# SakibSaikia/CPURayTracer

Hardware: AMD Instinct MI355X
Metric: Msamples/sec (WxHxspp/s), 1200x800 cover scene spp=128 d=50 (higher is better)
Workload: dtype f32; 1 GPU; cover scene (488 spheres, scene seed 1) 1200x800 spp=128 depth=50, render seed 1; rows sharded cyclically (row j to rank j mod N) over 1 GPU(s), RCCL gather of strips to rank 0; n_spheres=488, spp=128, spp_per_gpu=128, passes=1

## Files before the change

### cpuraytracer_amd/_capi.py

```python
import ctypes as C
import os

import numpy as np

_HERE = os.path.dirname(os.path.abspath(__file__))
LIB_PATH = os.path.join(_HERE, "lib", "librt_hip.so")


class RtSphere(C.Structure):
    _fields_ = [("cx", C.c_float), ("cy", C.c_float), ("cz", C.c_float), ("r", C.c_float)]


class RtMaterial(C.Structure):
    _fields_ = [("type", C.c_uint32), ("tex_type", C.c_uint32), ("smoothness", C.c_float), ("ior", C.c_float),
                ("tiling", C.c_float), ("rgb0", C.c_float * 3), ("rgb1", C.c_float * 3), ("luminance", C.c_float)]


class RtCamera(C.Structure):
    _fields_ = [("origin", C.c_float * 4), ("x", C.c_float * 4), ("y", C.c_float * 4),
                ("origin_image_plane", C.c_float * 4), ("aperture", C.c_float), ("focal_length", C.c_float)]


class RtLight(C.Structure):
    _fields_ = [("direction", C.c_float * 3), ("color", C.c_float * 3), ("luminance", C.c_float)]


class RtRowset(C.Structure):
    _fields_ = [("first_row", C.c_uint32), ("num_rows", C.c_uint32), ("block_rows", C.c_uint32),
                ("shard", C.c_uint32), ("nshards", C.c_uint32)]


class RtStats(C.Structure):
    _fields_ = [("samples", C.c_uint64), ("traversals", C.c_uint64), ("segments", C.c_uint64),
                ("ms_render", C.c_double), ("ms_accumulate", C.c_double), ("ms_resolve", C.c_double),
                ("local_rows", C.c_uint32), ("passes", C.c_uint32)]


SPHERE_DTYPE = np.dtype([("cx", "<f4"), ("cy", "<f4"), ("cz", "<f4"), ("r", "<f4")])
MATERIAL_DTYPE = np.dtype([("type", "<u4"), ("tex_type", "<u4"), ("smoothness", "<f4"), ("ior", "<f4"),
                           ("tiling", "<f4"), ("rgb0", "<f4", (3,)), ("rgb1", "<f4", (3,)), ("luminance", "<f4")])

RT_OK = 0
RT_ERR_NO_DEVICE = 1
RT_SAMPLER_COSINE_HEMISPHERE, RT_SAMPLER_SQRT_DISK = 1, 2

EXPORTS = [
    "rt_last_error", "rt_api_version", "rt_create", "rt_destroy", "rt_set_stream", "rt_set_workspace_limit", "rt_set_sampler", "rt_set_frame_pipelining", "rt_set_frame_batch", "rt_set_frame_lookahead", "rt_committed_samples",
    "rt_scene_upload", "rt_render", "rt_clear", "rt_resolve", "rt_last_resolve_ms", "rt_download", "rt_copy_to_device",
    "rt_synchronize", "rt_rowset_local_rows", "rt_rowset_global_row", "rt_unit_halton", "rt_unit_math",
    "rt_unit_primary_rays", "rt_unit_closest_hit", "rt_unit_trace", "rt_unit_camera_rays", "rt_unit_scatter", "rt_unit_tonemap", "rt_unit_layout", "rt_unit_layout_info", "rt_unit_grid_rows",
    "rt_unit_tile_masks", "rt_unit_tile_masks_host", "rt_unit_tile_cone",
]

_lib = None


class RtError(RuntimeError):
    def __init__(self, code, msg):
        super().__init__("librt_hip: [%d] %s" % (code, msg))
        self.code = code


def load():
    global _lib
    if _lib is not None:
        return _lib
    if not os.path.exists(LIB_PATH):
        raise RuntimeError("librt_hip.so is missing (%s): run `python -c 'import __graft_entry__ as g; g.build()'`; "
                           "there is no CPU fallback for the render path" % LIB_PATH)
    L = C.CDLL(LIB_PATH)
    L.rt_last_error.restype = C.c_char_p
    L.rt_api_version.restype = C.c_int
    L.rt_create.argtypes = [C.c_int, C.POINTER(C.c_void_p)]
    L.rt_destroy.argtypes = [C.c_void_p]
    L.rt_destroy.restype = None
    L.rt_set_stream.argtypes = [C.c_void_p, C.c_void_p]
    L.rt_set_workspace_limit.argtypes = [C.c_void_p, C.c_uint64]
    L.rt_set_sampler.argtypes = [C.c_void_p, C.c_uint32]
    L.rt_set_frame_pipelining.argtypes = [C.c_void_p, C.c_uint32]
    L.rt_set_frame_batch.argtypes = [C.c_void_p, C.c_uint32]
    L.rt_committed_samples.argtypes = [C.c_void_p, C.POINTER(C.c_uint32)]
    L.rt_set_frame_lookahead.argtypes = [C.c_void_p, C.c_uint32]
    L.rt_scene_upload.argtypes = [C.c_void_p, C.c_void_p, C.c_void_p, C.c_uint32, C.POINTER(RtCamera), C.POINTER(RtLight), C.c_uint32,
                                  C.POINTER(RtMaterial), C.c_float]
    L.rt_render.argtypes = [C.c_void_p, C.c_uint32, C.c_uint32, RtRowset, C.c_uint32, C.c_uint32, C.c_uint32, C.c_uint64,
                            C.POINTER(RtStats)]
    L.rt_clear.argtypes = [C.c_void_p]
    L.rt_resolve.argtypes = [C.c_void_p, C.c_uint32]
    L.rt_last_resolve_ms.argtypes = [C.c_void_p]
    L.rt_last_resolve_ms.restype = C.c_double
    L.rt_download.argtypes = [C.c_void_p, C.c_void_p, C.c_void_p]
    L.rt_copy_to_device.argtypes = [C.c_void_p, C.c_void_p, C.c_void_p]
    L.rt_synchronize.argtypes = [C.c_void_p]
    L.rt_rowset_local_rows.argtypes = [RtRowset]
    L.rt_rowset_local_rows.restype = C.c_uint32
    L.rt_rowset_global_row.argtypes = [RtRowset, C.c_uint32]
    L.rt_rowset_global_row.restype = C.c_uint32
    L.rt_unit_halton.argtypes = [C.c_void_p, C.c_void_p, C.c_uint32, C.c_uint32, C.c_void_p]
    L.rt_unit_math.argtypes = [C.c_void_p, C.c_uint32, C.c_void_p, C.c_void_p, C.c_uint32, C.c_void_p]
    L.rt_unit_primary_rays.argtypes = [C.c_void_p, C.c_uint32, C.c_uint32, C.c_void_p, C.c_uint32, C.c_void_p]
    L.rt_unit_closest_hit.argtypes = [C.c_void_p, C.c_void_p, C.c_uint32, C.c_void_p]
    L.rt_unit_trace.argtypes = [C.c_void_p, C.c_uint32, C.c_uint32, C.c_void_p, C.c_uint32, C.c_uint32, C.c_uint64,
                                C.c_void_p, C.c_void_p]
    L.rt_unit_camera_rays.argtypes = [C.c_void_p, C.POINTER(RtCamera), C.c_void_p, C.c_uint32, C.c_void_p]
    L.rt_unit_scatter.argtypes = [C.c_void_p, C.POINTER(RtMaterial), C.POINTER(RtLight), C.POINTER(C.c_float), C.c_void_p, C.c_uint32,
                                  C.c_void_p]
    L.rt_unit_tonemap.argtypes = [C.c_void_p, C.c_void_p, C.c_uint32, C.c_uint32, C.c_void_p]
    L.rt_unit_layout.argtypes = [C.c_void_p, C.c_uint32, C.c_uint32, C.POINTER(C.c_uint32), C.c_void_p, C.c_void_p]
    L.rt_unit_layout_info.argtypes = [C.c_void_p, C.c_uint32, C.POINTER(C.c_uint32)]
    if hasattr(L, "rt_unit_tile_masks"):
        L.rt_unit_tile_masks.argtypes = [C.c_void_p, C.c_uint32, C.c_uint32, RtRowset, C.c_uint32, C.POINTER(C.c_uint32), C.c_void_p,
                                         C.c_uint32, C.c_void_p, C.c_void_p]
        L.rt_unit_tile_masks_host.argtypes = [C.c_void_p, C.c_uint32, C.POINTER(RtCamera), C.c_uint32, C.c_uint32, RtRowset, C.c_uint32,
                                              C.c_uint32, C.POINTER(C.c_uint32), C.c_void_p, C.c_void_p]
        L.rt_unit_tile_cone.argtypes = [C.POINTER(RtCamera), C.c_uint32, C.c_uint32, C.c_uint32, C.c_uint32, C.c_uint32, C.c_void_p]
    _lib = L
    return L


def check(rc):
    if rc != RT_OK:
        raise RtError(rc, load().rt_last_error().decode())


def whole_image(H):
    return RtRowset(0, H, H, 0, 1)


BLOCK_ROWS = 1


def cyclic_rows(H, rank, world, block_rows=BLOCK_ROWS):
    return RtRowset(0, H, block_rows, rank, world)
```

### cpuraytracer_amd/csrc/rt_capi.hip

```cpp
#include <hip/hip_runtime.h>

#include <algorithm>
#include <cmath>
#include <cstdio>
#include <cstdlib>
#include <cstring>
#include <memory>
#include <mutex>
#include <set>
#include <string>
#include <unordered_map>
#include <array>
#include <utility>
#include <vector>

#include "../../include/rt_api.h"
#include "rt_kernels.h"

namespace {

thread_local std::string g_err;

int Fail(int code, const std::string& msg) {
    g_err = msg;
    return code;
}

#define RT_HIP(call)                                                                                             \
    do {                                                                                                         \
        hipError_t e_ = (call);                                                                                  \
        if (e_ != hipSuccess) {                                                                                  \
            return Fail(e_ == hipErrorOutOfMemory ? RT_ERR_OUT_OF_MEMORY : RT_ERR_HIP,                           \
                        std::string(#call) + ": " + hipGetErrorString(e_) + " (" __FILE__ ":" + std::to_string(__LINE__) + ")"); \
        }                                                                                                        \
    } while (0)

uint32_t EnvU32(const char* name, uint32_t dflt) {
    const char* v = std::getenv(name);
    if (!v || !*v) return dflt;
    return (uint32_t)std::strtoul(v, nullptr, 10);
}

uint32_t TreeTopFromEnv() {
    const uint32_t t = EnvU32("RT_TREE_TOP", 128);
    return (t < 4 || t > 128) ? 128u : t;
}

template <typename T>
struct DevBuf {
    T* ptr = nullptr;
    size_t count = 0;
    int Reserve(size_t n) {
        if (n <= count) return RT_OK;
        if (ptr) (void)hipFree(ptr);
        ptr = nullptr;
        count = 0;
        hipError_t e = hipMalloc(reinterpret_cast<void**>(&ptr), n * sizeof(T));
        if (e != hipSuccess) {
            (void)hipGetLastError();
            return Fail(RT_ERR_OUT_OF_MEMORY, std::string("hipMalloc: ") + hipGetErrorString(e));
        }
        count = n;
        return RT_OK;
    }
    void Release() {
        if (ptr) (void)hipFree(ptr);
        ptr = nullptr;
        count = 0;
    }
};

}

struct rt_ctx {
    int device = 0;
    hipStream_t ownStream = nullptr;
    hipStream_t stream = nullptr;
    hipEvent_t ev[4] = {nullptr, nullptr, nullptr, nullptr};
    std::vector<hipEvent_t> passEv;
    int cuCount = 0;
    size_t ldsPerBlockMax = 0;
    uint64_t workspaceLimit = 8ull << 30;

    bool hasScene = false;
    uint32_t n = 0;
    DevBuf<float4> scan, tree, leaf;
    DevBuf<uint32_t> orig;
    DevBuf<uint16_t> sgCells, sgEntries, sgGlobal;
    DevBuf<float4> sgSph;
    struct ExtraLight {
        DevBuf<uint16_t> cells, entries, global;
    };
    ExtraLight extraIdx[RT_MAX_LIGHTS];
    DevBuf<rtd::LightRec> lightRecs;
    DevBuf<uint16_t> gridCells;
    DevBuf<uint32_t> gridQ;
    bool useShadowGrid = true;
    DevBuf<float> radius;
    DevBuf<rt_material> mats;
    DevBuf<uint4> mats16;
    bool mats16Ok = false;
    rtd::TraceParams base{};

    uint32_t W = 0, H = 0, rows = 0;
    rt_rowset rs{};
    uint32_t accumulated = 0;
    uint32_t sampler = 0;
    DevBuf<float> hdr;
    DevBuf<uint8_t> ldr;
    DevBuf<float> samples;
    DevBuf<uint32_t> queue;
    DevBuf<unsigned long long> counters;
    DevBuf<float2> jitterTab, lensTab;
    double lastResolveMs = 0.0;

    uint32_t blocksPerCu = 4;
    uint32_t blockThreads = 256;
    bool useMfma = true;
    bool matsInLds = true;
    bool useRayCache = true;
    bool useStash = true;
    bool treeInLds = true;
    uint32_t treeTop = 128;
    bool forceGlobal = false;

    bool useTileOrder = true;
    bool tileOrderValid = false;
    uint32_t tileW = 0, tileH = 0;
    rt_rowset tileRs{};
    DevBuf<float> pilotRays, pilotHits;
    DevBuf<uint32_t> tileOrder, matType;
    DevBuf<uint8_t> tileClass;
    bool tileMaskValid = false;
    uint32_t maskW = 0, maskH = 0, maskLimit = 0, maskTiles = 0;
    rt_rowset maskRs{};
    DevBuf<uint32_t> tileMasks;
    uint64_t freshScans = 0;

    uint32_t pipeDepth = 0;
    bool pipeOpen = false;
    uint32_t pipeSeq = 0;
    uint32_t pipeSppCap = 0, pipeNpix = 0, pipeRing = 0;
    uint32_t pipeInSel = 0;
    uint32_t pipeCommits = 0;
    uint32_t batchFrames = 1;
    bool pendOn = false;
    uint32_t pendW = 0, pendH = 0, pendS0 = 0, pendS1 = 0, pendDepth = 0;
    rt_rowset pendRs{};
    uint64_t pendSeed = 0;
    uint32_t lookahead = 1;
    bool aheadValid = false;
    uint32_t aheadW = 0, aheadH = 0, aheadBase = 0, aheadSpp = 0, aheadNext = 0, aheadDepth = 0;
    rt_rowset aheadRs{};
    uint64_t aheadSeed = 0;
    uint32_t pipeMaxDepth = 0;
    uint64_t pipeSeed = 0;
    rtd::RegionTable pipeRegions{};
    DevBuf<float> ring;
    DevBuf<rtd::ContEntry> cont[2];
    DevBuf<uint32_t> contN[2];
    DevBuf<rtd::FrameCtl> ctl;
};

static uint32_t RowsetLocalRows(rt_rowset rs) {
    if (rs.block_rows == 0 || rs.nshards == 0 || rs.shard >= rs.nshards) return 0;
    uint32_t rows = 0;
    const uint32_t nblocks = (rs.num_rows + rs.block_rows - 1) / rs.block_rows;
    for (uint32_t b = rs.shard; b < nblocks; b += rs.nshards) {
        const uint32_t r0 = b * rs.block_rows;
        const uint32_t left = rs.num_rows - r0;
        rows += left < rs.block_rows ? left : rs.block_rows;
    }
    return rows;
}

struct SceneLayout {
    std::vector<float4> scan;
    std::vector<uint32_t> orig;
    std::vector<float4> leaf;
    std::vector<float4> tree;
    uint32_t levelOff[rtd::kMaxLevels] = {0}, levelCnt[rtd::kMaxLevels] = {0};
    uint32_t nLevels = 1;
    uint32_t nGroups = 0;
    float boundNorm = 0.f;
    unsigned long long singleMask[2] = {0ull, 0ull};
    uint32_t nAlways = 0;
    float treeBox[9] = {0, 0, 0, 0, 0, 0, 0, 0, 0};
    bool treeBoxOn = false;
    bool gridOn = false;
    std::vector<uint16_t> gridCellStart;
    uint32_t gridNu = 0, gridNv = 0, gridAxU = 0, gridAxV = 2;
    float gridG0u = 0.f, gridG0v = 0.f, gridInvH = 0.f, gridRmaxOverH = 0.f, gridBigNorm = 0.f;
    std::vector<uint32_t> gridQ;
    float gridQc[8] = {0, 0, 0, 0, 0, 0, 0, 0};
};

static float4 BoundOf(const rt_sphere* sp, const std::vector<uint32_t>& ids, float* normOut, float marginK) {
    if (ids.empty()) return make_float4(0.f, 0.f, 0.f, 1e30f);
    const double kEps = (double)marginK * 5.9604644775390625e-08;
    double lo[3] = {1e300, 1e300, 1e300}, hi[3] = {-1e300, -1e300, -1e300};
    for (uint32_t k : ids) {
        const double c[3] = {sp[k].cx, sp[k].cy, sp[k].cz};
        for (int a = 0; a < 3; ++a) {
            lo[a] = std::min(lo[a], c[a] - (double)sp[k].r);
            hi[a] = std::max(hi[a], c[a] + (double)sp[k].r);
        }
    }
    double cc[3] = {0.5 * (lo[0] + hi[0]), 0.5 * (lo[1] + hi[1]), 0.5 * (lo[2] + hi[2])};
    if (ids.size() > 1) {
        auto reachOf = [&](const double c[3]) {
            double far = 0.0;
            for (uint32_t k : ids) {
                const double dx = sp[k].cx - c[0], dy = sp[k].cy - c[1], dz = sp[k].cz - c[2];
                far = std::max(far, std::sqrt(dx * dx + dy * dy + dz * dz) + (double)sp[k].r);
            }
            return far;
        };
        double best = reachOf(cc);
        double step = 0.25 * best;
        for (int it = 0; it < 400 && step > 1e-7 * best; ++it) {
            bool improved = false;
            for (int ax = 0; ax < 3; ++ax)
                for (int sgn = -1; sgn <= 1; sgn += 2) {
                    double t[3] = {cc[0], cc[1], cc[2]};
                    t[ax] += sgn * step;
                    const double r = reachOf(t);
                    if (r < best) {
                        best = r;
                        cc[0] = t[0]; cc[1] = t[1]; cc[2] = t[2];
                        improved = true;
                    }
                }
            if (!improved) step *= 0.5;
        }
    }
    const float Cf[3] = {(float)cc[0], (float)cc[1], (float)cc[2]};
    double R = 0, smax = 0;
    for (uint32_t k : ids) {
        const double dx = sp[k].cx - (double)Cf[0], dy = sp[k].cy - (double)Cf[1], dz = sp[k].cz - (double)Cf[2];
        const double si = std::sqrt(dx * dx + dy * dy + dz * dz);
        smax = std::max(smax, si);
        R = std::max(R, si + (double)sp[k].r);
    }
    const double C2 = (double)Cf[0] * Cf[0] + (double)Cf[1] * Cf[1] + (double)Cf[2] * Cf[2];
    const double Cn = std::sqrt(C2);
    const double Rf2 = R * R * (1.0 + 1e-5) + 0.01 * smax * smax + kEps * (2.0 * (Cn + R) * (Cn + R) + R * R);
    float w = (float)(C2 - Rf2);
    w = std::nextafterf(std::nextafterf(w, -INFINITY), -INFINITY);
    if (normOut) *normOut = std::max(*normOut, (float)((Cn + R) * 1.001));
    return make_float4(Cf[0], Cf[1], Cf[2], w);
}

static double EnclosingRadius(const rt_sphere* sp, const uint32_t* ids, size_t n) {
    if (n == 0) return 0.0;
    double lo[3] = {1e300, 1e300, 1e300}, hi[3] = {-1e300, -1e300, -1e300};
    for (size_t q = 0; q < n; ++q) {
        const rt_sphere& s = sp[ids[q]];
        const double c[3] = {s.cx, s.cy, s.cz};
        for (int a = 0; a < 3; ++a) {
            lo[a] = std::min(lo[a], c[a] - (double)s.r);
            hi[a] = std::max(hi[a], c[a] + (double)s.r);
        }
    }
    double cc[3] = {0.5 * (lo[0] + hi[0]), 0.5 * (lo[1] + hi[1]), 0.5 * (lo[2] + hi[2])};
    auto reachOf = [&](const double c[3]) {
        double far = 0.0;
        for (size_t q = 0; q < n; ++q) {
            const rt_sphere& s = sp[ids[q]];
            const double dx = s.cx - c[0], dy = s.cy - c[1], dz = s.cz - c[2];
            far = std::max(far, std::sqrt(dx * dx + dy * dy + dz * dz) + (double)s.r);
        }
        return far;
    };
    double best = reachOf(cc);
    if (n == 1) return best;
    double step = 0.25 * best;
    for (int it = 0; it < 60 && step > 1e-4 * best; ++it) {
        bool improved = false;
        for (int ax = 0; ax < 3; ++ax)
            for (int sgn = -1; sgn <= 1; sgn += 2) {
                double t[3] = {cc[0], cc[1], cc[2]};
                t[ax] += sgn * step;
                const double r = reachOf(t);
                if (r < best) { best = r; cc[0] = t[0]; cc[1] = t[1]; cc[2] = t[2]; improved = true; }
            }
        if (!improved) step *= 0.5;
    }
    return best;
}
// ... 577 lines not shown
            tp.ray_cache_off16 = (uint32_t)(ldsBytes / 16);
            tp.ray_cache_stride16 = (cap * rtd::kStashDwords * 4 + 15) / 16;
            ldsBytes += (size_t)wavesPerBlock * tp.ray_cache_stride16 * 16;
        }
        if (matsL2 && !useStash) return Fail(RT_ERR_HIP, "internal: materials through L2 without the stash variant");
        const bool matsGlobal = matsL2 || tree || (grid && !gridLds) || !tp.mats_in_lds || (!flat && !ldsTables && !gridLds);
        if (want16 && tp.mats16_mode == 0u && matsGlobal) tp.mats16_mode = 1u;
    }
    if (!useStash && ctx->useRayCache && ldsBytes + (size_t)wavesPerBlock * rtd::kRayCacheBytes <= 160 * 1024 / ctx->blocksPerCu) {
        tp.ray_cache_off16 = (uint32_t)(ldsBytes / 16);
        tp.ray_cache_stride16 = rtd::kRayCacheBytes / 16;
        ldsBytes += (size_t)wavesPerBlock * rtd::kRayCacheBytes;
    }
    if (std::getenv("RT_VERBOSE"))
        std::fprintf(stderr, "rt_trace launch: tree=%d flat=%d ldsTables=%d blocks=%u threads=%u lds=%zu B (cand %zu, tables %zu, leaf %zu, ops %zu, sg %zu, tree %zu, cache %s, stash %u)\n",
                     (int)tree, (int)flat + 2 * (int)grid + 4 * (int)gridLds, (int)ldsTables, blocks, ctx->blockThreads, ldsBytes, candBytes, ldsTables ? lds : (size_t)0, flat ? leafBytes : (size_t)0,
                     (flat || tree) ? MfmaOpsBytesFor(topCnt) : (size_t)0, sgBytes, treeBytes, (tp.ray_cache_off16 && !useStash) ? "yes" : "no", tp.stash_cap);
    const bool hitLds = flat && tp.mats_in_lds && (sgBytes != 0 || !tp.sg_enabled);
    if (carryMode != 0) {
        const bool ok = hitLds && tp.ray_cache_off16 != 0 && ctx->blockThreads == 1024;
        if (carryMode == 1) return ok ? RT_OK : RT_ERR_INVALID_ARG;
        if (!ok) return Fail(RT_ERR_INVALID_ARG, "frame pipelining needs the flat LDS variant of the trace kernel");
    }
#define RT_LAUNCH_FN(KERNEL)                                                                                                  \
    do {                                                                                                                      \
        const void* fn_ = reinterpret_cast<const void*>(&KERNEL);                                                             \
         \
        if (ldsBytes > 48 * 1024 && RaiseLdsLimit(ctx->device, fn_) != RT_OK) return RT_ERR_HIP;                               \
        hipLaunchKernelGGL(KERNEL, dim3(blocks), dim3(ctx->blockThreads), ldsBytes, ctx->stream, tp);                         \
    } while (0)
#define RT_LAUNCH_K(...)                                                          \
    do {                                                                          \
        if (tp.n_lights == 1u) RT_LAUNCH_FN((rtd::rt_trace_kernel<__VA_ARGS__>)); \
        else RT_LAUNCH_FN((rtd::rt_trace_kernel_lights<__VA_ARGS__>));            \
    } while (0)
#define RT_LAUNCH(LDS, T, M)                                                                        \
    do {                                                                                            \
        if (((M) == 1 && hitLds) || ((M) == 2 && tp.tree_in_lds)) {                                 \
            if (tp.ray_cache_off16) RT_LAUNCH_K(LDS, T, M, true, (M) != 0);  \
            else RT_LAUNCH_K(LDS, T, M, false, (M) != 0);                    \
        } else {                                                                                    \
            if (tp.ray_cache_off16) RT_LAUNCH_K(LDS, T, M, true, false);    \
            else RT_LAUNCH_K(LDS, T, M, false, false);                      \
        }                                                                                           \
    } while (0)
#define RT_LAUNCH_T(LDS, M)                                            \
    do {                                                               \
        if (ctx->blockThreads == 1024) RT_LAUNCH(LDS, 1024, M);        \
        else if (ctx->blockThreads == 512) RT_LAUNCH(LDS, 512, M);     \
        else RT_LAUNCH(LDS, 256, M);                                   \
    } while (0)
    if (carryMode == 2) RT_LAUNCH_K(true, 1024, 1, true, true, true);
    else if (gridLds && useStash && tp.grid_in_lds) RT_LAUNCH_K(true, 1024, 3, true, true, false, true);
    else if (gridLds && tp.grid_in_lds && tp.ray_cache_off16) RT_LAUNCH_K(true, 1024, 3, true, true);
    else if (gridLds && tp.grid_in_lds) RT_LAUNCH_K(true, 1024, 3, false, true);
    else if (grid && gridSgLds && useStash && tp.grid_in_lds) RT_LAUNCH_K(false, 1024, 3, true, true, false, true, false, true);
    else if (grid && gridSgLds) return Fail(RT_ERR_HIP, "internal: the grid variant with the shadow index in LDS needs the hit stash");
    else if (grid && ctx->blockThreads == 1024 && useStash && tp.grid_in_lds && gridQBytes != 0) RT_LAUNCH_K(false, 1024, 3, true, true, false, true, false, false, true);
    else if (grid && gridQBytes != 0) return Fail(RT_ERR_HIP, "internal: quantised grid bounds without the stash variant");
    else if (grid && ctx->blockThreads == 1024 && useStash && tp.grid_in_lds) RT_LAUNCH_K(false, 1024, 3, true, true, false, true);
    else if (grid && ctx->blockThreads == 1024 && tp.grid_in_lds && tp.ray_cache_off16) RT_LAUNCH_K(false, 1024, 3, true, true);
    else if (grid && ctx->blockThreads == 1024 && tp.grid_in_lds) RT_LAUNCH_K(false, 1024, 3, false, true);
    else if (grid && ctx->blockThreads == 1024) RT_LAUNCH_K(false, 1024, 3, false, false);
    else if (grid && ctx->blockThreads == 512 && !tp.ray_cache_off16) RT_LAUNCH_K(false, 512, 3, false, false);
    else if (grid && ctx->blockThreads == 512) RT_LAUNCH_K(false, 512, 3, true, false);
    else if (grid && !tp.ray_cache_off16) RT_LAUNCH_K(false, 256, 3, false, false);
    else if (grid) RT_LAUNCH_K(false, 256, 3, true, false);
    else if (useStash && tree && tp.tree_in_lds) RT_LAUNCH_K(false, 1024, 2, true, true, false, true);
    else if (useStash && tree) RT_LAUNCH_K(false, 1024, 2, true, false, false, true);
    else if (useStash && hitLds && matsL2) RT_LAUNCH_K(true, 1024, 1, true, true, false, true, true);
    else if (useStash && hitLds) RT_LAUNCH_K(true, 1024, 1, true, true, false, true);
    else if (useStash) RT_LAUNCH_K(true, 1024, 1, true, false, false, true);
    else if (tree) RT_LAUNCH_T(false, 2);
    else if (flat) RT_LAUNCH_T(true, 1);
    else if (ldsTables) RT_LAUNCH_T(true, 0);
    else RT_LAUNCH_T(false, 0);
#undef RT_LAUNCH_T
#undef RT_LAUNCH
#undef RT_LAUNCH_K
#undef RT_LAUNCH_FN
    RT_HIP(hipGetLastError());
    return RT_OK;
}


static int LaunchClosest(rt_ctx* ctx, const float* dRays, uint32_t n, float* dOut) {
        rtd::TraceParams tp = ctx->base;
        const TraceVariant V = ChooseVariant(ctx, tp);
        tp.mats_in_lds = 0;
        tp.sg_in_lds = 0;
        const uint32_t topCnt = tp.level_cnt[tp.n_levels - 1];
        const size_t waves = 256 / 64;
        size_t ldsBytes = waves * (V.grid ? rtd::kWaveGridBytes : (V.tree ? rtd::kWaveCandBytes : rtd::kWaveListBytes));
        if (V.grid) {
            tp.grid_in_lds = 0;
        } else if (V.tree) {
            ldsBytes += MfmaOpsBytesFor(topCnt);
            const size_t treeBytes = (size_t)(tp.level_off[tp.n_levels - 1] + topCnt) * 16;
            tp.tree_in_lds = (ctx->treeInLds && ldsBytes + treeBytes <= 160 * 1024) ? 1u : 0u;
            if (tp.tree_in_lds) ldsBytes += treeBytes;
        } else if (V.flat || V.ldsTables) {
            ldsBytes += LdsBytesFor(tp.n, tp.n_padded, false);
            if (V.flat) ldsBytes += V.leafBytes + MfmaOpsBytesFor(topCnt);
        }
#define RT_UNIT_CLOSEST(LDS, M)                                                                                        \
    do {                                                                                                               \
        const void* fn_ = reinterpret_cast<const void*>(&rtd::k_unit_closest<LDS, M>);                                 \
        if (ldsBytes > 48 * 1024) RT_HIP(hipFuncSetAttribute(fn_, hipFuncAttributeMaxDynamicSharedMemorySize, (int)ldsBytes)); \
        hipLaunchKernelGGL((rtd::k_unit_closest<LDS, M>), dim3((n + 255) / 256), dim3(256), ldsBytes, ctx->stream, tp, dRays, n, dOut); \
    } while (0)
        if (V.grid) RT_UNIT_CLOSEST(false, 3);
        else if (V.tree) RT_UNIT_CLOSEST(false, 2);
        else if (V.flat) RT_UNIT_CLOSEST(true, 1);
        else if (V.ldsTables) RT_UNIT_CLOSEST(true, 0);
        else RT_UNIT_CLOSEST(false, 0);
#undef RT_UNIT_CLOSEST
        RT_HIP(hipGetLastError());
    return RT_OK;
}

static int BuildTileOrder(rt_ctx* ctx, uint32_t W, uint32_t H, rt_rowset rs, uint32_t npix) {
    if (ctx->tileOrderValid && ctx->tileW == W && ctx->tileH == H && std::memcmp(&ctx->tileRs, &rs, sizeof(rs)) == 0) return RT_OK;
    ctx->tileOrderValid = false;
    const uint32_t nFull = npix >> 6;
    if (!ctx->useTileOrder || nFull < 2u * (uint32_t)ctx->cuCount) return RT_OK;
    int rc;
    const uint32_t nPilot = nFull * rtd::kPilotsPerTile;
    if ((rc = ctx->pilotRays.Reserve((size_t)nPilot * 6)) != RT_OK) return rc;
    if ((rc = ctx->pilotHits.Reserve((size_t)nPilot * 10)) != RT_OK) return rc;
    if ((rc = ctx->tileClass.Reserve(nFull)) != RT_OK) return rc;
    if ((rc = ctx->tileOrder.Reserve(nFull)) != RT_OK) return rc;
    rtd::TraceParams tp = ctx->base;
    tp.W = W;
    tp.H = H;
    tp.rs = rs;
    tp.s0 = 1;
    tp.sampler = ctx->sampler;
    tp.jitter_tab = nullptr;
    tp.lens_tab = nullptr;
    hipLaunchKernelGGL(rtd::rt_pilot_rays_kernel, dim3((nPilot + 255) / 256), dim3(256), 0, ctx->stream, tp, nFull, ctx->pilotRays.ptr);
    RT_HIP(hipGetLastError());
    if ((rc = LaunchClosest(ctx, ctx->pilotRays.ptr, nPilot, ctx->pilotHits.ptr)) != RT_OK) return rc;
    hipLaunchKernelGGL(rtd::rt_tile_class_kernel, dim3((nFull + 255) / 256), dim3(256), 0, ctx->stream, ctx->pilotHits.ptr, nFull, W,
                       ctx->matType.ptr, ctx->tileClass.ptr);
    hipLaunchKernelGGL(rtd::rt_tile_order_kernel, dim3(1), dim3(1024), 0, ctx->stream, ctx->tileClass.ptr, nFull, ctx->tileOrder.ptr);
    RT_HIP(hipGetLastError());
    ctx->tileOrderValid = true;
    ctx->tileW = W;
    ctx->tileH = H;
    ctx->tileRs = rs;
    return RT_OK;
}

static int BuildTileMasks(rt_ctx* ctx, uint32_t W, uint32_t H, rt_rowset rs, uint32_t npix) {
    const uint32_t limit = EnvU32("RT_PRIMARY_MASK_LIMIT", rtd::kTileMaskLimitDefault);
    const uint32_t nFull = npix >> 6;
    const rtd::TraceParams& b = ctx->base;
    const bool wanted = EnvU32("RT_PRIMARY_MASK", 1u) != 0u && nFull != 0u && b.n_levels == 1u && b.level_cnt[0] <= 128u &&
                        ChooseVariant(ctx, b).flat;
    if (!wanted) {
        ctx->tileMaskValid = false;
        return RT_OK;
    }
    if (ctx->tileMaskValid && ctx->maskW == W && ctx->maskH == H && ctx->maskLimit == limit && std::memcmp(&ctx->maskRs, &rs, sizeof(rs)) == 0)
        return RT_OK;
    ctx->tileMaskValid = false;
    int rc;
    if ((rc = ctx->tileMasks.Reserve((size_t)nFull * rtd::kTileMaskWords)) != RT_OK) return rc;
    rtd::TraceParams tp = b;
    tp.W = W;
    tp.H = H;
    tp.rs = rs;
    hipLaunchKernelGGL(rtd::rt_tile_mask_kernel, dim3((nFull + 3) / 4), dim3(256), 0, ctx->stream, tp, nFull, limit, ctx->tileMasks.ptr);
    RT_HIP(hipGetLastError());
    ctx->tileMaskValid = true;
    ctx->maskW = W;
    ctx->maskH = H;
    ctx->maskLimit = limit;
    ctx->maskTiles = nFull;
    ctx->maskRs = rs;
    return RT_OK;
}

static void PipelineDrop(rt_ctx* ctx) { ctx->pipeOpen = false; }
static uint32_t PipelineWaves(const rt_ctx* ctx) { return (uint32_t)ctx->cuCount * ctx->blocksPerCu * (ctx->blockThreads / 64); }
static void PipelineShards(const rt_ctx* ctx, rtd::TraceParams& tp) {
    uint32_t qb = EnvU32("RT_PIPE_QUEUE_BLOCK", rtd::kCarryQueueBlock) / 64u * 64u;
    if (qb == 0) qb = 64;
    QueueShards(tp, PipelineWaves(ctx), qb, EnvU32("RT_PIPE_STATIC_BLOCKS", 1));
}

static int PipelineTraceAndCommit(rt_ctx* ctx, rtd::TraceParams& tp, uint32_t npix, bool carry) {
    tp.ctl = ctx->ctl.ptr;
    tp.cont_in = ctx->cont[ctx->pipeInSel].ptr;
    tp.cont_in_n = ctx->contN[ctx->pipeInSel].ptr;
    tp.cont_out = ctx->cont[ctx->pipeInSel ^ 1u].ptr;
    tp.cont_out_n = ctx->contN[ctx->pipeInSel ^ 1u].ptr;
    tp.carry = carry ? 1u : 0u;
    tp.region_seq = ctx->pipeSeq;
    tp.max_carry_age = ctx->pipeDepth;
    tp.min_iters = EnvU32("RT_PIPE_MIN_ITERS", 8);
    tp.counters = ctx->counters.ptr;
    int rc = LaunchTrace(ctx, tp, 2);
    if (rc != RT_OK) return rc;
    hipLaunchKernelGGL(rtd::rt_commit_kernel, dim3((npix + 255) / 256), dim3(256), 0, ctx->stream, ctx->ring.ptr, ctx->hdr.ptr, npix,
                       npix * ctx->pipeSppCap, ctx->pipeRing, ctx->pipeRegions, ctx->ctl.ptr, ctx->pipeSeq, ctx->pipeCommits);
    RT_HIP(hipGetLastError());
    ++ctx->pipeCommits;
    ctx->pipeInSel ^= 1u;
    return RT_OK;
}

static int PipelineFlush(rt_ctx* ctx) {
    if (!ctx->pipeOpen) return RT_OK;
    const uint32_t npix = ctx->pipeNpix;
    rtd::TraceParams tp = ctx->base;
    tp.total_paths = 0;
    PipelineShards(ctx, tp);
    hipLaunchKernelGGL(rtd::rt_raygen_tables_kernel, dim3(1), dim3(256), 0, ctx->stream, (float2*)nullptr, 0u, 0u, (float2*)nullptr, 0u, 0u,
                       ctx->sampler, ctx->queue.ptr, ctx->ctl.ptr);
    RT_HIP(hipGetLastError());
    tp.W = ctx->W;
    tp.H = ctx->H;
    tp.rs = ctx->rs;
    tp.s0 = 1;
    tp.spp_pass = 1;
    tp.npix_local = npix;
    tp.max_depth = ctx->pipeMaxDepth;
    tp.sampler = ctx->sampler;
    tp.seed = ctx->pipeSeed;
    tp.samples = ctx->ring.ptr;
    int rc = PipelineTraceAndCommit(ctx, tp, npix, false);
    ctx->pipeOpen = false;
    if (rc != RT_OK) ctx->accumulated = 0;
    return rc;
}

static int PipelineRender(rt_ctx* ctx, uint32_t W, uint32_t H, rt_rowset rs, uint32_t npix, uint32_t s0, uint32_t s1, uint32_t max_depth,
                          uint64_t seed) {
    const uint32_t spp = s1 - s0;
    const uint32_t nRing = ctx->pipeDepth + 2u;
    int rc;
    if (ctx->pipeOpen && (ctx->pipeNpix != npix || spp > ctx->pipeSppCap || ctx->pipeRing != nRing || ctx->pipeMaxDepth != max_depth ||
                          ctx->pipeSeed != seed)) {
        if ((rc = PipelineFlush(ctx)) != RT_OK) return rc;
    }
    if (!ctx->pipeOpen) {
        ctx->pipeNpix = npix;
        ctx->pipeSppCap = spp;
        ctx->pipeRing = nRing;
        ctx->pipeMaxDepth = max_depth;
        ctx->pipeSeed = seed;
        ctx->pipeInSel = 0;
        ctx->pipeRegions = rtd::RegionTable{};
        const size_t waves = PipelineWaves(ctx);
        if ((rc = ctx->ring.Reserve((size_t)nRing * npix * spp * 3)) != RT_OK) return rc;
        for (int k = 0; k < 2; ++k) {
            if ((rc = ctx->cont[k].Reserve(waves * 64)) != RT_OK) return rc;
            if ((rc = ctx->contN[k].Reserve(waves)) != RT_OK) return rc;
            RT_HIP(hipMemsetAsync(ctx->contN[k].ptr, 0, waves * sizeof(uint32_t), ctx->stream));
        }
        if ((rc = ctx->ctl.Reserve(1)) != RT_OK) return rc;
        rtd::FrameCtl init{};
        init.oldest_open = 0xffffffffu;
        init.committed_seq[0] = ctx->pipeSeq;
        init.committed_samples[0] = ctx->accumulated;
        ctx->pipeCommits = 0;
        RT_HIP(hipMemcpyAsync(ctx->ctl.ptr, &init, sizeof(init), hipMemcpyHostToDevice, ctx->stream));
        RT_HIP(hipStreamSynchronize(ctx->stream));
        ctx->pipeOpen = true;
    }
    const uint32_t seq = ++ctx->pipeSeq;
    const uint32_t slot = seq % nRing;
    ctx->pipeRegions.seq[slot] = seq;
    ctx->pipeRegions.spp[slot] = spp;
    rtd::TraceParams tp = ctx->base;
    tp.W = W;
    tp.H = H;
    tp.rs = rs;
    tp.s0 = s0;
    tp.spp_pass = spp;
    tp.total_paths = npix * spp;
    tp.npix_local = npix;
    tp.max_depth = max_depth;
    tp.sampler = ctx->sampler;
    tp.seed = seed;
    tp.path_list = nullptr;
    tp.tile_order = nullptr;
    tp.samples = ctx->ring.ptr;
    tp.sample_base = slot * npix * ctx->pipeSppCap;
    tp.trav_out = nullptr;
    const uint32_t k0 = s0 + rs.first_row;
    const uint32_t nLens = spp + W + rs.num_rows;
    if ((rc = ctx->jitterTab.Reserve(spp)) != RT_OK) return rc;
    if ((rc = ctx->lensTab.Reserve(nLens)) != RT_OK) return rc;
    tp.jitter_tab = ctx->jitterTab.ptr;
    tp.lens_tab = ctx->lensTab.ptr;
    tp.lens_k0 = k0;
    const uint32_t nmax = spp > nLens ? spp : nLens;
    PipelineShards(ctx, tp);
    hipLaunchKernelGGL(rtd::rt_raygen_tables_kernel, dim3((nmax + 255) / 256), dim3(256), 0, ctx->stream, ctx->jitterTab.ptr, s0, spp,
                       ctx->lensTab.ptr, k0, nLens, ctx->sampler, ctx->queue.ptr, ctx->ctl.ptr);
    RT_HIP(hipGetLastError());
    return PipelineTraceAndCommit(ctx, tp, npix, true);
}

namespace {
template <typename T>
struct TmpDev {
    T* p = nullptr;
    ~TmpDev() {
        if (p) (void)hipFree(p);
    }
    hipError_t Alloc(size_t n) { return hipMalloc(reinterpret_cast<void**>(&p), (n ? n : 1) * sizeof(T)); }
};
}

extern "C" {

const char* rt_last_error(void) { return g_err.c_str(); }
int rt_api_version(void) { return RT_API_VERSION; }

int rt_create(int device_ordinal, rt_ctx** out) {
    if (!out) return Fail(RT_ERR_INVALID_ARG, "rt_create: null out");
    *out = nullptr;
    int count = 0;
    hipError_t e = hipGetDeviceCount(&count);
    if (e != hipSuccess || count <= 0)
        return Fail(RT_ERR_NO_DEVICE, std::string("rt_create: no HIP device (") + hipGetErrorString(e) +
                                          "); this library has no CPU fallback");
    if (device_ordinal < 0 || device_ordinal >= count) return Fail(RT_ERR_NO_DEVICE, "rt_create: device ordinal out of range");
    RT_HIP(hipSetDevice(device_ordinal));
    std::unique_ptr<rt_ctx, void (*)(rt_ctx*)> guard(new rt_ctx(), rt_destroy);
    rt_ctx* ctx = guard.get();
    ctx->device = device_ordinal;
    hipDeviceProp_t prop;
    RT_HIP(hipGetDeviceProperties(&prop, device_ordinal));
    ctx->cuCount = prop.multiProcessorCount;
    ctx->ldsPerBlockMax = prop.sharedMemPerBlock;
    RT_HIP(hipStreamCreateWithFlags(&ctx->ownStream, hipStreamNonBlocking));
    ctx->stream = ctx->ownStream;
    for (auto& ev : ctx->ev) RT_HIP(hipEventCreate(&ev));
    {
        const char* scan = std::getenv("RT_SCAN");
        ctx->useMfma = !(scan && std::strcmp(scan, "valu") == 0);
        ctx->matsInLds = EnvU32("RT_MATS_LDS", 1) != 0;
        ctx->useShadowGrid = EnvU32("RT_SHADOW_GRID", 1) != 0;
        ctx->useRayCache = EnvU32("RT_RAY_CACHE", 1) != 0;
        ctx->useStash = EnvU32("RT_STASH", 1) != 0;
        ctx->treeInLds = EnvU32("RT_TREE_LDS", 1) != 0;
        ctx->useTileOrder = EnvU32("RT_TILE_ORDER", 1) != 0;
        ctx->treeTop = TreeTopFromEnv();
    }
    ctx->blocksPerCu = EnvU32("RT_BLOCKS_PER_CU", ctx->useMfma ? 1 : 4);
    if (ctx->blocksPerCu == 0) ctx->blocksPerCu = 1;
    ctx->forceGlobal = EnvU32("RT_FORCE_GLOBAL_TABLES", 0) != 0;
    ctx->blockThreads = EnvU32("RT_BLOCK_THREADS", ctx->useMfma ? 1024 : 256);
    if (ctx->blockThreads != 256 && ctx->blockThreads != 512 && ctx->blockThreads != 1024) ctx->blockThreads = 256;
    int rc = ctx->queue.Reserve(rtd::kQueueShards * rtd::kShardStrideWords);
    if (rc == RT_OK) rc = ctx->counters.Reserve(4);
    if (rc != RT_OK) return rc;
    {
        size_t freeB = 0, totalB = 0;
        RT_HIP(hipMemGetInfo(&freeB, &totalB));
        uint64_t lim = 64ull << 30;
        if (lim > freeB / 2) lim = freeB / 2;
        const uint32_t envGiB = EnvU32("RT_WORKSPACE_GIB", 0);
        if (envGiB) lim = (uint64_t)envGiB << 30;
        if (lim < (1ull << 20)) lim = 1ull << 20;
        ctx->workspaceLimit = lim;
    }
    *out = guard.release();
    return RT_OK;
}

void rt_destroy(rt_ctx* ctx) {
    if (!ctx) return;
    (void)hipSetDevice(ctx->device);
    (void)hipStreamSynchronize(ctx->stream);
    ctx->scan.Release();
    ctx->orig.Release();
    ctx->tree.Release();
    ctx->sgCells.Release();
    ctx->gridCells.Release();
    ctx->gridQ.Release();
    ctx->sgEntries.Release();
    ctx->sgGlobal.Release();
    ctx->sgSph.Release();
    for (auto& x : ctx->extraIdx) {
        x.cells.Release();
        x.entries.Release();
        x.global.Release();
    }
    ctx->lightRecs.Release();
    ctx->radius.Release();
    ctx->mats.Release();
    ctx->mats16.Release();
    ctx->hdr.Release();
    ctx->ldr.Release();
    ctx->samples.Release();
    ctx->queue.Release();
    ctx->counters.Release();
    ctx->jitterTab.Release();
    ctx->lensTab.Release();
    ctx->leaf.Release();
    ctx->pilotRays.Release();
    ctx->pilotHits.Release();
    ctx->tileOrder.Release();
    ctx->tileMasks.Release();
    ctx->tileClass.Release();
    ctx->matType.Release();
    ctx->ring.Release();
    ctx->cont[0].Release();
    ctx->cont[1].Release();
    ctx->contN[0].Release();
    ctx->contN[1].Release();
    ctx->ctl.Release();
    for (auto& ev : ctx->ev)
        if (ev) (void)hipEventDestroy(ev);
    for (auto& ev : ctx->passEv)
        if (ev) (void)hipEventDestroy(ev);
    if (ctx->ownStream) (void)hipStreamDestroy(ctx->ownStream);
    delete ctx;
}

static int BatchFlush(rt_ctx* ctx);

int rt_set_stream(rt_ctx* ctx, void* hip_stream) {
    if (!ctx) return Fail(RT_ERR_INVALID_ARG, "rt_set_stream: null ctx");
    {
        RT_HIP(hipSetDevice(ctx->device));
        const int rcb = BatchFlush(ctx);
        if (rcb != RT_OK) return rcb;
        const int rcf = PipelineFlush(ctx);
        if (rcf != RT_OK) return rcf;
    }
    ctx->aheadValid = false;
    ctx->stream = hip_stream ? reinterpret_cast<hipStream_t>(hip_stream) : ctx->ownStream;
    return RT_OK;
}

int rt_set_workspace_limit(rt_ctx* ctx, uint64_t bytes) {
    if (!ctx || bytes < (1u << 20)) return Fail(RT_ERR_INVALID_ARG, "rt_set_workspace_limit: need >= 1 MiB");
    ctx->workspaceLimit = bytes;
    return RT_OK;
}

static bool PackMaterials(const std::vector<rt_material>& matc, std::vector<uint4>& out) {
    auto byteOf = [](float c, uint32_t& b) {
        const float r = std::nearbyint(c * 255.0f);
        if (!(r >= 0.f && r <= 255.f)) return false;
        b = (uint32_t)r;
        return (float)b * (1.0f / 255.0f) == c;
    };
    out.assign(matc.size(), make_uint4(0u, 0u, 0u, 0u));
    for (size_t e = 0; e < matc.size(); ++e) {
        const rt_material& m = matc[e];
        if (m.type > 3u || m.tex_type > 1u) return false;
        uint32_t c0[3] = {0, 0, 0}, c1[3] = {0, 0, 0};
        const bool glass = m.type == RT_MAT_DIELECTRIC_TRANSPARENT;
        for (int k = 0; k < 3; ++k) {
            if (!glass && !byteOf(m.rgb0[k], c0[k])) return false;
            if (!glass && m.tex_type == RT_TEX_CHECKER && !byteOf(m.rgb1[k], c1[k])) return false;
        }
        const float slotA = m.type == RT_MAT_EMISSIVE ? m.luminance : m.smoothness;
        const float slotB = glass ? m.ior : m.tiling;
        uint32_t a, b;
        std::memcpy(&a, &slotA, 4);
        std::memcpy(&b, &slotB, 4);
        out[e] = make_uint4(m.type | m.tex_type << 2 | c0[0] << 8 | c0[1] << 16 | c0[2] << 24, c1[0] | c1[1] << 8 | c1[2] << 16, a, b);
    }
    return true;
}

int rt_scene_upload(rt_ctx* ctx, const rt_sphere* spheres, const rt_material* materials, uint32_t n, const rt_camera* camera,
                    const rt_light* lights, uint32_t n_lights, const rt_material* sky, float exposure_scale) {
    if (!ctx || !spheres || !materials || !camera || (!lights && n_lights != 0) || !sky || n == 0)
        return Fail(RT_ERR_INVALID_ARG, "rt_scene_upload: null pointer or empty scene");
    if (n_lights > RT_MAX_LIGHTS) return Fail(RT_ERR_INVALID_ARG, "rt_scene_upload: more than RT_MAX_LIGHTS lights");
    const rt_light noLight{{0.f, 1.f, 0.f}, {0.f, 0.f, 0.f}, 0.f};
    const rt_light* sun = n_lights ? lights : &noLight;
    RT_HIP(hipSetDevice(ctx->device));
    int rc;
    if ((rc = BatchFlush(ctx)) != RT_OK) return rc;
    SceneLayout L;
    BuildLayout(spheres, n, ctx->treeTop, L);
    if (L.scan.size() >= 65536) return Fail(RT_ERR_INVALID_ARG, "rt_scene_upload: scenes beyond 65,535 scan entries (about 65,000 spheres) are not supported");
    const uint32_t nPad = (uint32_t)L.scan.size();
    if ((rc = ctx->scan.Reserve(nPad)) != RT_OK) return rc;
    if ((rc = ctx->orig.Reserve(nPad)) != RT_OK) return rc;
    if ((rc = ctx->tree.Reserve(L.tree.size())) != RT_OK) return rc;
    if ((rc = ctx->leaf.Reserve(nPad)) != RT_OK) return rc;
    if ((rc = ctx->radius.Reserve(nPad)) != RT_OK) return rc;
    if ((rc = ctx->mats.Reserve(nPad)) != RT_OK) return rc;
    std::vector<float> rad(nPad, 0.f);
    std::vector<rt_material> matc(nPad);
    std::memset(matc.data(), 0, nPad * sizeof(rt_material));
    for (uint32_t e = 0; e < nPad; ++e) {
        if (L.orig[e] == 0xffffffffu) continue;
        rad[e] = spheres[L.orig[e]].r;
        matc[e] = materials[L.orig[e]];
    }
    RT_HIP(hipStreamSynchronize(ctx->stream));
    RT_HIP(hipMemcpy(ctx->scan.ptr, L.scan.data(), nPad * sizeof(float4), hipMemcpyHostToDevice));
    RT_HIP(hipMemcpy(ctx->orig.ptr, L.orig.data(), nPad * sizeof(uint32_t), hipMemcpyHostToDevice));
    RT_HIP(hipMemcpy(ctx->tree.ptr, L.tree.data(), L.tree.size() * sizeof(float4), hipMemcpyHostToDevice));
    RT_HIP(hipMemcpy(ctx->leaf.ptr, L.leaf.data(), nPad * sizeof(float4), hipMemcpyHostToDevice));
    RT_HIP(hipMemcpy(ctx->radius.ptr, rad.data(), nPad * sizeof(float), hipMemcpyHostToDevice));
    RT_HIP(hipMemcpy(ctx->mats.ptr, matc.data(), nPad * sizeof(rt_material), hipMemcpyHostToDevice));
    {
        std::vector<uint4> m16;
        ctx->mats16Ok = PackMaterials(matc, m16);
        if (ctx->mats16Ok) {
            if ((rc = ctx->mats16.Reserve(nPad)) != RT_OK) return rc;
            RT_HIP(hipMemcpy(ctx->mats16.ptr, m16.data(), nPad * sizeof(uint4), hipMemcpyHostToDevice));
        }
    }
    {
        std::vector<uint32_t> types(n);
        for (uint32_t k = 0; k < n; ++k) types[k] = materials[k].type;
        if ((rc = ctx->matType.Reserve(n)) != RT_OK) return rc;
        RT_HIP(hipMemcpy(ctx->matType.ptr, types.data(), n * sizeof(uint32_t), hipMemcpyHostToDevice));
        ctx->tileOrderValid = false;
        ctx->tileMaskValid = false;
    }

    ShadowGrid SG;
    if (ctx->useShadowGrid && n_lights != 0) BuildShadowGrid(spheres, L, sun->direction, (L.gridOn || L.nLevels > 1) ? EnvU32("RT_SHADOW_CELLS", 256u) : 64u, SG);
    std::vector<rtd::LightRec> recs;
    for (uint32_t k = 1; k < n_lights; ++k) {
        ShadowGrid G2;
        if (ctx->useShadowGrid) BuildShadowGrid(spheres, L, lights[k].direction, EnvU32("RT_SHADOW_CELLS", 256u), G2);
        rt_ctx::ExtraLight& X = ctx->extraIdx[k];
        rtd::LightRec R{};
        for (int c = 0; c < 3; ++c) {
            R.sun_dir[c] = lights[k].direction[c];
            R.sun_rad[c] = lights[k].luminance * lights[k].color[c];
            R.cam_o[c] = camera->origin[c];
        }
        R.sg_enabled = G2.enabled ? 1u : 0u;
        if (G2.enabled) {
            if ((rc = X.cells.Reserve(G2.cellStart.size())) != RT_OK) return rc;
            if ((rc = X.entries.Reserve(G2.entries.size() + 1)) != RT_OK) return rc;
            if ((rc = X.global.Reserve(G2.global.size() + 1)) != RT_OK) return rc;
            RT_HIP(hipMemcpy(X.cells.ptr, G2.cellStart.data(), G2.cellStart.size() * 2, hipMemcpyHostToDevice));
            if (!G2.entries.empty()) RT_HIP(hipMemcpy(X.entries.ptr, G2.entries.data(), G2.entries.size() * 2, hipMemcpyHostToDevice));
            if (!G2.global.empty()) RT_HIP(hipMemcpy(X.global.ptr, G2.global.data(), G2.global.size() * 2, hipMemcpyHostToDevice));
            for (int c = 0; c < 3; ++c) {
                R.sg_e1[c] = G2.e1[c];
                R.sg_e2[c] = G2.e2[c];
            }
            R.sg_u0 = G2.u0; R.sg_v0 = G2.v0; R.sg_inv_cell = G2.invCell; R.sg_p0sq = G2.p0sq;
            R.sg_nx = G2.nx; R.sg_ny = G2.ny; R.sg_nglobal = (uint32_t)G2.global.size();
            R.cell_start = X.cells.ptr; R.entries = X.entries.ptr; R.global = X.global.ptr;
        }
        recs.push_back(R);
    }
    if (!recs.empty()) {
        if ((rc = ctx->lightRecs.Reserve(recs.size())) != RT_OK) return rc;
        RT_HIP(hipMemcpy(ctx->lightRecs.ptr, recs.data(), recs.size() * sizeof(rtd::LightRec), hipMemcpyHostToDevice));
    }
    if (SG.enabled) {
// ... 139 lines not shown
    ctx->aheadValid = false;
    PipelineDrop(ctx);
    ctx->accumulated = 0;
    return RT_OK;
}

uint32_t rt_rowset_local_rows(rt_rowset rs) { return RowsetLocalRows(rs); }
uint32_t rt_rowset_global_row(rt_rowset rs, uint32_t lr) {
    const uint32_t lb = lr / rs.block_rows;
    const uint32_t k = lr % rs.block_rows;
    return rs.first_row + (lb * rs.nshards + rs.shard) * rs.block_rows + k;
}

static int RenderNow(rt_ctx* ctx, uint32_t W, uint32_t H, rt_rowset rs, uint32_t s0, uint32_t s1, uint32_t max_depth, uint64_t seed,
                     rt_stats* out_stats, uint32_t aheadEnd = 0);

static int BatchFlush(rt_ctx* ctx) {
    if (!ctx->pendOn) return RT_OK;
    ctx->pendOn = false;
    return RenderNow(ctx, ctx->pendW, ctx->pendH, ctx->pendRs, ctx->pendS0, ctx->pendS1, ctx->pendDepth, ctx->pendSeed, nullptr);
}

static bool PendingMustRender(const rt_ctx* ctx) { return ctx->pendOn && (ctx->accumulated == 0 || ctx->pendS0 == 1u); }

int rt_set_frame_batch(rt_ctx* ctx, uint32_t frames) {
    if (!ctx || frames == 0 || frames > 4096) return Fail(RT_ERR_INVALID_ARG, "rt_set_frame_batch: frames must be 1..4096");
    RT_HIP(hipSetDevice(ctx->device));
    const int rc = BatchFlush(ctx);
    ctx->batchFrames = frames;
    return rc;
}

int rt_set_frame_lookahead(rt_ctx* ctx, uint32_t frames) {
    if (!ctx || frames == 0 || frames > 4096) return Fail(RT_ERR_INVALID_ARG, "rt_set_frame_lookahead: frames must be 1..4096");
    ctx->lookahead = frames;
    ctx->aheadValid = false;
    return RT_OK;
}

int rt_render(rt_ctx* ctx, uint32_t W, uint32_t H, rt_rowset rs, uint32_t s0, uint32_t s1, uint32_t max_depth, uint64_t seed,
              rt_stats* out_stats) {
    if (!ctx) return Fail(RT_ERR_INVALID_ARG, "rt_render: null ctx");
    if (ctx->lookahead > 1 && ctx->batchFrames <= 1 && ctx->pipeDepth == 0 && out_stats == nullptr && ctx->hasScene && W != 0 && H != 0 && s0 != 0 && s1 > s0) {
        if (ctx->aheadValid && ctx->aheadW == W && ctx->aheadH == H && std::memcmp(&ctx->aheadRs, &rs, sizeof(rs)) == 0 && ctx->aheadDepth == max_depth &&
            ctx->aheadSeed == seed && s0 == ctx->aheadNext && s1 <= ctx->aheadBase + ctx->aheadSpp && ctx->accumulated + 1 == s0) {
            RT_HIP(hipSetDevice(ctx->device));
            const uint32_t npix = ctx->W * ctx->rows;
            hipLaunchKernelGGL(rtd::rt_accumulate_kernel, dim3((npix + 255) / 256), dim3(256), 0, ctx->stream, ctx->samples.ptr, ctx->hdr.ptr, npix,
                               ctx->aheadSpp, s0 - ctx->aheadBase, s1 - s0);
            RT_HIP(hipGetLastError());
            ctx->aheadNext = s1;
            ctx->accumulated += s1 - s0;
            return RT_OK;
        }
        const uint32_t want = s1 - s0 > ctx->lookahead ? s1 - s0 : ctx->lookahead;
        return RenderNow(ctx, W, H, rs, s0, s1, max_depth, seed, nullptr, s0 + want);
    }
    if (ctx->batchFrames > 1 && out_stats == nullptr && ctx->pipeDepth == 0 && ctx->hasScene && W != 0 && H != 0 && s0 != 0 && s1 > s0) {
        if (ctx->pendOn && !(ctx->pendW == W && ctx->pendH == H && std::memcmp(&ctx->pendRs, &rs, sizeof(rs)) == 0 && ctx->pendDepth == max_depth &&
                             ctx->pendSeed == seed && ctx->pendS1 == s0)) {
            const int rcf = BatchFlush(ctx);
            if (rcf != RT_OK) return rcf;
        }
        if (!ctx->pendOn) {
            const uint32_t rows = RowsetLocalRows(rs);
            const bool sameStrip = ctx->W == W && ctx->H == H && ctx->rows == rows && std::memcmp(&ctx->rs, &rs, sizeof(rs)) == 0;
            const bool starts = s0 == 1, continues = ctx->accumulated != 0 && sameStrip && s0 == ctx->accumulated + 1;
            if (rows != 0 && (uint64_t)rs.first_row + rs.num_rows <= H && (starts || continues)) {
                ctx->pendOn = true;
                ctx->pendW = W; ctx->pendH = H; ctx->pendRs = rs; ctx->pendS0 = s0; ctx->pendDepth = max_depth; ctx->pendSeed = seed;
            }
        }
        if (ctx->pendOn) {
            ctx->pendS1 = s1;
            if (ctx->pendS1 - ctx->pendS0 >= ctx->batchFrames) return BatchFlush(ctx);
            return RT_OK;
        }
    }
    const int rcb = BatchFlush(ctx);
    if (rcb != RT_OK) return rcb;
    return RenderNow(ctx, W, H, rs, s0, s1, max_depth, seed, out_stats);
}

static int RenderNow(rt_ctx* ctx, uint32_t W, uint32_t H, rt_rowset rs, uint32_t s0, uint32_t s1, uint32_t max_depth, uint64_t seed,
                     rt_stats* out_stats, uint32_t aheadEnd) {
    ctx->aheadValid = false;
    if (!ctx->hasScene) return Fail(RT_ERR_NO_SCENE, "rt_render: no scene uploaded");
    if (W == 0 || H == 0 || s0 == 0 || s1 <= s0) return Fail(RT_ERR_INVALID_ARG, "rt_render: empty image or sample range");
    const uint32_t rows = RowsetLocalRows(rs);
    if (rows == 0 || (uint64_t)rs.first_row + rs.num_rows > H) return Fail(RT_ERR_INVALID_ARG, "rt_render: bad row set");
    const uint64_t npix64 = (uint64_t)W * rows;
    if (npix64 > (1ull << 31) || (uint64_t)W * H > 0xffffffffull) return Fail(RT_ERR_INVALID_ARG, "rt_render: image too large");
    RT_HIP(hipSetDevice(ctx->device));
    const uint32_t npix = (uint32_t)npix64;

    const bool sameStrip = ctx->W == W && ctx->H == H && ctx->rows == rows && std::memcmp(&ctx->rs, &rs, sizeof(rs)) == 0;
    bool pipelined = ctx->pipeDepth > 0 && out_stats == nullptr;
    if (pipelined) {
        rtd::TraceParams probe = ctx->base;
        probe.total_paths = npix;
        pipelined = LaunchTrace(ctx, probe, 1) == RT_OK && (uint64_t)npix * (s1 - s0) * (ctx->pipeDepth + 2u) < (1ull << 31);
    }
    if (s0 == 1 || ctx->accumulated == 0) PipelineDrop(ctx);
    else if (!pipelined) {
        int rcf = PipelineFlush(ctx);
        if (rcf != RT_OK) return rcf;
    }
    if (s0 == 1 || ctx->accumulated == 0) {
        if (s0 != 1) return Fail(RT_ERR_SEQUENCE, "rt_render: first call of an accumulation must start at s0 == 1");
        int rc;
        if ((rc = ctx->hdr.Reserve((size_t)npix * 3)) != RT_OK) return rc;
        if ((rc = ctx->ldr.Reserve((size_t)npix * 3)) != RT_OK) return rc;
        RT_HIP(hipMemsetAsync(ctx->hdr.ptr, 0, (size_t)npix * 3 * sizeof(float), ctx->stream));
        ctx->W = W;
        ctx->H = H;
        ctx->rows = rows;
        ctx->rs = rs;
        ctx->accumulated = 0;
        if ((rc = BuildTileOrder(ctx, W, H, rs, npix)) != RT_OK) return rc;
        if ((rc = BuildTileMasks(ctx, W, H, rs, npix)) != RT_OK) return rc;
    } else if (!sameStrip || s0 != ctx->accumulated + 1) {
        return Fail(RT_ERR_SEQUENCE, "rt_render: sample range or row set does not continue the accumulation");
    }

    if (pipelined) {
        int rcp = PipelineRender(ctx, W, H, rs, npix, s0, s1, max_depth, seed);
        if (rcp != RT_OK) {
            ctx->accumulated = 0;
            PipelineDrop(ctx);
            return rcp;
        }
        ctx->accumulated += s1 - s0;
        return RT_OK;
    }

    const uint64_t bytesPerSpp = (uint64_t)npix * 12;
    uint64_t sppMax = ctx->workspaceLimit / bytesPerSpp;
    const uint64_t sppPathCap = ((1ull << 31) - 1) / npix;
    if (sppMax > sppPathCap) sppMax = sppPathCap;
    if (sppMax == 0) return Fail(RT_ERR_OUT_OF_MEMORY, "rt_render: workspace limit below one sample per pixel");
    const uint32_t sppTotal = s1 - s0;
    if (aheadEnd <= s1 || (uint64_t)(aheadEnd - s0) > sppMax || pipelined) aheadEnd = 0;
    const uint32_t sppTrace = aheadEnd ? aheadEnd - s0 : sppTotal;
    uint32_t sppPass = (uint32_t)(sppMax < sppTrace ? sppMax : sppTrace);
    int rc;
    while ((rc = ctx->samples.Reserve((size_t)npix * sppPass * 3)) != RT_OK) {
        if (rc != RT_ERR_OUT_OF_MEMORY || sppPass == 1u) return rc;
        sppPass = (sppPass + 1u) / 2u;
    }

    uint32_t passes = 0;
    auto runPasses = [&]() -> int {
        int rc;
        RT_HIP(hipMemsetAsync(ctx->counters.ptr, 0, 4 * sizeof(unsigned long long), ctx->stream));
        ctx->freshScans = 0;
        const uint32_t sEnd = aheadEnd ? aheadEnd : s1;
        for (uint32_t s = s0; s < sEnd; s += sppPass) {
            const uint32_t spp = (sEnd - s) < sppPass ? (sEnd - s) : sppPass;
            rtd::TraceParams tp = ctx->base;
            tp.W = W;
            tp.H = H;
            tp.rs = rs;
            tp.s0 = s;
            tp.spp_pass = spp;
            tp.total_paths = npix * spp;
            tp.npix_local = npix;
            tp.max_depth = max_depth;
            tp.sampler = ctx->sampler;
            tp.seed = seed;
            tp.path_list = nullptr;
            tp.tile_order = ctx->tileOrderValid ? ctx->tileOrder.ptr : nullptr;
            tp.tile_masks = (ctx->tileMaskValid && ctx->maskW == W && ctx->maskH == H && std::memcmp(&ctx->maskRs, &rs, sizeof(rs)) == 0) ? ctx->tileMasks.ptr : nullptr;
            ctx->freshScans += ((uint64_t)tp.total_paths + 63u) / 64u;
            tp.samples = ctx->samples.ptr;
            tp.trav_out = nullptr;
            tp.counters = ctx->counters.ptr;
            const uint32_t k0 = s + rs.first_row;
            const uint32_t nLens = spp + W + rs.num_rows;
            if ((rc = ctx->jitterTab.Reserve(spp)) != RT_OK) return rc;
            if ((rc = ctx->lensTab.Reserve(nLens)) != RT_OK) return rc;
            tp.jitter_tab = ctx->jitterTab.ptr;
            tp.lens_tab = ctx->lensTab.ptr;
            tp.lens_k0 = k0;
            while (ctx->passEv.size() < 3 * (size_t)(passes + 1)) {
                hipEvent_t e = nullptr;
                RT_HIP(hipEventCreate(&e));
                ctx->passEv.push_back(e);
            }
            hipEvent_t* ev = ctx->passEv.data() + 3 * (size_t)passes;
            RT_HIP(hipEventRecord(ev[0], ctx->stream));
            {
                const uint32_t nmax = spp > nLens ? spp : nLens;
                hipLaunchKernelGGL(rtd::rt_raygen_tables_kernel, dim3((nmax + 255) / 256), dim3(256), 0, ctx->stream, ctx->jitterTab.ptr, s,
                                   spp, ctx->lensTab.ptr, k0, nLens, ctx->sampler);
                RT_HIP(hipGetLastError());
            }
            if ((rc = LaunchTrace(ctx, tp)) != RT_OK) return rc;
            RT_HIP(hipEventRecord(ev[1], ctx->stream));
            hipLaunchKernelGGL(rtd::rt_accumulate_kernel, dim3((npix + 255) / 256), dim3(256), 0, ctx->stream, ctx->samples.ptr,
                               ctx->hdr.ptr, npix, spp, 0u, aheadEnd ? sppTotal : spp);
            RT_HIP(hipGetLastError());
            RT_HIP(hipEventRecord(ev[2], ctx->stream));
            ++passes;
        }
        return RT_OK;
    };
    if ((rc = runPasses()) != RT_OK) {
        ctx->accumulated = 0;
        return rc;
    }
    ctx->accumulated += sppTotal;
    if (aheadEnd && ctx->samples.ptr && passes == 1) {
        ctx->aheadValid = true;
        ctx->aheadW = W; ctx->aheadH = H; ctx->aheadRs = rs; ctx->aheadDepth = max_depth; ctx->aheadSeed = seed;
        ctx->aheadBase = s0; ctx->aheadSpp = sppTrace; ctx->aheadNext = s1;
    }

    if (out_stats) {
        float msTrace = 0.f, msAcc = 0.f;
        RT_HIP(hipEventSynchronize(ctx->passEv[3 * (size_t)(passes - 1) + 2]));
        for (uint32_t k = 0; k < passes; ++k) {
            float a = 0.f, b = 0.f;
            RT_HIP(hipEventElapsedTime(&a, ctx->passEv[3 * (size_t)k], ctx->passEv[3 * (size_t)k + 1]));
            RT_HIP(hipEventElapsedTime(&b, ctx->passEv[3 * (size_t)k + 1], ctx->passEv[3 * (size_t)k + 2]));
            msTrace += a;
            msAcc += b;
        }
        unsigned long long c[2] = {0, 0};
        RT_HIP(hipMemcpy(c, ctx->counters.ptr, sizeof(c), hipMemcpyDeviceToHost));
        std::memset(out_stats, 0, sizeof(*out_stats));
        out_stats->samples = (uint64_t)npix * sppTotal;
        out_stats->traversals = c[0];
        out_stats->segments = c[1];
        out_stats->ms_render = msTrace;
        out_stats->ms_accumulate = msAcc;
        out_stats->ms_resolve = 0.0;
        out_stats->local_rows = rows;
        out_stats->passes = passes;
    }
    return RT_OK;
}

int rt_resolve(rt_ctx* ctx, uint32_t n_samples) {
    if (!ctx) return Fail(RT_ERR_INVALID_ARG, "rt_resolve: null ctx");
    if (PendingMustRender(ctx)) {
        const int rcb = BatchFlush(ctx);
        if (rcb != RT_OK) return rcb;
    }
    if (ctx->accumulated == 0) return Fail(RT_ERR_SEQUENCE, "rt_resolve: nothing accumulated");
    RT_HIP(hipSetDevice(ctx->device));
    const uint32_t n = n_samples ? n_samples : ctx->accumulated;
    const uint32_t npix = ctx->W * ctx->rows;
    RT_HIP(hipEventRecord(ctx->ev[0], ctx->stream));
    const uint32_t* devCount = (ctx->pipeOpen && n_samples == 0) ? &ctx->ctl.ptr->committed_samples[ctx->pipeCommits & 1u] : nullptr;
    hipLaunchKernelGGL(rtd::rt_resolve_kernel, dim3((npix + 255) / 256), dim3(256), 0, ctx->stream, ctx->hdr.ptr, ctx->ldr.ptr, npix, n,
                       devCount);
    RT_HIP(hipGetLastError());
    RT_HIP(hipEventRecord(ctx->ev[1], ctx->stream));
    RT_HIP(hipEventSynchronize(ctx->ev[1]));
    float ms = 0.f;
    RT_HIP(hipEventElapsedTime(&ms, ctx->ev[0], ctx->ev[1]));
    ctx->lastResolveMs = ms;
    return RT_OK;
}

double rt_last_resolve_ms(rt_ctx* ctx) { return ctx ? ctx->lastResolveMs : 0.0; }

int rt_download(rt_ctx* ctx, float* hdr_rgb, uint8_t* ldr_rgb) {
    if (!ctx) return Fail(RT_ERR_INVALID_ARG, "rt_download: null ctx");
    if (PendingMustRender(ctx)) {
        const int rcb = BatchFlush(ctx);
        if (rcb != RT_OK) return rcb;
    }
    if (ctx->accumulated == 0) return Fail(RT_ERR_SEQUENCE, "rt_download: nothing rendered");
    RT_HIP(hipSetDevice(ctx->device));
    const size_t npix = (size_t)ctx->W * ctx->rows;
    RT_HIP(hipStreamSynchronize(ctx->stream));
    if (hdr_rgb) RT_HIP(hipMemcpy(hdr_rgb, ctx->hdr.ptr, npix * 3 * sizeof(float), hipMemcpyDeviceToHost));
    if (ldr_rgb) RT_HIP(hipMemcpy(ldr_rgb, ctx->ldr.ptr, npix * 3, hipMemcpyDeviceToHost));
    return RT_OK;
}

int rt_copy_to_device(rt_ctx* ctx, void* dev_hdr_rgb, void* dev_ldr_rgb) {
    if (!ctx) return Fail(RT_ERR_INVALID_ARG, "rt_copy_to_device: null ctx");
    if (PendingMustRender(ctx)) {
        const int rcb = BatchFlush(ctx);
        if (rcb != RT_OK) return rcb;
    }
    if (ctx->accumulated == 0) return Fail(RT_ERR_SEQUENCE, "rt_copy_to_device: nothing rendered");
    RT_HIP(hipSetDevice(ctx->device));
    const size_t npix = (size_t)ctx->W * ctx->rows;
    if (dev_hdr_rgb) RT_HIP(hipMemcpyAsync(dev_hdr_rgb, ctx->hdr.ptr, npix * 3 * sizeof(float), hipMemcpyDeviceToDevice, ctx->stream));
    if (dev_ldr_rgb) RT_HIP(hipMemcpyAsync(dev_ldr_rgb, ctx->ldr.ptr, npix * 3, hipMemcpyDeviceToDevice, ctx->stream));
    return RT_OK;
}

int rt_synchronize(rt_ctx* ctx) {
    if (!ctx) return Fail(RT_ERR_INVALID_ARG, "rt_synchronize: null ctx");
    RT_HIP(hipSetDevice(ctx->device));
    int rcf = BatchFlush(ctx);
    if (rcf != RT_OK) return rcf;
    rcf = PipelineFlush(ctx);
    if (rcf != RT_OK) return rcf;
    RT_HIP(hipStreamSynchronize(ctx->stream));
    return RT_OK;
}

int rt_unit_halton(rt_ctx* ctx, const uint32_t* index, uint32_t base, uint32_t n, float* out) {
    if (!ctx || !index || !out || base < 2) return Fail(RT_ERR_INVALID_ARG, "rt_unit_halton: invalid argument");
    if (n == 0) return RT_OK;
    RT_HIP(hipSetDevice(ctx->device));
    TmpDev<uint32_t> dIdx;
    TmpDev<float> dOut;
    RT_HIP(dIdx.Alloc(n));
    RT_HIP(dOut.Alloc(n));
    RT_HIP(hipMemcpy(dIdx.p, index, n * sizeof(uint32_t), hipMemcpyHostToDevice));
    hipLaunchKernelGGL(rtd::k_unit_halton, dim3((n + 255) / 256), dim3(256), 0, ctx->stream, dIdx.p, base, n, dOut.p);
    RT_HIP(hipGetLastError());
    RT_HIP(hipStreamSynchronize(ctx->stream));
    RT_HIP(hipMemcpy(out, dOut.p, n * sizeof(float), hipMemcpyDeviceToHost));
    return RT_OK;
}

int rt_unit_math(rt_ctx* ctx, uint32_t op, const float* x, const float* y, uint32_t n, float* out) {
    if (!ctx || !x || !out || op > 9) return Fail(RT_ERR_INVALID_ARG, "rt_unit_math: invalid argument");
    if (n == 0) return RT_OK;
    RT_HIP(hipSetDevice(ctx->device));
    TmpDev<float> dX, dY, dOut;
    RT_HIP(dX.Alloc(n));
    RT_HIP(dY.Alloc(n));
    RT_HIP(dOut.Alloc(n));
    RT_HIP(hipMemcpy(dX.p, x, n * sizeof(float), hipMemcpyHostToDevice));
    if (y) RT_HIP(hipMemcpy(dY.p, y, n * sizeof(float), hipMemcpyHostToDevice));
    else RT_HIP(hipMemset(dY.p, 0, n * sizeof(float)));
    hipLaunchKernelGGL(rtd::k_unit_math, dim3((n + 255) / 256), dim3(256), 0, ctx->stream, op, dX.p, dY.p, n, dOut.p);
    RT_HIP(hipGetLastError());
    RT_HIP(hipStreamSynchronize(ctx->stream));
    RT_HIP(hipMemcpy(out, dOut.p, n * sizeof(float), hipMemcpyDeviceToHost));
    return RT_OK;
}

int rt_unit_primary_rays(rt_ctx* ctx, uint32_t W, uint32_t H, const uint32_t* ijs, uint32_t n, float* out_rays) {
    if (!ctx || !ijs || !out_rays || W == 0 || H == 0) return Fail(RT_ERR_INVALID_ARG, "rt_unit_primary_rays: invalid argument");
    if (!ctx->hasScene) return Fail(RT_ERR_NO_SCENE, "rt_unit_primary_rays: no scene uploaded");
    if (n == 0) return RT_OK;
    RT_HIP(hipSetDevice(ctx->device));
    TmpDev<uint32_t> dIjs;
    TmpDev<float> dOut;
    RT_HIP(dIjs.Alloc((size_t)n * 3));
    RT_HIP(dOut.Alloc((size_t)n * 6));
    RT_HIP(hipMemcpy(dIjs.p, ijs, (size_t)n * 3 * sizeof(uint32_t), hipMemcpyHostToDevice));
    rtd::TraceParams tp = ctx->base;
    tp.W = W;
    tp.H = H;
    tp.sampler = ctx->sampler;
    hipLaunchKernelGGL(rtd::k_unit_primary, dim3((n + 255) / 256), dim3(256), 0, ctx->stream, tp, dIjs.p, n, dOut.p);
    RT_HIP(hipGetLastError());
    RT_HIP(hipStreamSynchronize(ctx->stream));
    RT_HIP(hipMemcpy(out_rays, dOut.p, (size_t)n * 6 * sizeof(float), hipMemcpyDeviceToHost));
    return RT_OK;
}

int rt_unit_closest_hit(rt_ctx* ctx, const float* rays, uint32_t n, float* out_hits) {
    if (!ctx || !rays || !out_hits) return Fail(RT_ERR_INVALID_ARG, "rt_unit_closest_hit: invalid argument");
    if (!ctx->hasScene) return Fail(RT_ERR_NO_SCENE, "rt_unit_closest_hit: no scene uploaded");
    if (n == 0) return RT_OK;
    RT_HIP(hipSetDevice(ctx->device));
    TmpDev<float> dRays, dOut;
    RT_HIP(dRays.Alloc((size_t)n * 6));
    RT_HIP(dOut.Alloc((size_t)n * 10));
    RT_HIP(hipMemcpy(dRays.p, rays, (size_t)n * 6 * sizeof(float), hipMemcpyHostToDevice));
    {
        const int rcl = LaunchClosest(ctx, dRays.p, n, dOut.p);
        if (rcl != RT_OK) return rcl;
    }
    RT_HIP(hipGetLastError());
    RT_HIP(hipStreamSynchronize(ctx->stream));
    RT_HIP(hipMemcpy(out_hits, dOut.p, (size_t)n * 10 * sizeof(float), hipMemcpyDeviceToHost));
    return RT_OK;
}

int rt_unit_trace(rt_ctx* ctx, uint32_t W, uint32_t H, const uint32_t* ijs, uint32_t n, uint32_t max_depth, uint64_t seed,
                  float* out_rgb, uint32_t* out_traversals) {
    if (!ctx || !ijs || !out_rgb || W == 0 || H == 0) return Fail(RT_ERR_INVALID_ARG, "rt_unit_trace: invalid argument");
    if (!ctx->hasScene) return Fail(RT_ERR_NO_SCENE, "rt_unit_trace: no scene uploaded");
    if (n == 0) return RT_OK;
    RT_HIP(hipSetDevice(ctx->device));
    TmpDev<uint32_t> dIjs, dTrav;
    TmpDev<float> dOut;
    RT_HIP(dIjs.Alloc((size_t)n * 3));
    RT_HIP(dTrav.Alloc(n));
    RT_HIP(dOut.Alloc((size_t)n * 3));
    RT_HIP(hipMemcpy(dIjs.p, ijs, (size_t)n * 3 * sizeof(uint32_t), hipMemcpyHostToDevice));
    RT_HIP(hipMemsetAsync(ctx->counters.ptr, 0, 4 * sizeof(unsigned long long), ctx->stream));
    rtd::TraceParams tp = ctx->base;
    tp.W = W;
    tp.H = H;
    tp.rs = rt_rowset{0, H, H, 0, 1};
    tp.s0 = 1;
    tp.spp_pass = 1;
    tp.total_paths = n;
    tp.npix_local = n;
    tp.max_depth = max_depth;
    tp.sampler = ctx->sampler;
    tp.seed = seed;
    tp.path_list = dIjs.p;
    tp.jitter_tab = nullptr;
    tp.lens_tab = nullptr;
    tp.samples = dOut.p;
    tp.trav_out = dTrav.p;
    tp.counters = ctx->counters.ptr;
    int rc = LaunchTrace(ctx, tp);
    if (rc != RT_OK) return rc;
    RT_HIP(hipStreamSynchronize(ctx->stream));
    RT_HIP(hipMemcpy(out_rgb, dOut.p, (size_t)n * 3 * sizeof(float), hipMemcpyDeviceToHost));
    if (out_traversals) RT_HIP(hipMemcpy(out_traversals, dTrav.p, n * sizeof(uint32_t), hipMemcpyDeviceToHost));
    return RT_OK;
}

int rt_unit_camera_rays(rt_ctx* ctx, const rt_camera* camera, const float* uv_offset, uint32_t n, float* out_rays) {
    if (!ctx || !camera || !uv_offset || !out_rays) return Fail(RT_ERR_INVALID_ARG, "rt_unit_camera_rays: invalid argument");
    if (n == 0) return RT_OK;
    RT_HIP(hipSetDevice(ctx->device));
    TmpDev<float> dIn, dOut;
    RT_HIP(dIn.Alloc((size_t)n * 4));
    RT_HIP(dOut.Alloc((size_t)n * 6));
    RT_HIP(hipMemcpy(dIn.p, uv_offset, (size_t)n * 4 * sizeof(float), hipMemcpyHostToDevice));
    rtd::TraceParams tp{};
    for (int k = 0; k < 3; ++k) {
        tp.cam_o[k] = camera->origin[k];
        tp.cam_x[k] = camera->x[k];
        tp.cam_y[k] = camera->y[k];
        tp.cam_oip[k] = camera->origin_image_plane[k];
    }
    tp.aperture = camera->aperture;
    tp.focal = camera->focal_length;
    hipLaunchKernelGGL(rtd::k_unit_camera, dim3((n + 255) / 256), dim3(256), 0, ctx->stream, tp, dIn.p, n, dOut.p);
    RT_HIP(hipGetLastError());
    RT_HIP(hipStreamSynchronize(ctx->stream));
    RT_HIP(hipMemcpy(out_rays, dOut.p, (size_t)n * 6 * sizeof(float), hipMemcpyDeviceToHost));
    return RT_OK;
}

int rt_unit_scatter(rt_ctx* ctx, const rt_material* material, const rt_light* sun, const float view_origin[3], const float* in,
                    uint32_t n, float* out) {
    if (!ctx || !material || !sun || !view_origin || !in || !out) return Fail(RT_ERR_INVALID_ARG, "rt_unit_scatter: invalid argument");
    if (n == 0) return RT_OK;
    RT_HIP(hipSetDevice(ctx->device));
    TmpDev<float> dIn, dOut;
    TmpDev<rt_material> dMat;
    RT_HIP(dIn.Alloc((size_t)n * 12));
    RT_HIP(dOut.Alloc((size_t)n * 11));
    RT_HIP(dMat.Alloc(1));
    RT_HIP(hipMemcpy(dIn.p, in, (size_t)n * 12 * sizeof(float), hipMemcpyHostToDevice));
    RT_HIP(hipMemcpy(dMat.p, material, sizeof(rt_material), hipMemcpyHostToDevice));
    rtd::TraceParams tp{};
    for (int k = 0; k < 3; ++k) {
        tp.cam_o[k] = view_origin[k];
        tp.sun_dir[k] = sun->direction[k];
        tp.sun_rad[k] = sun->luminance * sun->color[k];
    }
    tp.sampler = ctx->sampler;
    hipLaunchKernelGGL(rtd::k_unit_scatter, dim3((n + 255) / 256), dim3(256), 0, ctx->stream, tp, dMat.p, dIn.p, n, dOut.p);
    RT_HIP(hipGetLastError());
    RT_HIP(hipStreamSynchronize(ctx->stream));
    RT_HIP(hipMemcpy(out, dOut.p, (size_t)n * 11 * sizeof(float), hipMemcpyDeviceToHost));
    return RT_OK;
}

int rt_unit_tonemap(rt_ctx* ctx, const float* hdr_rgb, uint32_t n, uint32_t n_samples, uint8_t* out_rgb) {
    if (!ctx || !hdr_rgb || !out_rgb || n_samples == 0) return Fail(RT_ERR_INVALID_ARG, "rt_unit_tonemap: invalid argument");
    if (n == 0) return RT_OK;
    RT_HIP(hipSetDevice(ctx->device));
    TmpDev<float> dIn;
    TmpDev<uint8_t> dOut;
    RT_HIP(dIn.Alloc((size_t)n * 3));
    RT_HIP(dOut.Alloc((size_t)n * 3));
    RT_HIP(hipMemcpy(dIn.p, hdr_rgb, (size_t)n * 3 * sizeof(float), hipMemcpyHostToDevice));
    hipLaunchKernelGGL(rtd::k_unit_tonemap, dim3((n + 255) / 256), dim3(256), 0, ctx->stream, dIn.p, n, n_samples, dOut.p);
    RT_HIP(hipGetLastError());
    RT_HIP(hipStreamSynchronize(ctx->stream));
    RT_HIP(hipMemcpy(out_rgb, dOut.p, (size_t)n * 3, hipMemcpyDeviceToHost));
    return RT_OK;
}

int rt_unit_layout(const rt_sphere* spheres, uint32_t n, uint32_t cap_groups, uint32_t* n_groups, uint32_t* orig, float* bounds) {
    if (!spheres || n == 0 || !n_groups) return Fail(RT_ERR_INVALID_ARG, "rt_unit_layout: invalid argument");
    SceneLayout L;
    BuildLayout(spheres, n, TreeTopFromEnv(), L);
    *n_groups = L.nGroups;
    if (cap_groups == 0) return RT_OK;
    if (cap_groups < L.nGroups || !orig || !bounds) return Fail(RT_ERR_INVALID_ARG, "rt_unit_layout: capacity too small");
    std::memcpy(orig, L.orig.data(), (size_t)L.nGroups * 4 * sizeof(uint32_t));
    std::memcpy(bounds, L.tree.data(), (size_t)L.nGroups * sizeof(float4));
    return RT_OK;
}

int rt_unit_grid_rows(const float* segments, const int32_t* iu, uint32_t n, int32_t nv, int32_t* out_rows, float* out_s_enter) {
    if (!segments || !iu || !out_rows || nv <= 0) return Fail(RT_ERR_INVALID_ARG, "rt_unit_grid_rows: invalid argument");
    for (uint32_t k = 0; k < n; ++k) {
        const float* q = segments + 5 * (size_t)k;
        float slope, invAbsDu, sEnter;
        rtd::grid_segment_slope(q[0], q[1], q[2], q[3], slope, invAbsDu);
        int r0, r1;
        rtd::grid_slab_rows(q[0], q[1], q[2], q[3], q[4], slope, invAbsDu, (int)iu[k], (int)nv, r0, r1, sEnter);
        out_rows[2 * k] = r0;
        out_rows[2 * k + 1] = r1;
        if (out_s_enter) out_s_enter[k] = sEnter;
    }
    return RT_OK;
}

int rt_unit_layout_info(const rt_sphere* spheres, uint32_t n, uint32_t out[5]) {
    if (!spheres || n == 0 || !out) return Fail(RT_ERR_INVALID_ARG, "rt_unit_layout_info: invalid argument");
    SceneLayout L;
    BuildLayout(spheres, n, TreeTopFromEnv(), L);
    out[0] = L.gridOn ? 1u : (L.nLevels > 1 ? 2u : 0u);
    out[1] = L.gridOn ? L.gridNu : 0u;
    out[2] = L.gridOn ? L.gridNv : 0u;
    out[3] = L.nAlways;
    out[4] = L.nLevels;
    return RT_OK;
}

int rt_unit_tile_masks(rt_ctx* ctx, uint32_t W, uint32_t H, rt_rowset rs, uint32_t cap_tiles, uint32_t* n_tiles, uint32_t* words,
                       uint32_t cap_spheres, uint32_t* group_of_sphere, uint64_t scans[2]) {
    if (!ctx || !n_tiles || W == 0 || H == 0) return Fail(RT_ERR_INVALID_ARG, "rt_unit_tile_masks: invalid argument");
    if (!ctx->hasScene) return Fail(RT_ERR_NO_SCENE, "rt_unit_tile_masks: no scene uploaded");
    const uint32_t rows = RowsetLocalRows(rs);
    if (rows == 0 || (uint64_t)rs.first_row + rs.num_rows > H || (uint64_t)W * rows > (1ull << 31)) return Fail(RT_ERR_INVALID_ARG, "rt_unit_tile_masks: bad row set");
    RT_HIP(hipSetDevice(ctx->device));
    int rc;
    if ((rc = BuildTileMasks(ctx, W, H, rs, W * rows)) != RT_OK) return rc;
    *n_tiles = ctx->tileMaskValid ? ctx->maskTiles : 0u;
    RT_HIP(hipStreamSynchronize(ctx->stream));
    if (words && *n_tiles != 0u) {
        if (cap_tiles < *n_tiles) return Fail(RT_ERR_INVALID_ARG, "rt_unit_tile_masks: capacity too small");
        RT_HIP(hipMemcpy(words, ctx->tileMasks.ptr, (size_t)*n_tiles * rtd::kTileMaskWords * sizeof(uint32_t), hipMemcpyDeviceToHost));
    }
    if (group_of_sphere) {
        if (cap_spheres < ctx->n) return Fail(RT_ERR_INVALID_ARG, "rt_unit_tile_masks: sphere capacity too small");
        std::vector<uint32_t> orig(ctx->base.n_padded);
        RT_HIP(hipMemcpy(orig.data(), ctx->orig.ptr, orig.size() * sizeof(uint32_t), hipMemcpyDeviceToHost));
        for (uint32_t k = 0; k < ctx->n; ++k) group_of_sphere[k] = 0xffffffffu;
        for (uint32_t e = 0; e < (uint32_t)orig.size(); ++e)
            if (orig[e] < ctx->n) group_of_sphere[orig[e]] = e >> 2;
    }
    if (scans) {
        unsigned long long c[4] = {0, 0, 0, 0};
        RT_HIP(hipMemcpy(c, ctx->counters.ptr, sizeof(c), hipMemcpyDeviceToHost));
        scans[0] = ctx->freshScans;
        scans[1] = c[3];
    }
    return RT_OK;
}

int rt_unit_tile_masks_host(const rt_sphere* spheres, uint32_t n, const rt_camera* camera, uint32_t W, uint32_t H, rt_rowset rs, uint32_t limit,
                            uint32_t cap_tiles, uint32_t* n_tiles, uint32_t* words, uint32_t* group_of_sphere) {
    if (!spheres || n == 0 || !camera || !n_tiles || W == 0 || H == 0) return Fail(RT_ERR_INVALID_ARG, "rt_unit_tile_masks_host: invalid argument");
    const uint32_t rows = RowsetLocalRows(rs);
    if (rows == 0 || (uint64_t)rs.first_row + rs.num_rows > H || (uint64_t)W * rows > (1ull << 31)) return Fail(RT_ERR_INVALID_ARG, "rt_unit_tile_masks_host: bad row set");
    SceneLayout L;
    BuildLayout(spheres, n, TreeTopFromEnv(), L);
    const uint32_t nTop = L.levelCnt[L.nLevels - 1];
    const uint32_t nFull = (W * rows) >> 6;
    *n_tiles = (L.nLevels == 1 && !L.gridOn && nTop <= 128u) ? nFull : 0u;
    if (*n_tiles == 0u || !words) return RT_OK;
    if (cap_tiles < nFull) return Fail(RT_ERR_INVALID_ARG, "rt_unit_tile_masks_host: capacity too small");
    const rtd::TileMaskCam c = rtd::tile_mask_cam(camera->origin, camera->x, camera->y, camera->origin_image_plane, camera->aperture, camera->focal_length, W, H);
    for (uint32_t t = 0; t < nFull; ++t) {
        uint32_t* w = words + (size_t)rtd::kTileMaskWords * t;
        for (uint32_t k = 0; k < rtd::kTileMaskWords; ++k) w[k] = 0u;
        bool bad = false;
        uint32_t cnt = 0;
        for (uint32_t g = 0; g < nTop; ++g) {
            const float4 B = L.tree[L.levelOff[L.nLevels - 1] + g];
            const float b[4] = {B.x, B.y, B.z, B.w};
            const int r = rtd::tile_group_reached(c, rs, t, b);
            bad = bad || r < 0;
            if (r > 0) {
                uint32_t word, bit;
                rtd::tile_mask_slot(g, word, bit);
                w[word] |= bit;
                ++cnt;
            }
        }
        w[4] = rtd::tile_mask_flags(bad, cnt, limit);
        w[5] = cnt;
    }
    if (group_of_sphere) {
        for (uint32_t k = 0; k < n; ++k) group_of_sphere[k] = 0xffffffffu;
        for (uint32_t e = 0; e < (uint32_t)L.orig.size(); ++e)
            if (L.orig[e] < n) group_of_sphere[L.orig[e]] = e >> 2;
    }
    return RT_OK;
}

int rt_unit_tile_cone(const rt_camera* camera, uint32_t W, uint32_t H, uint32_t i0, uint32_t i1, uint32_t j, double out[9]) {
    if (!camera || !out || W == 0 || H == 0) return Fail(RT_ERR_INVALID_ARG, "rt_unit_tile_cone: invalid argument");
    const rtd::TileMaskCam c = rtd::tile_mask_cam(camera->origin, camera->x, camera->y, camera->origin_image_plane, camera->aperture, camera->focal_length, W, H);
    const rtd::TileCone t = rtd::tile_run_cone(c, i0, i1, j);
    for (int k = 0; k < 3; ++k) {
        out[k] = t.o[k];
        out[3 + k] = t.D[k];
    }
    out[6] = t.rhoL;
    out[7] = t.rhoF;
    out[8] = t.ok ? 1.0 : 0.0;
    return RT_OK;
}

#ifdef RT_TIMELINE
int rt_debug_timeline(rt_ctx* ctx, unsigned long long out[16]) {
    if (!ctx || !out) return Fail(RT_ERR_INVALID_ARG, "rt_debug_timeline: invalid argument");
    RT_HIP(hipSetDevice(ctx->device));
    RT_HIP(hipStreamSynchronize(ctx->stream));
    RT_HIP(hipMemcpyFromSymbol(out, HIP_SYMBOL(rtd::g_tl), 16 * sizeof(unsigned long long)));
    unsigned long long z[16] = {~0ull, 0, 0, 0, 0, 0, ~0ull, ~0ull, 0, 0, 0, 0, 0, 0, ~0ull, 0};
    RT_HIP(hipMemcpyToSymbol(HIP_SYMBOL(rtd::g_tl), z, sizeof(z)));
    return RT_OK;
}
int rt_debug_timeline_waves(rt_ctx* ctx, unsigned long long out[4096 * 8]) {
    if (!ctx || !out) return Fail(RT_ERR_INVALID_ARG, "rt_debug_timeline_waves: invalid argument");
    RT_HIP(hipSetDevice(ctx->device));
    RT_HIP(hipStreamSynchronize(ctx->stream));
    RT_HIP(hipMemcpyFromSymbol(out, HIP_SYMBOL(rtd::g_tlWave), 4096 * 8 * sizeof(unsigned long long)));
    return RT_OK;
}
int rt_debug_timeline_ring(rt_ctx* ctx, unsigned long long out[4096 * 16]) {
    if (!ctx || !out) return Fail(RT_ERR_INVALID_ARG, "rt_debug_timeline_ring: invalid argument");
    RT_HIP(hipSetDevice(ctx->device));
    RT_HIP(hipStreamSynchronize(ctx->stream));
    RT_HIP(hipMemcpyFromSymbol(out, HIP_SYMBOL(rtd::g_tlRing), 4096 * 16 * sizeof(unsigned long long)));
    return RT_OK;
}
int rt_debug_timeline_last(rt_ctx* ctx, unsigned int out[4096 * 4]) {
    if (!ctx || !out) return Fail(RT_ERR_INVALID_ARG, "rt_debug_timeline_last: invalid argument");
    RT_HIP(hipSetDevice(ctx->device));
    RT_HIP(hipStreamSynchronize(ctx->stream));
    RT_HIP(hipMemcpyFromSymbol(out, HIP_SYMBOL(rtd::g_tlLast), 4096 * 4 * sizeof(unsigned int)));
    return RT_OK;
}
int rt_debug_timeline_hist(rt_ctx* ctx, unsigned int out[1024]) {
    if (!ctx || !out) return Fail(RT_ERR_INVALID_ARG, "rt_debug_timeline_hist: invalid argument");
    RT_HIP(hipSetDevice(ctx->device));
    RT_HIP(hipStreamSynchronize(ctx->stream));
    RT_HIP(hipMemcpyFromSymbol(out, HIP_SYMBOL(rtd::g_tlHist), 1024 * sizeof(unsigned int)));
    static unsigned int zero[1024];
    RT_HIP(hipMemcpyToSymbol(HIP_SYMBOL(rtd::g_tlHist), zero, sizeof(zero)));
    return RT_OK;
}
#endif

#ifdef RT_STAMPS
int rt_debug_stamps(rt_ctx* ctx, unsigned long long out[20]) {
    if (!ctx || !out) return Fail(RT_ERR_INVALID_ARG, "rt_debug_stamps: invalid argument");
    RT_HIP(hipSetDevice(ctx->device));
    RT_HIP(hipStreamSynchronize(ctx->stream));
    RT_HIP(hipMemcpyFromSymbol(out, HIP_SYMBOL(rtd::g_dbg), 20 * sizeof(unsigned long long)));
    unsigned long long z[20] = {0};
    RT_HIP(hipMemcpyToSymbol(HIP_SYMBOL(rtd::g_dbg), z, sizeof(z)));
    return RT_OK;
}
#endif

#ifdef RT_PHASES
int rt_debug_sites(rt_ctx* ctx, unsigned long long* out, uint32_t cap, const char** names) {
    static const char* kNames =
#define RT_SITE_NAME(n) #n ","
        RT_SITE_LIST(RT_SITE_NAME)
#undef RT_SITE_NAME
        ;
    if (names) *names = kNames;
    if (!ctx || !out || cap < 2u * rtd::SITE_COUNT) return Fail(RT_ERR_INVALID_ARG, "rt_debug_sites: invalid argument");
    RT_HIP(hipSetDevice(ctx->device));
    RT_HIP(hipStreamSynchronize(ctx->stream));
    static unsigned long long raw[rtd::SITE_COUNT * 16];
    RT_HIP(hipMemcpyFromSymbol(raw, HIP_SYMBOL(rtd::g_sites), sizeof(raw)));
    for (uint32_t k = 0; k < rtd::SITE_COUNT; ++k) {
        out[2 * k] = raw[16 * k];
        out[2 * k + 1] = raw[16 * k + 1];
    }
    std::memset(raw, 0, sizeof(raw));
    RT_HIP(hipMemcpyToSymbol(HIP_SYMBOL(rtd::g_sites), raw, sizeof(raw)));
    return RT_OK;
}
#endif

}
```

### cpuraytracer_amd/csrc/rt_kernels.h

```cpp
#pragma once

#include "rt_params.h"
#include "rt_scan.h"
#include "rt_shade.h"
#include "rt_tile_mask.h"

namespace rtd {

enum : uint32_t { kIdle = 0u, kNeedClosest = 1u, kNeedShadow = 2u, kHaveHit = 3u };

constexpr uint32_t kStashDwords = 19;

RT_DEV void path_coordinates(const TraceParams& p, uint32_t q, uint32_t& i, uint32_t& j, uint32_t& s, uint32_t& slot) {
    if (p.path_list) {
        RT_SITE(K_PATHLIST);
        i = p.path_list[3 * q];
        j = p.path_list[3 * q + 1];
        s = p.path_list[3 * q + 2];
        slot = q;
    } else {
        const uint32_t tileSpan = 64u * p.spp_pass;
        const uint32_t nFull = p.npix_local >> 6;
        const uint32_t tileW = fastdiv(q, p.fd_tile);
        uint32_t pl, k;
// ... 397 lines not shown
                              : any_hit_all(scanTab, p.n_padded, pos, sunDir, aSun);
                    sh = occ ? v3(0.f, 0.f, 0.f) : shade_only(K, m, tex, pos, nrm, mt);
                } else {
                    const LightRec& Lk = p.extra_lights[k - 1u];
                    const V3 dirK = v3(Lk.sun_dir[0], Lk.sun_dir[1], Lk.sun_dir[2]);
                    const float aK = dot3(dirK, dirK);
                    occ = (Lk.sg_enabled && pp <= Lk.sg_p0sq)
                              ? shadow_query(Lk, scanTab, Lk.cell_start, Lk.entries, Lk.global, false, globSph, globIds, (const float4*)nullptr, pos, dirK, aK)
                              : any_hit_all(scanTab, p.n_padded, pos, dirK, aK);
                    sh = occ ? v3(0.f, 0.f, 0.f) : shade_only(Lk, m, tex, pos, nrm, mt);
                }
                ++nTrav;
                ++pathTrav;
                direct = direct + sh;
            }
            rad = rad + thr * (emitOnly + direct);
            if (cont) {
                thr = thr * atten;
                ro = pos;
                rd = nextDir;
                ++depth;
            } else {
                finished = true;
            }
            return;
        }
        const bool useIndex = K.sg_enabled && dot3(pos, pos) <= K.sg_p0sq;
        bool occluded = false;
        if (useIndex) occluded = shadow_query(K, scanTab, sgCell, sgEntries, sgGlobal, p.sg_glob16 != 0u, globSph, globIds, (!kLds && kScan >= 2) ? p.sg_sph : nullptr, pos, sunDir, aSun);
        RT_STAMP(th2);
        shade_value(K, m, tex, pos, nrm, !occluded, local, localOcc, mt);
        RT_STAMP(th3);
#ifdef RT_STAMPS
        thA = th0;
        thB = th3;
#endif
        RT_ACC(cyHit[0], th0, th1);
        RT_ACC(cyHit[1], th1, th2);
        RT_ACC(cyHit[2], th2, th3);
        if (useIndex) {
            RT_SITE(H_INDEXED);
            ++nTrav;
            ++pathTrav;
            if (!occluded) rad = rad + thr * local;
            else if (!scattered) rad = rad + thr * localOcc;
            if (cont) {
                thr = thr * atten;
                ro = pos;
                rd = nextDir;
                ++depth;
            } else {
                finished = true;
            }
        } else {
            RT_SITE(H_FARHIT);
            pend = thr * local;
            pathScattered = scattered;
            if (!scattered) nextDir = thr * localOcc;
            contAfterShadow = cont;
            thr = thr * atten;
            ro = pos;
            rd = sunDir;
            state = kNeedShadow;
        }
    };
    constexpr bool kPrim = kStash && kScan == 1;
    for (;;) {
        RT_SITE(K_ITER);
        RT_STAMP(ts0);
        uint32_t primTile = 0xffffffffu;
        uint64_t idleMask = __ballot(state == kIdle);
        if (kStash) {
            float* stash = reinterpret_cast<float*>(rayCache);
            const uint32_t cap = p.stash_cap;
            if (stashCnt != 0u && idleMask != 0ull) {
                RT_SITE(K_POP);
                const uint32_t nIdle = (uint32_t)__popcll(idleMask);
                const uint32_t n = stashCnt < nIdle ? stashCnt : nIdle;
                const uint32_t r = prefix_count(idleMask);
                if (state == kIdle && r < n) {
                    RT_SITE(K_POP_LANE);
                    const float* e = stash + (stashCnt - 1u - r);
                    ro = v3(e[0], e[cap], e[2u * cap]);
                    rd = v3(e[3u * cap], e[4u * cap], e[5u * cap]);
                    thr = v3(e[6u * cap], e[7u * cap], e[8u * cap]);
                    rad = v3(e[9u * cap], e[10u * cap], e[11u * cap]);
                    draws.rng = Rng{__float_as_uint(e[12u * cap]), __float_as_uint(e[13u * cap]), __float_as_uint(e[14u * cap]),
                                    __float_as_uint(e[15u * cap])};
                    q = __float_as_uint(e[16u * cap]);
                    depth = __float_as_uint(e[17u * cap]);
                    pathTrav = __float_as_uint(e[18u * cap]);
                    state = kHaveHit;
                }
                stashCnt -= n;
            }
            const uint64_t hitMask = __ballot(state == kHaveHit);
            const uint32_t nHit = (uint32_t)__popcll(hitMask);
            bool process = nHit > p.stash_process;
            if (!process && nHit != 0u && __ballot(state == kNeedClosest || state == kNeedShadow) == 0ull) {
                if (blkNext == blkEnd && !queueEmpty && !nextBlock()) queueEmpty = true;
                if (blkNext == blkEnd) {
                    process = true;
                } else {
                    RT_SITE(K_PUSH);
                    wave_lds_handoff();
                    if (state == kHaveHit) {
                        RT_SITE(K_PUSH_LANE);
                        float* e = stash + prefix_count(hitMask);
                        e[0] = ro.x; e[cap] = ro.y; e[2u * cap] = ro.z;
                        e[3u * cap] = rd.x; e[4u * cap] = rd.y; e[5u * cap] = rd.z;
                        e[6u * cap] = thr.x; e[7u * cap] = thr.y; e[8u * cap] = thr.z;
                        e[9u * cap] = rad.x; e[10u * cap] = rad.y; e[11u * cap] = rad.z;
                        e[12u * cap] = __uint_as_float(draws.rng.s0); e[13u * cap] = __uint_as_float(draws.rng.s1);
                        e[14u * cap] = __uint_as_float(draws.rng.s2); e[15u * cap] = __uint_as_float(draws.rng.s3);
                        e[16u * cap] = __uint_as_float(q);
                        e[17u * cap] = __uint_as_float(depth);
                        e[18u * cap] = __uint_as_float(pathTrav);
                        state = kIdle;
                    }
                    stashCnt = nHit;
                    wave_lds_handoff();
                }
            }
            if (process) {
                RT_SITE(K_PROCESS);
                bool finished = false;
                if (state == kHaveHit) {
                    const int hidx = (int)(depth >> 16);
                    depth &= 0xffffu;
                    state = kNeedClosest;
                    processHit(hidx, ro, finished);
                }
                if (finished) finishPath();
            }
            if (__ballot(state != kIdle) == 0ull) {
                if (blkNext == blkEnd && !queueEmpty && !nextBlock()) queueEmpty = true;
                if (blkNext != blkEnd) {
                    RT_SITE(K_GEN);
#ifdef RT_TIMELINE
                    if (blkNext % kBlk == 0u) {
                        tlLastClaim = __builtin_amdgcn_s_memrealtime();
                        ++tlBlocks;
                        tlLastBlock = blkNext / kBlk;
                    }
#endif
                    const uint32_t nGen = (blkEnd - blkNext) < (uint32_t)kWaveSize ? (blkEnd - blkNext) : (uint32_t)kWaveSize;
                    if (kPrim) {
                        if (p.tile_masks != nullptr && nGen == (uint32_t)kWaveSize && (blkNext & 63u) == 0u) {
                            RT_SITE(K_GEN_TILE);
                            const uint32_t tw = fastdiv(blkNext, p.fd_tile);
                            if (tw < (p.npix_local >> 6)) {
                                const uint32_t tile = (uint32_t)__builtin_amdgcn_readfirstlane((int)(p.tile_order ? p.tile_order[tw] : tw));
                                const uint32_t flags = (uint32_t)__builtin_amdgcn_readfirstlane((int)p.tile_masks[kTileMaskWords * tile + 4u]);
                                if (flags & 1u) primTile = tile;
                            }
                        }
                    }
                    if (lane < nGen) {
                        RT_SITE(K_GEN_LANE);
                        uint32_t i, j, sN;
                        path_coordinates(p, blkNext + lane, i, j, sN, q);
                        draws.rng = rng_seed(p.seed, j * p.W + i, sN);
                        gen_primary_ray(K, i, j, sN, ro, rd);
                        thr = v3(1.f, 1.f, 1.f);
                        rad = v3(0.f, 0.f, 0.f);
                        depth = 0;
                        pathTrav = 0;
                        state = kNeedClosest;
#ifdef RT_TIMELINE
                        tlBorn = (uint32_t)(__builtin_amdgcn_s_memrealtime() - tl0);
#endif
                    }
                    blkNext += nGen;
                }
            }
        } else if (kCache) {
            while (idleMask != 0ull) {
                if (cachePos == cacheCnt) {
                    if (queueEmpty) break;
                    if (blkNext == blkEnd && !nextBlock()) {
                        queueEmpty = true;
                        break;
                    }
#ifdef RT_TIMELINE
                    if (blkNext % kBlk == 0u) {
                        tlLastClaim = __builtin_amdgcn_s_memrealtime();
                        ++tlBlocks;
                        tlLastBlock = blkNext / kBlk;
#ifdef RT_TIMELINE_RING
                        if (!kCarry && gwave < 4096u && lane == 0)
                            g_tlRing[16u * gwave + (tlBlocks & 15u)] = ((tlLastClaim - tl0) << 24) | (unsigned long long)(__popcll(__ballot(state != kIdle)) & 127) << 17 | (tlLastBlock >> 3);
#endif
                    }
#endif
                    const uint32_t nGen = (blkEnd - blkNext) < (uint32_t)kWaveSize ? (blkEnd - blkNext) : (uint32_t)kWaveSize;
                    wave_lds_handoff();
                    if (lane < nGen) {
                        const uint32_t qn = blkNext + lane;
                        uint32_t i, j, s, slotn;
                        path_coordinates(p, qn, i, j, s, slotn);
                        const Rng g = rng_seed(p.seed, j * p.W + i, s);
                        V3 go, gd;
                        gen_primary_ray(K, i, j, s, go, gd);
                        float4* slot = rayCache + 3u * lane;
                        slot[0] = make_float4(go.x, go.y, go.z, gd.x);
                        slot[1] = make_float4(gd.y, gd.z, __uint_as_float(g.s0), __uint_as_float(g.s1));
                        slot[2] = make_float4(__uint_as_float(g.s2), __uint_as_float(g.s3), __uint_as_float(slotn), 0.f);
                    }
                    blkNext += nGen;
                    cacheCnt = nGen;
                    cachePos = 0;
                    wave_lds_handoff();
                }
                const uint32_t avail = cacheCnt - cachePos;
                const uint32_t want = (uint32_t)__popcll(idleMask);
                const uint32_t rank = prefix_count(idleMask);
                if (state == kIdle && rank < avail) {
                    const float4* slot = rayCache + 3u * (cachePos + rank);
                    const float4 A = slot[0], B = slot[1], C = slot[2];
                    ro = v3(A.x, A.y, A.z);
                    rd = v3(A.w, B.x, B.y);
                    draws.rng = Rng{__float_as_uint(B.z), __float_as_uint(B.w), __float_as_uint(C.x), __float_as_uint(C.y)};
                    q = __float_as_uint(C.z);
                    thr = v3(1.f, 1.f, 1.f);
                    rad = v3(0.f, 0.f, 0.f);
                    depth = 0;
                    pathTrav = 0;
                    if (kCarry) seq8 = p.region_seq & 255u;
                    state = kNeedClosest;
#ifdef RT_TIMELINE
                    tlBorn = (uint32_t)(__builtin_amdgcn_s_memrealtime() - tl0);
#endif
                }
                cachePos += want < avail ? want : avail;
                idleMask = __ballot(state == kIdle);
            }
        } else {
            while (idleMask != 0ull && !queueEmpty) {
                if (blkNext == blkEnd) {
                    uint32_t shardUnused = 0;
                    if (!claim_block(p, ldsK, lane, kBlk, blkNext, blkEnd, shardUnused)) {
                        queueEmpty = true;
                        break;
                    }
                }
                const uint32_t avail = blkEnd - blkNext;
                const uint32_t want = (uint32_t)__popcll(idleMask);
                const uint32_t rank = prefix_count(idleMask);
                if (state == kIdle && rank < avail) {
                    uint32_t i, j, s;
                    path_coordinates(p, blkNext + rank, i, j, s, q);
                    draws.rng = rng_seed(p.seed, j * p.W + i, s);
                    gen_primary_ray(K, i, j, s, ro, rd);
                    thr = v3(1.f, 1.f, 1.f);
                    rad = v3(0.f, 0.f, 0.f);
                    depth = 0;
                    pathTrav = 0;
                    state = kNeedClosest;
                }
                blkNext += want < avail ? want : avail;
                idleMask = __ballot(state == kIdle);
            }
        }
        if (__ballot(state != kIdle) == 0ull) {
            if (kStash && stashCnt != 0u) continue;
            break;
        }
#ifdef RT_TIMELINE
        ++tlIters;
        if (queueEmpty && cachePos == cacheCnt) {
            if (tlDrain == 0ull) tlDrain = __builtin_amdgcn_s_memrealtime();
            ++drainIters;
        }
#endif
        if (kCarry) {
            ++itersHere;
            const bool nothingToStart = queueEmpty && cachePos == cacheCnt && p.carry != 0u && itersHere >= p.min_iters;
            const bool carriable = state == kIdle || ((p.region_seq - seq8) & 255u) < p.max_carry_age;
            if (nothingToStart && __ballot(!carriable) == 0ull) {
                const uint64_t liveMask = __ballot(state != kIdle);
                carried = (uint32_t)__popcll(liveMask);
                uint32_t age1 = 0;
                if (state != kIdle) {
                    ContEntry* e = p.cont_out + ((size_t)gwave * kWaveSize + prefix_count(liveMask));
                    e->a = make_float4(ro.x, ro.y, ro.z, rd.x);
                    e->b = make_float4(rd.y, rd.z, thr.x, thr.y);
                    e->c = make_float4(thr.z, rad.x, rad.y, rad.z);
                    e->d = make_float4(__uint_as_float(draws.rng.s0), __uint_as_float(draws.rng.s1), __uint_as_float(draws.rng.s2),
                                       __uint_as_float(draws.rng.s3));
                    e->e = make_float4(__uint_as_float(q), __uint_as_float(depth), __uint_as_float(seq8), __uint_as_float(pathTrav));
                    e->f = make_float4(pend.x, pend.y, pend.z, nextDir.x);
                    e->g = make_float4(nextDir.y, nextDir.z, __uint_as_float(state | (contAfterShadow ? 4u : 0u) | (pathScattered ? 8u : 0u)), 0.f);
                    age1 = 1u + ((p.region_seq - seq8) & 255u);
                }
                for (int off = 32; off > 0; off >>= 1) {
                    const uint32_t o2 = (uint32_t)__shfl_xor((int)age1, off);
                    age1 = o2 > age1 ? o2 : age1;
                }
                if (lane == 0) atomicMax(&ldsK->exit_age_max, age1);
                break;
            }
        }

        RT_STAMP(ts1);
        float tmin = 0.f;
        int idx = -1;
        const bool live = kStash ? (state == kNeedClosest || state == kNeedShadow) : (state != kIdle);
        if (kMfma) {
            const uint32_t* tileMask = nullptr;
            if (kPrim && primTile != 0xffffffffu) {
                tileMask = p.tile_masks + kTileMaskWords * primTile;
                if (lane == 0) __hip_atomic_fetch_add(&ldsK->prim_masked, 1u, __ATOMIC_RELAXED, __HIP_MEMORY_SCOPE_WORKGROUP);
            }
            scan_list_mfma<kScan == 2, kPrim>(scanTab, leafTab, origTab, mfmaOps, nTiles, nTop, treeTab, p.level_off, p.n_levels, p.bound_norm, p.single_mask, p.n_always, p.tree_box_on ? p.tree_box : nullptr, ro, rd,
                                       live, tmin, idx, waveCand, lane, dbgScan, tileMask);
        } else if (kScan == 3) {
            const GridParams G{gridCells, p.grid_nu, p.grid_nv, p.grid_ax_u, p.grid_ax_v, p.grid_g0u, p.grid_g0v, p.grid_inv_h, p.grid_rmax_over_h, p.grid_big_norm};
            const GridQuant Q{gridQ, p.grid_q[0], p.grid_q[1], p.grid_q[2], p.grid_q[3], p.grid_q[4], p.grid_q[5], p.grid_q[6], p.grid_q[7]};
            scan_list_grid<kGridQ>(scanTab, leafTab, origTab, G, gridCells, p.n_always, p.tree_box, p.bound_norm, ro, rd, live, tmin, idx, waveCand, lane, Q);
        } else if (live) {
            scan_list_deferred(scanTab, origTab, p.n_padded, ro, rd, tmin, idx, cand);
        }
        if (live) {
            ++nTrav;
            ++pathTrav;
        }

        RT_STAMP(ts2);
        bool finished = false;
#ifdef RT_STAMPS
        thA = 0;
        thB = 0;
#endif
        if (state == kNeedClosest) {
            ++nSeg;
            if (idx < 0) {
                RT_SITE(K_TRANS_MISS);
                const V3 sky = v3(K.sky_emit[0], K.sky_emit[1], K.sky_emit[2]);
                rad = rad + thr * sky;
                finished = true;
            } else if (kStash) {
                RT_SITE(K_TRANS_HIT);
                ro = tmin * rd + ro;
                depth |= (uint32_t)idx << 16;
                state = kHaveHit;
            } else {
                processHit(idx, tmin * rd + ro, finished);
            }
        } else if (state == kNeedShadow) {
            RT_SITE(K_TRANS_SHADOW);
            if (idx < 0) rad = rad + pend;
            else if (!pathScattered) rad = rad + nextDir;
            if (contAfterShadow) {
                rd = nextDir;
                ++depth;
                state = kNeedClosest;
            } else {
                finished = true;
            }
        }
        if (finished) finishPath();
        RT_STAMP(ts3);
#ifdef RT_STAMPS
        if (thA != 0) {
            cyHit[3] += thA - ts2;
            cyHit[4] += ts3 - thB;
            cyHit[5] += 1;
        }
#endif
        RT_ACC(cyRefill, ts0, ts1);
        RT_ACC(cyScan, ts1, ts2);
        RT_ACC(cyTrans, ts2, ts3);
#ifdef RT_STAMPS
        cyIters += 1;
#endif
    }

    if (kCarry) {
        if (lane == 0) {
            p.cont_out_n[gwave] = carried;
            const uint32_t ticket = atomicAdd(&ldsK->exit_ticket, 1u);
            if (ticket == (uint32_t)(kThreads / kWaveSize) - 1u) {
                const uint32_t m = atomicMax(&ldsK->exit_age_max, 0u);
                if (m != 0u) atomicMin(&p.ctl->oldest_open, p.region_seq - (m - 1u));
            }
        }
    }
#ifdef RT_TIMELINE
    if (lane == 0) {
        const unsigned long long tl2 = __builtin_amdgcn_s_memrealtime();
        if (gwave < 4096u) {
            unsigned long long* w = g_tlWave + 8u * gwave;
            w[0] = tl0; w[1] = kCarry ? tl1 : (tlDrain != 0ull ? tlDrain : tl2); w[2] = tl2; w[3] = tlBlocks; w[4] = kCarry ? carried : tlLastBlock;
            w[5] = kCarry ? ((tlLastClaim - tl0) << 8 | (unsigned long long)tlCarriedIn) : tlLastClaim; w[6] = tlIters; w[7] = drainIters;
        }
    }
#endif
    unsigned long long t = nTrav, s = nSeg;
    for (int off = 32; off > 0; off >>= 1) {
        t += __shfl_down(t, off);
        s += __shfl_down(s, off);
    }
#ifdef RT_STAMPS
    {
        unsigned long long it = dbgScan[2];
        for (int off = 32; off > 0; off >>= 1) it += __shfl_down(it, off);
        if (lane == 0) atomicAdd(&g_dbg[6], it);
    }
#endif
    if (lane == 0) {
        atomicAdd(&p.counters[0], t);
        atomicAdd(&p.counters[1], s);
        if (kPrim && p.tile_masks != nullptr) {
            const uint32_t ticket = __hip_atomic_fetch_add(&ldsK->exit_ticket, 1u, __ATOMIC_ACQ_REL, __HIP_MEMORY_SCOPE_WORKGROUP);
            if (ticket == (uint32_t)(kThreads / kWaveSize) - 1u)
                atomicAdd(&p.counters[3], (unsigned long long)__hip_atomic_load(&ldsK->prim_masked, __ATOMIC_RELAXED, __HIP_MEMORY_SCOPE_WORKGROUP));
        }
#ifdef RT_STAMPS
        atomicAdd(&g_dbg[0], cyRefill);
        atomicAdd(&g_dbg[1], cyScan);
        atomicAdd(&g_dbg[2], cyTrans);
        atomicAdd(&g_dbg[3], cyIters);
        atomicAdd(&g_dbg[4], dbgScan[0]);
        atomicAdd(&g_dbg[5], dbgScan[1]);
        atomicAdd(&g_dbg[7], dbgScan[3]);
        atomicAdd(&g_dbg[8], dbgScan[4]);
        atomicAdd(&g_dbg[9], dbgScan[5]);
        atomicAdd(&g_dbg[10], dbgScan[6]);
        atomicAdd(&g_dbg[11], dbgScan[7]);
        atomicAdd(&g_dbg[12], cyHit[0]);
        atomicAdd(&g_dbg[13], cyHit[1]);
        atomicAdd(&g_dbg[14], cyHit[2]);
        atomicAdd(&g_dbg[15], cyHit[3]);
        atomicAdd(&g_dbg[16], cyHit[4]);
        atomicAdd(&g_dbg[17], cyHit[5]);
#endif
    }
}

template <bool kLds, int kThreads, int kScan, bool kCache, bool kHitLds = false, bool kCarry = false, bool kStash = false, bool kMatsL2 = false,
          bool kSgLds = false, bool kGridQ = false>
__global__ void __launch_bounds__(kThreads, 1) rt_trace_kernel(const TraceParams p) {
    trace_body<false, kLds, kThreads, kScan, kCache, kHitLds, kCarry, kStash, kMatsL2, kSgLds, kGridQ>(p);
}
template <bool kLds, int kThreads, int kScan, bool kCache, bool kHitLds = false, bool kCarry = false, bool kStash = false, bool kMatsL2 = false,
          bool kSgLds = false, bool kGridQ = false>
__global__ void __launch_bounds__(kThreads, 1) rt_trace_kernel_lights(const TraceParams p) {
    trace_body<true, kLds, kThreads, kScan, kCache, kHitLds, kCarry, kStash, kMatsL2, kSgLds, kGridQ>(p);
}

__global__ void __launch_bounds__(256) rt_raygen_tables_kernel(float2* jitter, uint32_t s0, uint32_t nJitter, float2* lens, uint32_t k0,
                                                               uint32_t nLens, uint32_t sampler, uint32_t* shardHeads = nullptr,
                                                               FrameCtl* ctl = nullptr) {
    const uint32_t k = blockIdx.x * blockDim.x + threadIdx.x;
    if (shardHeads && k < kQueueShards) shardHeads[kShardStrideWords * k] = 0u;
    if (ctl && k == 0) ctl->oldest_open = 0xffffffffu;
    if (k < nJitter) jitter[k] = make_float2(halton(s0 + k, 2), halton(s0 + k, 3));
    if (k < nLens) {
        float lx, ly;
        halton_disk_4_5(k0 + k, lx, ly, sampler);
        lens[k] = make_float2(lx, ly);
    }
}

#ifndef RT_PILOTS_PER_TILE
#define RT_PILOTS_PER_TILE 3
#endif
constexpr uint32_t kPilotsPerTile = RT_PILOTS_PER_TILE;
__global__ void __launch_bounds__(256) rt_pilot_rays_kernel(const TraceParams p, uint32_t nFull, float* rays) {
    const uint32_t t = blockIdx.x * blockDim.x + threadIdx.x;
    if (t >= nFull * kPilotsPerTile) return;
    const uint32_t tile = t / kPilotsPerTile, which = t - tile * kPilotsPerTile;
    const uint32_t pl = (tile << 6) + (which * 63u + (kPilotsPerTile - 1u) / 2u) / (kPilotsPerTile - 1u);
    const uint32_t lr = pl / p.W;
    V3 o, d;
    gen_primary_ray(p, pl - lr * p.W, rowset_global_row(p.rs, lr), 1u, o, d);
    float* w = rays + 6 * (size_t)t;
    w[0] = o.x; w[1] = o.y; w[2] = o.z; w[3] = d.x; w[4] = d.y; w[5] = d.z;
}
RT_DEV uint32_t pilot_class(const float* hits, uint32_t t, const uint32_t* matTypeByOrig) {
    uint32_t c = 0;
    for (uint32_t k = 0; k < kPilotsPerTile; ++k) {
        const int oidx = __float_as_int(hits[10 * ((size_t)t * kPilotsPerTile + k) + 1]);
        if (oidx >= 0) {
            const uint32_t ty = matTypeByOrig[oidx];
            const uint32_t ck = ty == RT_MAT_DIELECTRIC_TRANSPARENT ? 3u : (ty == RT_MAT_METAL ? 2u : 1u);
            c = ck > c ? ck : c;
        }
    }
    return c;
}
__global__ void __launch_bounds__(256) rt_tile_class_kernel(const float* hits, uint32_t nFull, uint32_t W, const uint32_t* matTypeByOrig,
                                                            uint8_t* cls) {
    const uint32_t t = blockIdx.x * blockDim.x + threadIdx.x;
    if (t >= nFull) return;
    uint32_t c = pilot_class(hits, t, matTypeByOrig);
    if (c != 3u) {
        const int64_t first = (int64_t)t << 6;
        const int64_t near[6] = {first - 64, first + 64, first - (int64_t)W, first - (int64_t)W + 63, first + (int64_t)W, first + (int64_t)W + 63};
        for (int k = 0; k < 6; ++k) {
            const int64_t n = near[k] >> 6;
            if (near[k] >= 0 && n < (int64_t)nFull && pilot_class(hits, (uint32_t)n, matTypeByOrig) == 3u) c = 3u;
        }
    }
    cls[t] = (uint8_t)c;
}
__global__ void __launch_bounds__(1024) rt_tile_order_kernel(const uint8_t* cls, uint32_t nFull, uint32_t* order) {
    __shared__ uint32_t waveTot[16][4];
    const uint32_t tid = threadIdx.x, lane = tid & 63u, w = tid >> 6;
    const uint32_t per = (nFull + 1023u) / 1024u;
    const uint32_t t0 = tid * per < nFull ? tid * per : nFull, t1 = (t0 + per) < nFull ? (t0 + per) : nFull;
    uint32_t cnt[4] = {0u, 0u, 0u, 0u};
    for (uint32_t t = t0; t < t1; ++t) {
        const uint32_t c = cls[t];
        for (uint32_t k = 0; k < 4u; ++k) cnt[k] += c == k ? 1u : 0u;
    }
    uint32_t pos[4];
    for (uint32_t k = 0; k < 4u; ++k) {
        uint32_t incl = cnt[k];
        for (int off = 1; off < 64; off <<= 1) {
            const uint32_t v = (uint32_t)__shfl_up((int)incl, off);
            if ((int)lane >= off) incl += v;
        }
        if (lane == 63u) waveTot[w][k] = incl;
        pos[k] = incl - cnt[k];
    }
    __syncthreads();
    uint32_t base = 0;
    for (int k = 3; k >= 0; --k) {
        uint32_t before = 0, tot = 0;
        for (uint32_t v = 0; v < 16u; ++v) {
            before += v < w ? waveTot[v][k] : 0u;
            tot += waveTot[v][k];
        }
        pos[k] += base + before;
        base += tot;
    }
    for (uint32_t t = t0; t < t1; ++t) {
        const uint32_t c = cls[t];
        uint32_t at = 0;
        for (uint32_t k = 0; k < 4u; ++k) {
            at = c == k ? pos[k] : at;
            pos[k] += c == k ? 1u : 0u;
        }
        order[at] = t;
    }
}

static_assert(kTileMaskPerRay == 2.0 * (double)kMarginRel, "the masks bound the filter's own per-ray margin");
__global__ void __launch_bounds__(256) rt_tile_mask_kernel(const TraceParams p, uint32_t nFull, uint32_t limit, uint32_t* __restrict__ words) {
    const uint32_t tile = blockIdx.x * 4u + (threadIdx.x >> 6), lane = threadIdx.x & 63u;
    if (tile >= nFull) return;
    RT_SITE(T_MASK);
    const TileMaskCam c = tile_mask_cam(p.cam_o, p.cam_x, p.cam_y, p.cam_oip, p.aperture, p.focal, p.W, p.H);
    const uint32_t topLevel = p.n_levels - 1u;
    const uint32_t nTop = p.level_cnt[topLevel];
    const float4* bounds = p.tree + p.level_off[topLevel];
    int r0 = 0, r1 = 0;
    if (lane < nTop) {
        const float4 B = bounds[lane];
        const float b[4] = {B.x, B.y, B.z, B.w};
        r0 = tile_group_reached(c, p.rs, tile, b);
    }
    if (lane + 64u < nTop && nTop <= 128u) {
        const float4 B = bounds[lane + 64u];
        const float b[4] = {B.x, B.y, B.z, B.w};
        r1 = tile_group_reached(c, p.rs, tile, b);
    }
    const uint64_t m0 = __ballot(r0 > 0), m1 = __ballot(r1 > 0);
    const bool bad = __ballot(r0 < 0 || r1 < 0) != 0ull || nTop > 128u;
    if (lane == 0) {
        auto wordA = [](uint64_t m) { return __builtin_bitreverse32((uint32_t)m & 0xffffu) | (__builtin_bitreverse32((uint32_t)(m >> 32) & 0xffffu) >> 16); };
        auto wordB = [](uint64_t m) { return __builtin_bitreverse32((uint32_t)(m >> 16) & 0xffffu) | (__builtin_bitreverse32((uint32_t)(m >> 48) & 0xffffu) >> 16); };
        const uint32_t cnt = (uint32_t)(__popcll(m0) + __popcll(m1));
        uint4* w = reinterpret_cast<uint4*>(words + (size_t)kTileMaskWords * tile);
        w[0] = make_uint4(wordA(m0), wordA(m1), wordB(m0), wordB(m1));
        w[1] = make_uint4(tile_mask_flags(bad, cnt, limit), cnt, 0u, 0u);
    }
}

__global__ void __launch_bounds__(256) rt_accumulate_kernel(const float* __restrict__ samples, float* __restrict__ hdr, uint32_t npix,
                                                            uint32_t spp, uint32_t first = 0, uint32_t count = 0xffffffffu) {
    const uint32_t pix = blockIdx.x * blockDim.x + threadIdx.x;
    if (pix >= npix) return;
    float r = hdr[3 * (size_t)pix], g = hdr[3 * (size_t)pix + 1], b = hdr[3 * (size_t)pix + 2];
    const uint32_t nFull = npix >> 6, tile = pix >> 6;
    const uint32_t stride = tile < nFull ? 64u : npix - (nFull << 6);
    const float3* sp = reinterpret_cast<const float3*>(samples) + (size_t)tile * 64u * spp + (pix - (tile << 6));
    uint32_t s = first < spp ? first : spp;
    const uint32_t end = count > spp - s ? spp : s + count;
    for (; s + 8 <= end; s += 8) {
        float3 v[8];
#pragma unroll
        for (int k = 0; k < 8; ++k) v[k] = sp[(size_t)(s + k) * stride];
#pragma unroll
        for (int k = 0; k < 8; ++k) {
            r += v[k].x;
            g += v[k].y;
            b += v[k].z;
        }
    }
    for (; s < end; ++s) {
        const float3 v = sp[(size_t)s * stride];
        r += v.x;
        g += v.y;
        b += v.z;
    }
    hdr[3 * (size_t)pix] = r;
    hdr[3 * (size_t)pix + 1] = g;
    hdr[3 * (size_t)pix + 2] = b;
}

struct RegionTable {
    uint32_t seq[kMaxFramesInFlight];
    uint32_t spp[kMaxFramesInFlight];
};
__global__ void __launch_bounds__(256) rt_commit_kernel(const float* __restrict__ ring, float* __restrict__ hdr, uint32_t npix,
                                                        uint32_t regionEntries, uint32_t nRing, RegionTable rt, FrameCtl* ctl,
                                                        uint32_t newestSeq, uint32_t commitNo) {
    const uint32_t committed = ctl->committed_seq[commitNo & 1u], open = ctl->oldest_open;
    uint32_t limit = newestSeq;
    if (open != 0xffffffffu && open - 1u < limit) limit = open - 1u;
    if (limit < committed) limit = committed;
    if (blockIdx.x == 0 && threadIdx.x == 0) {
        uint32_t add = 0;
        for (uint32_t q = committed + 1u; q <= limit; ++q) add += rt.spp[q % nRing];
        ctl->committed_seq[(commitNo + 1u) & 1u] = limit;
        ctl->committed_samples[(commitNo + 1u) & 1u] = ctl->committed_samples[commitNo & 1u] + add;
    }
    if (limit == committed) return;
    for (uint32_t pix = blockIdx.x * blockDim.x + threadIdx.x; pix < npix; pix += gridDim.x * blockDim.x) {
        float r = hdr[3 * (size_t)pix], g = hdr[3 * (size_t)pix + 1], b = hdr[3 * (size_t)pix + 2];
        const uint32_t nFull = npix >> 6, tile = pix >> 6;
        const uint32_t stride = tile < nFull ? 64u : npix - (nFull << 6);
        for (uint32_t q = committed + 1u; q <= limit; ++q) {
            const uint32_t slot = q % nRing, spp = rt.spp[slot];
            const float3* sp = reinterpret_cast<const float3*>(ring) + (size_t)slot * regionEntries + (size_t)tile * 64u * spp + (pix - (tile << 6));
            for (uint32_t s = 0; s < spp; ++s) {
                const float3 v = sp[(size_t)s * stride];
                r += v.x;
                g += v.y;
                b += v.z;
            }
        }
        hdr[3 * (size_t)pix] = r;
        hdr[3 * (size_t)pix + 1] = g;
        hdr[3 * (size_t)pix + 2] = b;
    }
}

RT_DEV float tonemap_channel(float h, float n) {
    const float a = 2.51f, b = 0.03f, c = 2.43f, d = 0.59f, e = 0.14f;
    float color = h / n;
    color = sat1((color * (a * color + b)) / (color * (c * color + d) + e));
    color = rt_powf(color, 1 / 2.2f);
    return color;
}
__global__ void __launch_bounds__(256) rt_resolve_kernel(const float* __restrict__ hdr, uint8_t* __restrict__ ldr, uint32_t npix,
                                                         uint32_t nSamples, const uint32_t* committedSamples = nullptr) {
    const uint32_t pix = blockIdx.x * blockDim.x + threadIdx.x;
    if (pix >= npix) return;
    if (committedSamples) nSamples = *committedSamples > 0u ? *committedSamples : 1u;
    const float n = (float)nSamples;
    for (int ch = 0; ch < 3; ++ch) ldr[3 * (size_t)pix + ch] = (uint8_t)rne_u8(tonemap_channel(hdr[3 * (size_t)pix + ch], n));
}

__global__ void k_unit_halton(const uint32_t* index, uint32_t base, uint32_t n, float* out) {
    const uint32_t k = blockIdx.x * blockDim.x + threadIdx.x;
    if (k < n) out[k] = halton(index[k], base);
}
__global__ void k_unit_math(uint32_t op, const float* x, const float* y, uint32_t n, float* out) {
    const uint32_t k = blockIdx.x * blockDim.x + threadIdx.x;
    if (k >= n) return;
    float r = 0.f;
    if (op == 0) r = rt_sinf(x[k]);
    else if (op == 1) r = rt_cosf(x[k]);
    else if (op == 2) r = rt_powf(x[k], y[k]);
    else if (op == 3) r = rt_tanf(x[k]);
#if RT_MARKSTEIN
    else if (op == 4) r = recip_rn(x[k]);
    else if (op == 5) {
        const V3 q = div3(v3(x[k], 0.f, -x[k]), y[k]);
        r = q.x;
    }
#else
    else if (op == 4) r = 1.0f / x[k];
    else if (op == 5) r = x[k] / y[k];
#endif
    else if (op == 6) r = x[k] / y[k];
    else if (op == 7) r = sqrt_rn(x[k]);
#if RT_FAST_SQRT
    else if (op == 8) r = sqrt_rn_core(x[k]);
#else
    else if (op == 8) r = __builtin_sqrtf(x[k]);
#endif
    else if (op == 9) r = __builtin_sqrtf(x[k]);
    out[k] = r;
}
__global__ void k_unit_primary(const TraceParams p, const uint32_t* ijs, uint32_t n, float* out) {
    const uint32_t k = blockIdx.x * blockDim.x + threadIdx.x;
    if (k >= n) return;
    V3 o, d;
    gen_primary_ray(p, ijs[3 * k], ijs[3 * k + 1], ijs[3 * k + 2], o, d);
    float* w = out + 6 * (size_t)k;
    w[0] = o.x; w[1] = o.y; w[2] = o.z; w[3] = d.x; w[4] = d.y; w[5] = d.z;
}
template <bool kLds, int kScan>
__global__ void __launch_bounds__(256) k_unit_closest(const TraceParams p, const float* rays, uint32_t n, float* out) {
    extern __shared__ float4 smem[];
    constexpr uint32_t kWaveRegion = wave_region_bytes<kScan>();
    uint16_t* candBase = reinterpret_cast<uint16_t*>(smem);
    float4* tabBase = smem + (256 / kWaveSize) * (kWaveRegion / 16);
    SceneTabs T;
    stage_scene<kLds, kScan>(p, tabBase, T);
    __syncthreads();
    const uint32_t lane = threadIdx.x & (kWaveSize - 1);
    uint16_t* waveCand = candBase + (threadIdx.x / kWaveSize) * (kWaveRegion / 2);
    const uint32_t k = blockIdx.x * blockDim.x + threadIdx.x;
    const bool live = k < n;
    V3 o = v3(0.f, 0.f, 0.f), d = v3(0.f, 0.f, 1.f);
    if (live) {
        const float* r = rays + 6 * (size_t)k;
        o = v3(r[0], r[1], r[2]);
        d = v3(r[3], r[4], r[5]);
    }
    float tmin = 0.f;
    int idx = -1;
    unsigned long long dbg[8] = {0, 0, 0, 0, 0, 0, 0, 0};
    (void)dbg;
    if (kScan == 3) {
// ... 57 lines not shown
```

### cpuraytracer_amd/csrc/rt_params.h

```cpp
#pragma once

#include <hip/hip_runtime.h>
#include <stdint.h>

#include "../../include/rt_api.h"
#include "rt_device_math.h"

namespace rtd {


#ifdef RT_STAMPS
static __device__ unsigned long long g_dbg[20];
RT_DEV unsigned long long rt_stamp() {
    unsigned long long t;
    __builtin_amdgcn_sched_barrier(0);
    asm volatile("s_memtime %0\n\ts_waitcnt lgkmcnt(0)" : "=s"(t)::"memory");
    __builtin_amdgcn_sched_barrier(0);
    return t;
}
#define RT_STAMP(var) const unsigned long long var = rt_stamp()
#define RT_ACC(sum, a, b) sum += (b) - (a)
#else
#define RT_STAMP(var)
#define RT_ACC(sum, a, b)
#endif

#ifdef RT_TIMELINE
static __device__ unsigned long long g_tl[16];
static __device__ unsigned long long g_tlRing[4096 * 16];
static __device__ unsigned int g_tlLast[4096 * 4];
static __device__ unsigned long long g_tlWave[4096 * 8];
static __device__ unsigned int g_tlHist[1024];
#endif

constexpr int kWaveSize = 64;
constexpr uint32_t kMaxLevels = 6;
constexpr uint32_t kQueueBlock = 128;
constexpr uint32_t kCarryQueueBlock = 128;

constexpr uint32_t kQueueShards = 8;
#ifndef RT_SHARD_STRIDE_WORDS
#define RT_SHARD_STRIDE_WORDS 32
#endif
constexpr uint32_t kShardStrideWords = RT_SHARD_STRIDE_WORDS;

struct FastDiv {
    uint32_t m, sh;
};
RT_DEV FastDiv make_fastdiv(uint32_t d) {
    uint32_t l = 0;
    while (l < 32u && (1ull << l) < (unsigned long long)d) ++l;
    FastDiv f;
    f.m = (uint32_t)((((1ull << l) - (unsigned long long)d) << 32) / (unsigned long long)d + 1ull);
    f.sh = (l < 1u ? l : 1u) | ((l > 0u ? l - 1u : 0u) << 8);
    return f;
}
RT_DEV uint32_t fastdiv(uint32_t n, FastDiv f) {
#if defined(__HIP_DEVICE_COMPILE__)
    const uint32_t t = __umulhi(f.m, n);
#else
    const uint32_t t = (uint32_t)(((unsigned long long)f.m * (unsigned long long)n) >> 32);
#endif
    return (t + ((n - t) >> (f.sh & 255u))) >> (f.sh >> 8);
}

struct ContEntry {
    float4 a, b, c, d, e;
    float4 f, g;
};
struct FrameCtl {
    uint32_t oldest_open;
    uint32_t committed_seq[2];
    uint32_t committed_samples[2];
};
constexpr uint32_t kMaxFramesInFlight = 16;
RT_DEV uint32_t sg_glob_slots(uint32_t nGlobal) { return nGlobal ? nGlobal + (nGlobal * 2u + 15u) / 16u : 0u; }

struct LightRec {
    float sun_dir[3], sun_rad[3];
    float cam_o[3];
    float sg_e1[3], sg_e2[3], sg_u0, sg_v0, sg_inv_cell, sg_p0sq;
    uint32_t sg_nx, sg_ny, sg_nglobal, sg_enabled;
    const uint16_t *cell_start, *entries, *global;
};

struct TraceParams {
    const float4* scan;
    const uint32_t* orig;
    const float4* leaf;
    const float4* tree;
    uint32_t level_off[kMaxLevels], level_cnt[kMaxLevels];
    uint32_t n_levels;
    uint32_t tree_in_lds;
    const float* radius;
    const rt_material* mats;
    const uint4* mats16;
    uint32_t mats16_mode;
    uint32_t n;
    uint32_t n_groups;
    uint32_t mats_in_lds;
    float bound_norm;
    unsigned long long single_mask[2];
    float tree_box[9];
    uint32_t tree_box_on;
    uint32_t n_always;
    uint32_t n_padded;
    const uint16_t* grid_cell_start;
    uint32_t grid_nu, grid_nv, grid_ax_u, grid_ax_v, grid_in_lds;
    float grid_g0u, grid_g0v, grid_inv_h, grid_rmax_over_h, grid_big_norm;
    const uint32_t* grid_qrec;
    float grid_q[8];
    const uint16_t* sg_cell_start;
    const uint16_t* sg_entries;
    const uint16_t* sg_global;
    const float4* sg_sph;
    uint32_t sg_nx, sg_ny, sg_nglobal, sg_nentries, sg_enabled, sg_in_lds;
    uint32_t sg_glob16;
    float sg_e1[3], sg_e2[3], sg_u0, sg_v0, sg_inv_cell, sg_p0sq;
    float cam_o[3], cam_x[3], cam_y[3], cam_oip[3];
    float aperture, focal;
    float sun_dir[3], sun_rad[3];
    uint32_t n_lights;
    const LightRec* extra_lights;
    float sky_emit[3];
    float exposure;
    uint32_t W, H;
    rt_rowset rs;
    uint32_t s0;
    uint32_t spp_pass;
    uint32_t total_paths;
    uint32_t npix_local;
    uint32_t max_depth;
    uint32_t sampler;
    uint64_t seed;
    const uint32_t* path_list;
    const uint32_t* tile_order;
    const float2* jitter_tab;
    const float2* lens_tab;
    uint32_t lens_k0;
    float* samples;
    uint32_t* trav_out;
    FrameCtl* ctl;
    const ContEntry* cont_in;
    const uint32_t* cont_in_n;
    ContEntry* cont_out;
    uint32_t* cont_out_n;
    uint32_t carry;
    uint32_t region_seq;
    uint32_t max_carry_age;
    uint32_t min_iters;
    uint32_t queue_block;
    uint32_t static_blocks;
    uint32_t dyn_begin, dyn_blocks;
    uint32_t sample_base;
    FastDiv fd_tile, fd_w, fd_rows;
    uint32_t ray_cache_off16;
    uint32_t ray_cache_stride16;
    uint32_t stash_cap;
    uint32_t stash_process;
    uint32_t* shard_heads;
    unsigned long long* counters;
    const uint32_t* tile_masks;
};

struct SceneConsts {
    float cam_o[3], cam_x[3], cam_y[3], cam_oip[3];
    float aperture, focal;
    float sun_dir[3], sun_rad[3];
    float sky_emit[3];
    float exposure;
    float sg_e1[3], sg_e2[3], sg_u0, sg_v0, sg_inv_cell, sg_p0sq;
    uint32_t sg_nx, sg_ny, sg_nglobal, sg_enabled;
    uint32_t W, H, s0, lens_k0;
    uint32_t sampler;
    const float2* jitter_tab;
    const float2* lens_tab;
    uint32_t exit_age_max;
    uint32_t exit_ticket;
    uint32_t dry_mask;
    uint32_t prim_masked;
};
constexpr uint32_t kSceneConstBytes = 256;
constexpr uint32_t kConstBytes = kSceneConstBytes + 8 * 256;
static_assert(sizeof(SceneConsts) <= kSceneConstBytes, "SceneConsts must fit its LDS slot");
static_assert(kMathTabWords <= 256, "math tables must fit their LDS slot");
RT_DEV void fill_consts(const TraceParams& p, SceneConsts& k) {
    for (int i = 0; i < 3; ++i) {
        k.cam_o[i] = p.cam_o[i]; k.cam_x[i] = p.cam_x[i]; k.cam_y[i] = p.cam_y[i]; k.cam_oip[i] = p.cam_oip[i];
        k.sun_dir[i] = p.sun_dir[i]; k.sun_rad[i] = p.sun_rad[i]; k.sky_emit[i] = p.sky_emit[i];
        k.sg_e1[i] = p.sg_e1[i]; k.sg_e2[i] = p.sg_e2[i];
    }
    k.aperture = p.aperture; k.focal = p.focal; k.exposure = p.exposure;
    k.sg_u0 = p.sg_u0; k.sg_v0 = p.sg_v0; k.sg_inv_cell = p.sg_inv_cell; k.sg_p0sq = p.sg_p0sq;
    k.sg_nx = p.sg_nx; k.sg_ny = p.sg_ny; k.sg_nglobal = p.sg_nglobal; k.sg_enabled = p.sg_enabled;
    k.W = p.W; k.H = p.H; k.s0 = p.s0; k.lens_k0 = p.lens_k0; k.sampler = p.sampler;
    k.jitter_tab = p.jitter_tab; k.lens_tab = p.lens_tab;
    k.exit_age_max = 0u; k.exit_ticket = 0u; k.dry_mask = 0u; k.prim_masked = 0u;
}

RT_DEV uint32_t rowset_global_row(const rt_rowset& rs, uint32_t lr, FastDiv byBlockRows) {
    const uint32_t lb = fastdiv(lr, byBlockRows);
    const uint32_t k = lr - lb * rs.block_rows;
    return rs.first_row + (lb * rs.nshards + rs.shard) * rs.block_rows + k;
}
RT_DEV uint32_t rowset_global_row(const rt_rowset& rs, uint32_t lr) {
    const uint32_t lb = lr / rs.block_rows;
    const uint32_t k = lr - lb * rs.block_rows;
    return rs.first_row + (lb * rs.nshards + rs.shard) * rs.block_rows + k;
}

template <class P>
RT_DEV void camera_get_ray(const P& p, float uvx, float uvy, float lensx, float lensy, V3& origin, V3& dir) {
    const V3 camO = v3(p.cam_o[0], p.cam_o[1], p.cam_o[2]);
    const V3 mx = v3(p.cam_x[0], p.cam_x[1], p.cam_x[2]);
    const V3 my = v3(p.cam_y[0], p.cam_y[1], p.cam_y[2]);
    const V3 oip = v3(p.cam_oip[0], p.cam_oip[1], p.cam_oip[2]);
    const float ndcx = 2.f * uvx - 1.f;
    const float ndcy = -2.f * uvy + 1.f;
    const V3 pp = (oip + ndcx * mx) + ndcy * my;
    const V3 focalPoint = camO + p.focal * normalize3(pp - camO);
    const float rdx = (0.5f * p.aperture) * lensx;
    const float rdy = (0.5f * p.aperture) * lensy;
    origin = (camO + rdx * mx) + rdy * my;
    dir = normalize3(focalPoint - origin);
}

RT_DEV void halton_disk_4_5(uint32_t k, float& lensx, float& lensy, uint32_t sampler = 0u) {
    const float theta = (2.f * 3.141592654f) * halton(k, 4);
    float r = halton(k, 5);
    if (sampler & RT_SAMPLER_SQRT_DISK) r = sqrt_rn(r);
    double sn, cs;
    sincos_f64(theta, sn, cs);
    lensx = r * (float)cs;
    lensy = r * (float)sn;
}
template <class P>
RT_DEV void gen_primary_ray(const P& p, uint32_t i, uint32_t j, uint32_t s, V3& origin, V3& dir) {
    const float xsize = (float)p.W;
    const float ysize = (float)p.H;
    float jx, jy, lensx, lensy;
    const uint32_t li = s + i + j;
    if (p.jitter_tab) {
        typedef const float __attribute__((address_space(1)))* GlobalF;
        const GlobalF jt = (GlobalF)(p.jitter_tab + (s - p.s0));
        const GlobalF lt = (GlobalF)(p.lens_tab + (li - p.lens_k0));
        jx = jt[0]; jy = jt[1]; lensx = lt[0]; lensy = lt[1];
    } else {
        RT_SITE(P_HALTON);
        jx = halton(s, 2);
        jy = halton(s, 3);
        halton_disk_4_5(li, lensx, lensy, p.sampler);
    }
    const float uvx = ((float)(int)i + jx) / xsize;
    const float uvy = ((float)(int)j + jy) / ysize;

    camera_get_ray(p, uvx, uvy, lensx, lensy, origin, dir);
}


}
```

### cpuraytracer_amd/csrc/rt_scan.h

```cpp
#pragma once

#include "rt_params.h"

namespace rtd {

constexpr uint32_t kScanGroup = 4;

RT_DEV void root_test(float disc, float b, float a, uint32_t i, const uint32_t* __restrict__ orig, float& tmin, int& idx) {
    if (disc > 0.f) {
        const float sq = sqrt_rn(disc);
        float t = (-b - sq) / a;
        if (!(t > 0.001f)) t = (-b + sq) / a;
        if (t > 0.001f && (t < tmin || (t == tmin && idx >= 0 && orig[i] < orig[idx]))) {
            tmin = t;
            idx = (int)i;
        }
    }
}

RT_DEV void scan_list(const float4* __restrict__ tab, const uint32_t* __restrict__ orig, uint32_t nEntries, V3 o, V3 d, float& tmin,
                      int& idx) {
    const float a = dot3(d, d);
    tmin = __builtin_inff();
    idx = -1;
// ... 168 lines not shown
    return __builtin_bit_cast(uint32_t, __builtin_convertvector(v, bf16x2));
}
RT_DEV void split_group_value(float v, uint32_t& hh, uint32_t& ll) {
    hh = bf16_pair_bits(v, v);
    const float rem = v - __uint_as_float(hh & 0xffff0000u);
    ll = bf16_pair_bits(rem, rem);
}
RT_DEV uint32_t split_ray_value(float v) {
    const uint32_t hh = bf16_pair_bits(v, v);
    const float rem = v - __uint_as_float(hh & 0xffff0000u);
    return bf16_pair_bits(v, rem);
}

RT_DEV uint32_t mfma_tiles_for(uint32_t nTop) { return (((nTop + 31u) / 32u) + 1u) & ~1u; }
RT_DEV void build_mfma_operands(const float4* __restrict__ bounds, uint32_t nGroups, uint32_t nTiles, float* __restrict__ ops, uint32_t tid,
                                uint32_t nthreads) {
    uint32_t* img = reinterpret_cast<uint32_t*>(ops);
    for (uint32_t e = tid; e < nTiles * 64; e += nthreads) {
        const uint32_t t = e >> 6, l = e & 63, h = l >> 5, R = l & 31u;
        const uint32_t gi = t * 32 + 16u * ((R >> 2) & 1u) + (R & 3u) + 4u * (R >> 3);
        float4 B = make_float4(0.f, 0.f, 0.f, 1e30f);
        if (gi < nGroups) B = bounds[gi];
        uint32_t* o = img + (size_t)t * kOpsPerTile + l;
        split_group_value(h == 0 ? -B.x : -B.z, o[0], o[64]);
        split_group_value(h == 0 ? -B.y : 1.f, o[128], o[192]);
        uint32_t y0hh, y0ll, y1hh, y1ll;
        split_group_value(h == 0 ? B.x : B.z, y0hh, y0ll);
        split_group_value(h == 0 ? B.y : B.w, y1hh, y1ll);
        o[256] = y0hh;
        o[320] = (y0ll & 0xffffu) | (y1hh << 16);
        o[384] = (y1hh & 0xffffu) | (y1ll << 16);
        o[448] = h == 0 ? 0x3f803f80u : 0u;
    }
}

#ifndef RT_FILTER_SQRT_RAW
#define RT_FILTER_SQRT_RAW 1
#endif
RT_DEV float filter_sqrt_up(float x) {
#if RT_FILTER_SQRT_RAW && defined(__HIP_DEVICE_COMPILE__)
    return __builtin_amdgcn_sqrtf(__builtin_fmaxf(x, 1e-30f)) * 1.000001f;
#else
    return __builtin_sqrtf(x);
#endif
}

#ifndef RT_EXACT_MARKSTEIN
#define RT_EXACT_MARKSTEIN 1
#endif
RT_DEV float pooled_root(float b, float sq, float ra) {
#if RT_MARKSTEIN && RT_EXACT_MARKSTEIN
    const bool ok = (__float_as_uint(ra) - 0x36000000u) <= 0x3b800000u && (__builtin_fabsf(b) + sq) < 0x1p100f;
    if (__builtin_expect(__ballot(!ok) == 0ull, 1)) {
        const float ya = recip_rn(ra);
        float t = div_rn(-b - sq, ra, ya);
        if (!(t > 0.001f)) t = div_rn(-b + sq, ra, ya);
        return t;
    }
#endif
    {
        RT_SITE(M_ROOT_SLOW);
        float t = (-b - sq) / ra;
        if (!(t > 0.001f)) t = (-b + sq) / ra;
        return t;
    }
}

RT_DEV float min_with_positive(float x, float p) {
    const int xi = __float_as_int(x), pi = __float_as_int(p);
    return __int_as_float(xi < pi ? xi : pi);
}

#ifndef RT_PK_POST
#define RT_PK_POST 0
#endif
RT_DEV void mfma_post(const f32x16& Tb, const f32x16& Tg, float bthr, uint32_t& rejectedBits) {
#if RT_PK_POST
#pragma unroll
    for (int e = 0; e < 16; e += 2) {
        const f32x2 m = {min_with_positive(Tb[e], bthr), min_with_positive(Tb[e + 1], bthr)};
        const f32x2 b = {Tb[e], Tb[e + 1]};
        const f32x2 t = {Tg[e], Tg[e + 1]};
        const f32x2 g = __builtin_elementwise_fma(m, b, -t);
        rejectedBits = __builtin_amdgcn_alignbit(rejectedBits, __float_as_uint(g[0]), 31);
        rejectedBits = __builtin_amdgcn_alignbit(rejectedBits, __float_as_uint(g[1]), 31);
    }
    return;
#endif
#pragma unroll
    for (int e = 0; e < 16; ++e) {
        const float t = Tg[e];
        const float g = __builtin_fmaf(min_with_positive(Tb[e], bthr), Tb[e], -t);
        rejectedBits = __builtin_amdgcn_alignbit(rejectedBits, __float_as_uint(g), 31);
    }
}

RT_DEV int bound_rejected(const float4 B, V3 g, V3 d, float a, float dO, float cr, float bt) {
    const float b = __builtin_fmaf(-d.z, B.z, __builtin_fmaf(-d.y, B.y, __builtin_fmaf(-d.x, B.x, dO)));
    const float t = __builtin_fmaf(g.z, B.z, __builtin_fmaf(g.y, B.y, __builtin_fmaf(g.x, B.x, __builtin_fmaf(a, B.w, cr))));
    return __float_as_int(__builtin_fmaf(min_with_positive(b, bt), b, -t));
}

RT_DEV int bound_rejected_far(const float4 B, V3 g, V3 d, float a, float dO, float cr, float bt, float u) {
    const float b = __builtin_fmaf(-d.z, B.z, __builtin_fmaf(-d.y, B.y, __builtin_fmaf(-d.x, B.x, dO)));
    const float t = __builtin_fmaf(g.z, B.z, __builtin_fmaf(g.y, B.y, __builtin_fmaf(g.x, B.x, __builtin_fmaf(a, B.w, cr))));
    const float dec = __builtin_fmaf(min_with_positive(b, bt), b, -t);
    const float bu = b + u;
    const float fo = __builtin_fmaf(u, b + bu, t);
    return (bu < -bt && fo > 0.f) ? -1 : __float_as_int(dec);
}

RT_DEV int bound_rejected_span(const float4 B, V3 g, V3 d, float a, float dO, float cr, float bt, float un, float uf) {
    const float b = __builtin_fmaf(-d.z, B.z, __builtin_fmaf(-d.y, B.y, __builtin_fmaf(-d.x, B.x, dO)));
    const float t = __builtin_fmaf(g.z, B.z, __builtin_fmaf(g.y, B.y, __builtin_fmaf(g.x, B.x, __builtin_fmaf(a, B.w, cr))));
    const float dec = __builtin_fmaf(min_with_positive(b, bt), b, -t);
    const float bf = b + uf;
    const float ff = __builtin_fmaf(uf, b + bf, t);
    const float bn = b + un;
    const float fn = __builtin_fmaf(un, b + bn, t);
    return ((bf < -bt && ff > 0.f) || (bn > bt && fn > 0.f)) ? -1 : __float_as_int(dec);
}

RT_DEV void wave_lds_handoff() {
    __builtin_amdgcn_fence(__ATOMIC_RELEASE, "wavefront");
    __builtin_amdgcn_wave_barrier();
    __builtin_amdgcn_fence(__ATOMIC_ACQUIRE, "wavefront");
}

RT_DEV uint32_t prefix_count(uint64_t mask) {
    return __builtin_amdgcn_mbcnt_hi((uint32_t)(mask >> 32), __builtin_amdgcn_mbcnt_lo((uint32_t)mask, 0u));
}
RT_DEV uint32_t wave_inclusive_sum(uint32_t v) {
    v += (uint32_t)__builtin_amdgcn_update_dpp(0, (int)v, 0x111, 0xf, 0xf, false);
    v += (uint32_t)__builtin_amdgcn_update_dpp(0, (int)v, 0x112, 0xf, 0xf, false);
    v += (uint32_t)__builtin_amdgcn_update_dpp(0, (int)v, 0x114, 0xf, 0xf, false);
    v += (uint32_t)__builtin_amdgcn_update_dpp(0, (int)v, 0x118, 0xf, 0xf, false);
    v += (uint32_t)__builtin_amdgcn_update_dpp(0, (int)v, 0x142, 0xa, 0xf, false);
    v += (uint32_t)__builtin_amdgcn_update_dpp(0, (int)v, 0x143, 0xc, 0xf, false);
    return v;
}
RT_DEV float lane_fetch(uint32_t src, float v) { return __int_as_float(__builtin_amdgcn_ds_bpermute((int)(src << 2), __float_as_int(v))); }

RT_DEV bool next_candidate(unsigned long long& cur, unsigned long long& nxt, uint32_t& hOff, uint32_t& gid) {
    if (cur == 0ull) {
        cur = nxt;
        nxt = 0ull;
        hOff = 16u;
    }
    if (cur == 0ull) return false;
    const uint32_t N = (uint32_t)__builtin_clzll(cur);
    cur &= ~(0x8000000000000000ull >> N);
    gid = hOff + N + (N & 48u);
    return true;
}

template <bool kTree, bool kPrim = false>
RT_DEV void scan_list_mfma(const float4* __restrict__ tab, const float4* __restrict__ leaf, const uint32_t* __restrict__ orig,
                           const float* __restrict__ ops, uint32_t nTiles,
                           uint32_t nTop, const float4* __restrict__ tree, const uint32_t* levelOff, uint32_t nLevels, float boundNorm,
                           const unsigned long long* singleMask, uint32_t nAlways, const float* treeBox, V3 o, V3 d, bool live, float& tmin, int& idx, uint16_t* waveCand, uint32_t lane, unsigned long long* dbg,
                           const uint32_t* tileMask = nullptr) {
    static_assert(!kPrim || !kTree, "tile masks belong to the flat scan");
    RT_SITE(S_SCAN);
    const float a = dot3(d, d);
    tmin = __builtin_inff();
    idx = -1;
    const float dO = dot3(d, o);
    const float m2a = -2.f * a;
    const float gx = m2a * o.x, gy = m2a * o.y, gz = m2a * o.z;
    const float oo = dot3(o, o);
    const float cr = live ? (a * oo) * (1.f - 2.f * kMarginRel) : 1e30f;
    const float crLeaf = (a * oo) * (1.f - 2.f * kMarginKLeaf * 5.9604645e-8f);
    const float bt = 1e-4f * filter_sqrt_up(a) * (filter_sqrt_up(oo) + boundNorm);
    unsigned long long cur, nxt;
    RT_STAMP(tf0);
    if (kPrim && tileMask != nullptr) {
        RT_SITE(S_MASKED);
        const uint4 m = *reinterpret_cast<const uint4*>(tileMask);
        cur = live ? (((unsigned long long)m.x << 32) | (unsigned long long)m.y) : 0ull;
        nxt = live ? (((unsigned long long)m.z << 32) | (unsigned long long)m.w) : 0ull;
    } else {
    uint32_t b01x = split_ray_value(d.x), b01y = split_ray_value(d.y), b23x = split_ray_value(d.z), b23y = split_ray_value(dO);
    const uint32_t sgx = split_ray_value(gx), sgy = split_ray_value(gy), sgz = split_ray_value(gz), sga = split_ray_value(a);
    uint32_t g01a = sgx, g01b = __builtin_amdgcn_perm(sgy, sgx, 0x05040100u), g01c = __builtin_amdgcn_alignbit(sgy, sgy, 16);
    uint32_t g23a = sgz, g23b = __builtin_amdgcn_perm(sga, sgz, 0x05040100u), g23c = __builtin_amdgcn_alignbit(sga, sga, 16);
    uint32_t cr0 = __float_as_uint(cr), cr1 = cr0, bt0 = __float_as_uint(bt), bt1 = bt0;
#define RT_SWAP32(A, B)                                                        \
    {                                                                          \
        const auto r_ = __builtin_amdgcn_permlane32_swap((A), (B), false, false); \
        (A) = r_[0];                                                           \
        (B) = r_[1];                                                           \
    }
    RT_SWAP32(b01x, b23x)
    RT_SWAP32(b01y, b23y)
    RT_SWAP32(g01a, g23a)
    RT_SWAP32(g01b, g23b)
    RT_SWAP32(g01c, g23c)
    RT_SWAP32(cr0, cr1)
    RT_SWAP32(bt0, bt1)
#undef RT_SWAP32
    const bf16x8 Bb0 = __builtin_bit_cast(bf16x8, (u32x4){b01x, b01x, b01y, b01y});
    const bf16x8 Bb1 = __builtin_bit_cast(bf16x8, (u32x4){b23x, b23x, b23y, b23y});
    const bf16x8 Bg0 = __builtin_bit_cast(bf16x8, (u32x4){g01a, g01b, g01c, split_ray_value(__uint_as_float(cr0))});
    const bf16x8 Bg1 = __builtin_bit_cast(bf16x8, (u32x4){g23a, g23b, g23c, split_ray_value(__uint_as_float(cr1))});
    const float btT0 = __uint_as_float(bt0), btT1 = __uint_as_float(bt1);
    const uint32_t* opsImg = reinterpret_cast<const uint32_t*>(ops);
    uint32_t w0a = 0xffffffffu, w1a = 0xffffffffu, w0b = 0xffffffffu, w1b = 0xffffffffu;
    for (uint32_t sp = 0; sp < nTiles; sp += 2) {
        RT_SITE(S_TILEPAIR);
        uint32_t r0 = 0u, r1 = 0u;
#pragma unroll
        for (uint32_t k = 0; k < 2; ++k) {
            const uint32_t* op = opsImg + (size_t)(sp + k) * kOpsPerTile + lane;
            const bf16x8 Ab = __builtin_bit_cast(bf16x8, (u32x4){op[0], op[64], op[128], op[192]});
            const bf16x8 Ag = __builtin_bit_cast(bf16x8, (u32x4){op[256], op[320], op[384], op[448]});
            const f32x16 zero = {0.f, 0.f, 0.f, 0.f, 0.f, 0.f, 0.f, 0.f, 0.f, 0.f, 0.f, 0.f, 0.f, 0.f, 0.f, 0.f};
            {
                const f32x16 Tb = __builtin_amdgcn_mfma_f32_32x32x16_bf16(Ab, Bb0, zero, 0, 0, 0);
                const f32x16 Tg = __builtin_amdgcn_mfma_f32_32x32x16_bf16(Ag, Bg0, zero, 0, 0, 0);
                mfma_post(Tb, Tg, btT0, r0);
            }
            {
                const f32x16 Tb = __builtin_amdgcn_mfma_f32_32x32x16_bf16(Ab, Bb1, zero, 0, 0, 0);
                const f32x16 Tg = __builtin_amdgcn_mfma_f32_32x32x16_bf16(Ag, Bg1, zero, 0, 0, 0);
                mfma_post(Tb, Tg, btT1, r1);
            }
        }
        if (sp == 0u) {
            w0a = r0;
            w1a = r1;
        } else {
            w0b = r0;
            w1b = r1;
        }
    }
    {
        const auto ra = __builtin_amdgcn_permlane32_swap(w0a, w1a, false, false);
        const auto rb = __builtin_amdgcn_permlane32_swap(w0b, w1b, false, false);
        w0a = ra[0]; w1a = ra[1]; w0b = rb[0]; w1b = rb[1];
    }
    cur = ~(((unsigned long long)w0a << 32) | (unsigned long long)w0b);
    nxt = ~(((unsigned long long)w1a << 32) | (unsigned long long)w1b);
    }
    RT_STAMP(tf1);
    uint32_t hOff = 0u;
#ifdef RT_STAMPS
    const uint32_t tot = (uint32_t)(__popcll(cur) + __popcll(nxt));
#endif
    if (!kTree) {
        uint16_t* poolA = waveCand;
        uint16_t* poolB = waveCand + kPoolA;
        unsigned long long* best = reinterpret_cast<unsigned long long*>(waveCand + kPoolA + kPoolB);
        best[lane] = ~0ull;
        wave_lds_handoff();
        uint32_t cntB = 0;
#if RT_LIST_WORDS
        uint32_t cw0 = (uint32_t)(cur >> 32), cw1 = (uint32_t)cur, cw2 = (uint32_t)(nxt >> 32), cw3 = (uint32_t)nxt;
        auto pushWord = [&](uint32_t w, uint32_t tagBase, uint32_t scale, uint16_t*& wp) __attribute__((always_inline)) {
            while (w != 0u) {
                RT_SITE(S_PUSH_WORD);
                const uint32_t N = (uint32_t)__builtin_clz(w);
                w ^= 0x80000000u >> N;
                *wp++ = (uint16_t)(tagBase + scale * (N + (N & 16u)));
            }
        };
        {
            const uint32_t s0 = cw0 & (uint32_t)(singleMask[0] >> 32), s1 = cw1 & (uint32_t)singleMask[0];
            const uint32_t s2 = cw2 & (uint32_t)(singleMask[1] >> 32), s3 = cw3 & (uint32_t)singleMask[1];
            const uint32_t nS = (uint32_t)(__builtin_popcount(s0) + __builtin_popcount(s1) + __builtin_popcount(s2) + __builtin_popcount(s3));
            const uint32_t inclS = wave_inclusive_sum(nS);
            const uint32_t totalS = (uint32_t)__builtin_amdgcn_readlane((int)inclS, 63);
            if (totalS != 0u && totalS <= kPoolB - 4u * kWaveSize) {
                RT_SITE(S_SINGLE);
                cw0 ^= s0; cw1 ^= s1; cw2 ^= s2; cw3 ^= s3;
                uint16_t* wp = poolB + (inclS - nS);
                const uint32_t tag = lane << 10;
                pushWord(s0, tag, 4u, wp);
                pushWord(s1, tag + 4u * 64u, 4u, wp);
                pushWord(s2, tag + 4u * 16u, 4u, wp);
                pushWord(s3, tag + 4u * 80u, 4u, wp);
                cntB = totalS;
            }
        }
        const uint32_t nMine = (uint32_t)(__builtin_popcount(cw0) + __builtin_popcount(cw1) + __builtin_popcount(cw2) + __builtin_popcount(cw3));
        bool pending = nMine != 0u;
#else
        {
            const unsigned long long sCur = cur & singleMask[0], sNxt = nxt & singleMask[1];
            const uint32_t nS = (uint32_t)(__popcll(sCur) + __popcll(sNxt));
            const uint32_t inclS = wave_inclusive_sum(nS);
            const uint32_t totalS = (uint32_t)__builtin_amdgcn_readlane((int)inclS, 63);
            if (totalS != 0u && totalS <= kPoolB - 4u * kWaveSize) {
                RT_SITE(S_SINGLE);
                cur &= ~sCur;
                nxt &= ~sNxt;
                uint16_t* wp = poolB + (inclS - nS);
                const uint32_t tag = lane << 10;
                unsigned long long m0 = sCur, m1 = sNxt;
                while (m0 != 0ull) {
                    RT_SITE(S_SINGLE_PUSH0);
                    const uint32_t N = (uint32_t)__builtin_clzll(m0);
                    m0 &= ~(0x8000000000000000ull >> N);
                    *wp++ = (uint16_t)(tag | (4u * (N + (N & 48u))));
                }
                while (m1 != 0ull) {
                    RT_SITE(S_SINGLE_PUSH1);
// ... 727 lines not shown
```

### cpuraytracer_amd/csrc/rt_sites.h

```cpp
#pragma once
#include <stdint.h>

namespace rtd {
#define RT_SITE_LIST(X) \
    X(K_WAVE) X(K_ITER) X(K_PATHLIST) X(K_PARTIAL) X(P_HALTON) X(M_DIV_SLOW) X(M_SQRT_SLOW) X(M_ROOT_SLOW) X(K_POP) X(K_POP_LANE) X(K_PUSH) \
    X(K_PUSH_LANE) X(K_PROCESS) X(K_GEN) X(K_GEN_LANE) X(K_NEXTBLOCK) X(K_CLAIM) X(K_TRANS_MISS) X(K_TRANS_HIT) \
    X(K_TRANS_SHADOW) X(K_FINISH) X(H_PROCESS) X(H_MAT16) X(H_MULTI) X(H_SCATTER) X(H_SHADEV) X(H_TRANSPARENT) X(H_METAL) X(H_OPAQUE) \
    X(H_OPAQUE_DIFFUSE) X(H_SHADOWQ) X(H_SQ_WALK) X(H_SQ_CONSIDER) X(H_SQ_GROUND) X(H_SQ_GTAIL) X(H_SQ_ROUND) X(H_SQ_TAIL1) X(H_SQ_CELL) \
    X(H_SQ_ROOTS) X(H_SQ_FULL) X(H_SHADE) X(H_INDEXED) X(H_FARHIT) X(S_SCAN) X(S_TILEPAIR) X(S_SINGLE) \
    X(S_SINGLE_PUSH0) X(S_SINGLE_PUSH1) X(S_PASS) X(S_TAKE) X(S_PUSH_WORD) X(S_TAKE_PUSH0) X(S_TAKE_PUSH1) X(S_ASTEP) X(S_ASTEP2) X(S_APUSH) X(S_DRAIN) X(S_BSTEP) X(S_BSTEP2) X(S_BMIN) \
    X(G_SCAN) X(G_DRAIN) X(G_BSTEP) X(G_BMIN) X(G_BIG) X(G_BIGPUSH) X(G_FEED) X(G_FEED_LANE) X(G_ROUND) X(G_STEP) X(G_PUSH) \
    X(K_GEN_TILE) X(S_MASKED) X(T_MASK)
enum RtSite : uint32_t {
#define RT_SITE_ENUM(n) SITE_##n,
    RT_SITE_LIST(RT_SITE_ENUM)
#undef RT_SITE_ENUM
    SITE_COUNT
};
#if defined(RT_PHASES) && defined(__HIPCC__)
static __device__ unsigned long long g_sites[SITE_COUNT * 16];
__device__ __forceinline__ void rt_site(uint32_t id) {
    const unsigned long long m = __ballot(1);
    if ((threadIdx.x & 63u) == (uint32_t)__ffsll(m) - 1u) {
        atomicAdd(&g_sites[id * 16u], 1ull);
        atomicAdd(&g_sites[id * 16u + 1u], (unsigned long long)__popcll(m));
    }
}
#define RT_SITE(n) rtd::rt_site(rtd::SITE_##n)
#else
#define RT_SITE(n)
#endif

}
```

### cpuraytracer_amd/csrc/rt_tile_mask.h

```cpp
#pragma once

#include <stdint.h>

#include "../../include/rt_api.h"
#include "rt_device_math.h"

namespace rtd {

constexpr uint32_t kTileMaskWords = 8;
constexpr uint32_t kTileMaskLimitDefault = 16;
constexpr double kTileMaskPerRay = 2.0 * 4096.0 * 5.9604644775390625e-8;

struct TileMaskCam {
    float cam_o[3], cam_x[3], cam_y[3], cam_oip[3];
    float aperture, focal;
    uint32_t W, H;
};

template <class A>
RT_DEV TileMaskCam tile_mask_cam(const A& o, const A& x, const A& y, const A& oip, float aperture, float focal, uint32_t W, uint32_t H) {
    TileMaskCam c;
    for (int k = 0; k < 3; ++k) {
        c.cam_o[k] = o[k]; c.cam_x[k] = x[k]; c.cam_y[k] = y[k]; c.cam_oip[k] = oip[k];
    }
    c.aperture = aperture; c.focal = focal; c.W = W; c.H = H;
    return c;
}
RT_DEV uint32_t tile_mask_flags(bool bad, uint32_t candidates, uint32_t limit) { return (!bad && candidates <= limit) ? 1u : 0u; }

struct TileCone {
    double o[3], D[3];
    double rhoL, rhoF, normO;
    bool ok;
};

RT_DEV double tm_len3(const double v[3]) { return __builtin_sqrt(v[0] * v[0] + v[1] * v[1] + v[2] * v[2]); }

RT_DEV bool tm_focal_offset(const TileMaskCam& c, double uvx, double uvy, double out[3]) {
    const double ndcx = 2.0 * uvx - 1.0, ndcy = -2.0 * uvy + 1.0;
    double v[3];
    for (int k = 0; k < 3; ++k) v[k] = ((double)c.cam_oip[k] + ndcx * (double)c.cam_x[k] + ndcy * (double)c.cam_y[k]) - (double)c.cam_o[k];
    const double l = tm_len3(v);
    if (!(l > 0.0) || !(l < 1e300)) return false;
    for (int k = 0; k < 3; ++k) out[k] = (double)c.focal * v[k] / l;
    return true;
}

RT_DEV TileCone tile_run_cone(const TileMaskCam& c, uint32_t i0, uint32_t i1, uint32_t j) {
    TileCone t;
    t.ok = false;
    t.rhoL = t.rhoF = t.normO = 0.0;
    for (int k = 0; k < 3; ++k) t.o[k] = t.D[k] = 0.0;
    const double W = (double)c.W, H = (double)c.H;
    const double mx[3] = {(double)c.cam_x[0], (double)c.cam_x[1], (double)c.cam_x[2]};
    const double my[3] = {(double)c.cam_y[0], (double)c.cam_y[1], (double)c.cam_y[2]};
    const double lx = tm_len3(mx), ly = tm_len3(my);
    if (!(c.focal > 0.f) || !(lx > 0.0) || !(ly > 0.0) || !(W > 0.0) || !(H > 0.0)) return t;
    const double u0 = ((double)i0 - 1.0) / W, u1 = ((double)i1 + 2.0) / W;
    const double v0 = ((double)j - 1.0) / H, v1 = ((double)j + 2.0) / H;
    if (!tm_focal_offset(c, 0.5 * (u0 + u1), 0.5 * (v0 + v1), t.D)) return t;
    double rho = 0.0;
    for (int q = 0; q < 4; ++q) {
        double f[3];
        if (!tm_focal_offset(c, (q & 1) ? u1 : u0, (q & 2) ? v1 : v0, f)) return t;
        if (!(f[0] * t.D[0] + f[1] * t.D[1] + f[2] * t.D[2] > 0.0)) return t;
        const double d[3] = {f[0] - t.D[0], f[1] - t.D[1], f[2] - t.D[2]};
        const double l = tm_len3(d);
        if (!(l <= rho)) rho = l;
    }
    const double ap = c.aperture < 0.f ? -(double)c.aperture : (double)c.aperture;
    t.rhoL = 0.5 * ap * (lx > ly ? lx : ly) * 1.4142135623730951;
    t.rhoF = rho;
    for (int k = 0; k < 3; ++k) t.o[k] = (double)c.cam_o[k];
    t.normO = tm_len3(t.o);
    t.ok = t.rhoL == t.rhoL && t.rhoF == t.rhoF && t.rhoL < 1e300 && t.rhoF < 1e300 && t.normO < 1e300;
    return t;
}

RT_DEV double tile_cone_reach(const TileCone& t, double lambda) { return (lambda < 1.0 ? 1.0 - lambda : lambda - 1.0) * t.rhoL + lambda * t.rhoF; }

RT_DEV bool tm_piece_reached(double DD, double wD, double ww, double alpha, double beta, double l0, double l1) {
    const double A2 = DD - beta * beta, B = wD + alpha * beta, C0 = ww - alpha * alpha;
    const double q0 = (A2 * l0 - 2.0 * B) * l0 + C0;
    if (!(q0 > 0.0)) return true;
    if (l1 >= 0.0) {
        const double q1 = (A2 * l1 - 2.0 * B) * l1 + C0;
        if (!(q1 > 0.0)) return true;
    } else if (!(A2 > 0.0)) {
        return true;
    }
    if (A2 > 0.0) {
        const double lv = B / A2;
        if (lv > l0 && (l1 < 0.0 || lv < l1)) {
            const double qv = C0 - B * lv;
            if (!(qv > 0.0)) return true;
        }
    }
    return false;
}

RT_DEV double tile_group_radius(const TileCone& t, const float b[4]) {
    const double C[3] = {(double)b[0], (double)b[1], (double)b[2]};
    const double cc = C[0] * C[0] + C[1] * C[1] + C[2] * C[2];
    double rf2 = cc - (double)b[3];
    if (!(rf2 > 0.0)) rf2 = 0.0;
    const double rf = __builtin_sqrt(rf2), omax = t.normO + t.rhoL;
    return __builtin_sqrt(rf2 + kTileMaskPerRay * omax * omax) + 1e-3 * rf + 1e-4 * (t.normO + __builtin_sqrt(cc) + rf);
}

RT_DEV bool tile_cone_reaches(const TileCone& t, const float b[4]) {
    const double R = tile_group_radius(t, b);
    const double w[3] = {(double)b[0] - t.o[0], (double)b[1] - t.o[1], (double)b[2] - t.o[2]};
    const double DD = t.D[0] * t.D[0] + t.D[1] * t.D[1] + t.D[2] * t.D[2];
    const double wD = w[0] * t.D[0] + w[1] * t.D[1] + w[2] * t.D[2];
    const double ww = w[0] * w[0] + w[1] * w[1] + w[2] * w[2];
    if (!(R == R) || !(ww == ww)) return true;
    return tm_piece_reached(DD, wD, ww, R + t.rhoL, t.rhoF - t.rhoL, 0.0, 1.0) ||
           tm_piece_reached(DD, wD, ww, R - t.rhoL, t.rhoF + t.rhoL, 1.0, -1.0);
}

RT_DEV int tile_group_reached(const TileMaskCam& c, const rt_rowset& rs, uint32_t tile, const float b[4]) {
    const uint32_t p0 = tile << 6, p1 = p0 + 63u;
    int reached = 0;
    for (uint32_t lr = p0 / c.W; lr <= p1 / c.W; ++lr) {
        const uint32_t r0 = lr * c.W;
        const uint32_t i0 = (p0 > r0 ? p0 : r0) - r0, i1 = (p1 < r0 + c.W - 1u ? p1 : r0 + c.W - 1u) - r0;
        const uint32_t lb = lr / rs.block_rows;
        const uint32_t j = rs.first_row + (lb * rs.nshards + rs.shard) * rs.block_rows + (lr - lb * rs.block_rows);
        const TileCone t = tile_run_cone(c, i0, i1, j);
        if (!t.ok) return -1;
        if (tile_cone_reaches(t, b)) reached = 1;
    }
    return reached;
}

RT_DEV void tile_mask_slot(uint32_t g, uint32_t& word, uint32_t& bit) {
    const uint32_t r = g & 63u, q = r >> 4;
    word = (g >> 6) + 2u * (q & 1u);
    bit = 0x80000000u >> ((r & 15u) + 16u * (q >> 1));
}

}
```

### include/rt_api.h

```cpp
#ifndef RT_API_H
#define RT_API_H

#include <stdint.h>

#ifdef __cplusplus
extern "C" {
#endif

#define RT_API_VERSION 2

enum rt_status {
    RT_OK = 0,
    RT_ERR_NO_DEVICE = 1,
    RT_ERR_INVALID_ARG = 2,
    RT_ERR_NO_SCENE = 3,
    RT_ERR_HIP = 4,
    RT_ERR_OUT_OF_MEMORY = 5,
    RT_ERR_SEQUENCE = 6
};


typedef struct rt_sphere {
    float cx, cy, cz, r;
} rt_sphere;

enum rt_material_type {
    RT_MAT_DIELECTRIC_OPAQUE = 0,
    RT_MAT_METAL = 1,
    RT_MAT_DIELECTRIC_TRANSPARENT = 2,
    RT_MAT_EMISSIVE = 3
};

enum rt_texture_type {
    RT_TEX_CONST = 0,
    RT_TEX_CHECKER = 1
};

typedef struct rt_material {
    uint32_t type;
    uint32_t tex_type;
    float smoothness;
    float ior;
    float tiling;
    float rgb0[3];
    float rgb1[3];
    float luminance;
} rt_material;

typedef struct rt_camera {
    float origin[4];
    float x[4];
    float y[4];
    float origin_image_plane[4];
    float aperture;
    float focal_length;
} rt_camera;

typedef struct rt_light {
    float direction[3];
    float color[3];
    float luminance;
} rt_light;

typedef struct rt_rowset {
    uint32_t first_row;
    uint32_t num_rows;
    uint32_t block_rows;
    uint32_t shard;
    uint32_t nshards;
} rt_rowset;

typedef struct rt_stats {
    uint64_t samples;
    uint64_t traversals;
    uint64_t segments;
    double ms_render;
    double ms_accumulate;
    double ms_resolve;
    uint32_t local_rows;
    uint32_t passes;
} rt_stats;

typedef struct rt_ctx rt_ctx;


const char* rt_last_error(void);
int rt_api_version(void);

int rt_create(int device_ordinal, rt_ctx** out);
void rt_destroy(rt_ctx* ctx);

int rt_set_stream(rt_ctx* ctx, void* hip_stream);

int rt_set_workspace_limit(rt_ctx* ctx, uint64_t bytes);


#define RT_MAX_LIGHTS 8
int rt_scene_upload(rt_ctx* ctx, const rt_sphere* spheres, const rt_material* materials, uint32_t n,
                    const rt_camera* camera, const rt_light* lights, uint32_t n_lights, const rt_material* sky,
                    float exposure_scale);


int rt_render(rt_ctx* ctx, uint32_t W, uint32_t H, rt_rowset rs, uint32_t s0, uint32_t s1,
              uint32_t max_depth, uint64_t seed, rt_stats* out_stats);

#define RT_SAMPLER_COSINE_HEMISPHERE 1u
#define RT_SAMPLER_SQRT_DISK 2u
int rt_set_sampler(rt_ctx* ctx, uint32_t flags);

int rt_set_frame_pipelining(rt_ctx* ctx, uint32_t depth);
int rt_set_frame_batch(rt_ctx* ctx, uint32_t frames);
int rt_set_frame_lookahead(rt_ctx* ctx, uint32_t frames);
int rt_committed_samples(rt_ctx* ctx, uint32_t* out);

int rt_clear(rt_ctx* ctx);

int rt_resolve(rt_ctx* ctx, uint32_t n_samples);
double rt_last_resolve_ms(rt_ctx* ctx);

int rt_download(rt_ctx* ctx, float* hdr_rgb, uint8_t* ldr_rgb);

int rt_copy_to_device(rt_ctx* ctx, void* dev_hdr_rgb, void* dev_ldr_rgb);

int rt_synchronize(rt_ctx* ctx);

uint32_t rt_rowset_local_rows(rt_rowset rs);
uint32_t rt_rowset_global_row(rt_rowset rs, uint32_t local_row);


int rt_unit_halton(rt_ctx* ctx, const uint32_t* index, uint32_t base, uint32_t n, float* out);
int rt_unit_math(rt_ctx* ctx, uint32_t op, const float* x, const float* y, uint32_t n, float* out);
int rt_unit_primary_rays(rt_ctx* ctx, uint32_t W, uint32_t H, const uint32_t* ijs ,
                         uint32_t n, float* out_rays);
int rt_unit_closest_hit(rt_ctx* ctx, const float* rays, uint32_t n, float* out_hits);
int rt_unit_trace(rt_ctx* ctx, uint32_t W, uint32_t H, const uint32_t* ijs, uint32_t n,
                  uint32_t max_depth, uint64_t seed, float* out_rgb, uint32_t* out_traversals);

int rt_unit_camera_rays(rt_ctx* ctx, const rt_camera* camera, const float* uv_offset, uint32_t n, float* out_rays);
int rt_unit_scatter(rt_ctx* ctx, const rt_material* material, const rt_light* sun, const float view_origin[3],
                    const float* in, uint32_t n, float* out);
int rt_unit_layout(const rt_sphere* spheres, uint32_t n, uint32_t cap_groups, uint32_t* n_groups, uint32_t* orig, float* bounds);
int rt_unit_layout_info(const rt_sphere* spheres, uint32_t n, uint32_t out[5]);
int rt_unit_grid_rows(const float* segments, const int32_t* iu, uint32_t n, int32_t nv, int32_t* out_rows, float* out_s_enter);
int rt_unit_tile_masks(rt_ctx* ctx, uint32_t W, uint32_t H, rt_rowset rs, uint32_t cap_tiles, uint32_t* n_tiles, uint32_t* words,
                       uint32_t cap_spheres, uint32_t* group_of_sphere, uint64_t scans[2]);
int rt_unit_tile_masks_host(const rt_sphere* spheres, uint32_t n, const rt_camera* camera, uint32_t W, uint32_t H, rt_rowset rs, uint32_t limit,
                            uint32_t cap_tiles, uint32_t* n_tiles, uint32_t* words, uint32_t* group_of_sphere);
int rt_unit_tile_cone(const rt_camera* camera, uint32_t W, uint32_t H, uint32_t i0, uint32_t i1, uint32_t j, double out[9]);
int rt_unit_tonemap(rt_ctx* ctx, const float* hdr_rgb, uint32_t n, uint32_t n_samples, uint8_t* out_rgb);

#ifdef __cplusplus
}
#endif
#endif
```

Baseline: 10400 Msamples/s.

## Add per-tile sphere lists for direct primary-ray intersection

Extends the tile mask kernel to build, per 64-pixel tile, an explicit list of up to 24 leaf sphere entries whose bounds are reached by the tile's primary-ray cone. Primary rays in tiles with a valid short list then run a brute-force broadcast intersection over only those spheres instead of the masked MFMA group scan. This is meant to cut primary-ray traversal work, at the cost of extra mask-build work, extra memory and a separate scan path that must return the same closest hit. Unit-test entry points and counters for direct-scanned tiles are added.

```diff
diff --git a/cpuraytracer_amd/_capi.py b/cpuraytracer_amd/_capi.py
--- a/cpuraytracer_amd/_capi.py
+++ b/cpuraytracer_amd/_capi.py
@@ -49,7 +49,7 @@
     "rt_scene_upload", "rt_render", "rt_clear", "rt_resolve", "rt_last_resolve_ms", "rt_download", "rt_copy_to_device",
     "rt_synchronize", "rt_rowset_local_rows", "rt_rowset_global_row", "rt_unit_halton", "rt_unit_math",
     "rt_unit_primary_rays", "rt_unit_closest_hit", "rt_unit_trace", "rt_unit_camera_rays", "rt_unit_scatter", "rt_unit_tonemap", "rt_unit_layout", "rt_unit_layout_info", "rt_unit_grid_rows",
-    "rt_unit_tile_masks", "rt_unit_tile_masks_host", "rt_unit_tile_cone",
+    "rt_unit_tile_masks", "rt_unit_tile_masks_host", "rt_unit_tile_cone", "rt_unit_tile_spheres", "rt_unit_tile_spheres_host",
 ]
 
 _lib = None
@@ -114,6 +114,10 @@
         L.rt_unit_tile_masks_host.argtypes = [C.c_void_p, C.c_uint32, C.POINTER(RtCamera), C.c_uint32, C.c_uint32, RtRowset, C.c_uint32,
                                               C.c_uint32, C.POINTER(C.c_uint32), C.c_void_p, C.c_void_p]
         L.rt_unit_tile_cone.argtypes = [C.POINTER(RtCamera), C.c_uint32, C.c_uint32, C.c_uint32, C.c_uint32, C.c_uint32, C.c_void_p]
+    if hasattr(L, "rt_unit_tile_spheres"):
+        L.rt_unit_tile_spheres.argtypes = [C.c_void_p, C.c_uint32, C.c_uint32, RtRowset, C.c_uint32, C.POINTER(C.c_uint32), C.c_void_p, C.c_void_p]
+        L.rt_unit_tile_spheres_host.argtypes = [C.c_void_p, C.c_uint32, C.POINTER(RtCamera), C.c_uint32, C.c_uint32, RtRowset, C.c_uint32, C.c_uint32,
+                                                C.c_uint32, C.POINTER(C.c_uint32), C.c_void_p, C.c_void_p]
     _lib = L
     return L
 
diff --git a/cpuraytracer_amd/csrc/rt_capi.hip b/cpuraytracer_amd/csrc/rt_capi.hip
--- a/cpuraytracer_amd/csrc/rt_capi.hip
+++ b/cpuraytracer_amd/csrc/rt_capi.hip
@@ -133,8 +133,10 @@
     DevBuf<uint8_t> tileClass;
     bool tileMaskValid = false;
     uint32_t maskW = 0, maskH = 0, maskLimit = 0, maskTiles = 0;
+    uint32_t maskSpheres = 0;
     rt_rowset maskRs{};
     DevBuf<uint32_t> tileMasks;
+    DevBuf<uint16_t> tileSpheres;
     uint64_t freshScans = 0;
 
     uint32_t pipeDepth = 0;
@@ -1018,8 +1020,13 @@
     return RT_OK;
 }
 
+static uint32_t TileSphereLimitFromEnv() {
+    const uint32_t v = EnvU32("RT_PRIMARY_SPHERES", rtd::kTileSphereLimitDefault);
+    return v > rtd::kTileSphereMax ? rtd::kTileSphereMax : v;
+}
 static int BuildTileMasks(rt_ctx* ctx, uint32_t W, uint32_t H, rt_rowset rs, uint32_t npix) {
     const uint32_t limit = EnvU32("RT_PRIMARY_MASK_LIMIT", rtd::kTileMaskLimitDefault);
+    const uint32_t sphLimit = TileSphereLimitFromEnv();
     const uint32_t nFull = npix >> 6;
     const rtd::TraceParams& b = ctx->base;
     const bool wanted = EnvU32("RT_PRIMARY_MASK", 1u) != 0u && nFull != 0u && b.n_levels == 1u && b.level_cnt[0] <= 128u &&
@@ -1028,21 +1035,25 @@
         ctx->tileMaskValid = false;
         return RT_OK;
     }
-    if (ctx->tileMaskValid && ctx->maskW == W && ctx->maskH == H && ctx->maskLimit == limit && std::memcmp(&ctx->maskRs, &rs, sizeof(rs)) == 0)
+    if (ctx->tileMaskValid && ctx->maskW == W && ctx->maskH == H && ctx->maskLimit == limit && ctx->maskSpheres == sphLimit &&
+        std::memcmp(&ctx->maskRs, &rs, sizeof(rs)) == 0)
         return RT_OK;
     ctx->tileMaskValid = false;
     int rc;
     if ((rc = ctx->tileMasks.Reserve((size_t)nFull * rtd::kTileMaskWords)) != RT_OK) return rc;
+    if (sphLimit != 0u && (rc = ctx->tileSpheres.Reserve((size_t)nFull * rtd::kTileSphereHalfs)) != RT_OK) return rc;
     rtd::TraceParams tp = b;
     tp.W = W;
     tp.H = H;
     tp.rs = rs;
-    hipLaunchKernelGGL(rtd::rt_tile_mask_kernel, dim3((nFull + 3) / 4), dim3(256), 0, ctx->stream, tp, nFull, limit, ctx->tileMasks.ptr);
+    hipLaunchKernelGGL(rtd::rt_tile_mask_kernel, dim3((nFull + 3) / 4), dim3(256), 0, ctx->stream, tp, nFull, limit, ctx->tileMasks.ptr,
+                       sphLimit, sphLimit != 0u ? ctx->tileSpheres.ptr : nullptr);
     RT_HIP(hipGetLastError());
     ctx->tileMaskValid = true;
     ctx->maskW = W;
     ctx->maskH = H;
     ctx->maskLimit = limit;
+    ctx->maskSpheres = sphLimit;
     ctx->maskTiles = nFull;
     ctx->maskRs = rs;
     return RT_OK;
@@ -1224,7 +1235,7 @@
     ctx->blockThreads = EnvU32("RT_BLOCK_THREADS", ctx->useMfma ? 1024 : 256);
     if (ctx->blockThreads != 256 && ctx->blockThreads != 512 && ctx->blockThreads != 1024) ctx->blockThreads = 256;
     int rc = ctx->queue.Reserve(rtd::kQueueShards * rtd::kShardStrideWords);
-    if (rc == RT_OK) rc = ctx->counters.Reserve(4);
+    if (rc == RT_OK) rc = ctx->counters.Reserve(6);
     if (rc != RT_OK) return rc;
     {
         size_t freeB = 0, totalB = 0;
@@ -1274,6 +1285,7 @@
     ctx->pilotHits.Release();
     ctx->tileOrder.Release();
     ctx->tileMasks.Release();
+    ctx->tileSpheres.Release();
     ctx->tileClass.Release();
     ctx->matType.Release();
     ctx->ring.Release();
@@ -1719,7 +1731,7 @@
     uint32_t passes = 0;
     auto runPasses = [&]() -> int {
         int rc;
-        RT_HIP(hipMemsetAsync(ctx->counters.ptr, 0, 4 * sizeof(unsigned long long), ctx->stream));
+        RT_HIP(hipMemsetAsync(ctx->counters.ptr, 0, 6 * sizeof(unsigned long long), ctx->stream));
         ctx->freshScans = 0;
         const uint32_t sEnd = aheadEnd ? aheadEnd : s1;
         for (uint32_t s = s0; s < sEnd; s += sppPass) {
@@ -1738,6 +1750,7 @@
             tp.path_list = nullptr;
             tp.tile_order = ctx->tileOrderValid ? ctx->tileOrder.ptr : nullptr;
             tp.tile_masks = (ctx->tileMaskValid && ctx->maskW == W && ctx->maskH == H && std::memcmp(&ctx->maskRs, &rs, sizeof(rs)) == 0) ? ctx->tileMasks.ptr : nullptr;
+            tp.tile_spheres = (tp.tile_masks != nullptr && ctx->maskSpheres != 0u) ? ctx->tileSpheres.ptr : nullptr;
             ctx->freshScans += ((uint64_t)tp.total_paths + 63u) / 64u;
             tp.samples = ctx->samples.ptr;
             tp.trav_out = nullptr;
@@ -1959,7 +1972,7 @@
     RT_HIP(dTrav.Alloc(n));
     RT_HIP(dOut.Alloc((size_t)n * 3));
     RT_HIP(hipMemcpy(dIjs.p, ijs, (size_t)n * 3 * sizeof(uint32_t), hipMemcpyHostToDevice));
-    RT_HIP(hipMemsetAsync(ctx->counters.ptr, 0, 4 * sizeof(unsigned long long), ctx->stream));
+    RT_HIP(hipMemsetAsync(ctx->counters.ptr, 0, 6 * sizeof(unsigned long long), ctx->stream));
     rtd::TraceParams tp = ctx->base;
     tp.W = W;
     tp.H = H;
@@ -2163,6 +2176,77 @@
     return RT_OK;
 }
 
+int rt_unit_tile_spheres(rt_ctx* ctx, uint32_t W, uint32_t H, rt_rowset rs, uint32_t cap_tiles, uint32_t* n_tiles, uint16_t* lists, uint64_t scans[3]) {
+    if (!ctx || !n_tiles || W == 0 || H == 0) return Fail(RT_ERR_INVALID_ARG, "rt_unit_tile_spheres: invalid argument");
+    if (!ctx->hasScene) return Fail(RT_ERR_NO_SCENE, "rt_unit_tile_spheres: no scene uploaded");
+    const uint32_t rows = RowsetLocalRows(rs);
+    if (rows == 0 || (uint64_t)rs.first_row + rs.num_rows > H || (uint64_t)W * rows > (1ull << 31)) return Fail(RT_ERR_INVALID_ARG, "rt_unit_tile_spheres: bad row set");
+    RT_HIP(hipSetDevice(ctx->device));
+    int rc;
+    if ((rc = BuildTileMasks(ctx, W, H, rs, W * rows)) != RT_OK) return rc;
+    *n_tiles = (ctx->tileMaskValid && ctx->maskSpheres != 0u) ? ctx->maskTiles : 0u;
+    RT_HIP(hipStreamSynchronize(ctx->stream));
+    if (lists && *n_tiles != 0u) {
+        if (cap_tiles < *n_tiles) return Fail(RT_ERR_INVALID_ARG, "rt_unit_tile_spheres: capacity too small");
+        RT_HIP(hipMemcpy(lists, ctx->tileSpheres.ptr, (size_t)*n_tiles * rtd::kTileSphereHalfs * sizeof(uint16_t), hipMemcpyDeviceToHost));
+    }
+    if (scans) {
+        unsigned long long c[5] = {0, 0, 0, 0, 0};
+        RT_HIP(hipMemcpy(c, ctx->counters.ptr, sizeof(c), hipMemcpyDeviceToHost));
+        scans[0] = ctx->freshScans;
+        scans[1] = c[3];
+        scans[2] = c[4];
+    }
+    return RT_OK;
+}
+
+int rt_unit_tile_spheres_host(const rt_sphere* spheres, uint32_t n, const rt_camera* camera, uint32_t W, uint32_t H, rt_rowset rs, uint32_t mask_limit,
+                              uint32_t sphere_limit, uint32_t cap_tiles, uint32_t* n_tiles, uint16_t* lists, uint32_t* entry_of_sphere) {
+    if (!spheres || n == 0 || !camera || !n_tiles || W == 0 || H == 0) return Fail(RT_ERR_INVALID_ARG, "rt_unit_tile_spheres_host: invalid argument");
+    const uint32_t rows = RowsetLocalRows(rs);
+    if (rows == 0 || (uint64_t)rs.first_row + rs.num_rows > H || (uint64_t)W * rows > (1ull << 31)) return Fail(RT_ERR_INVALID_ARG, "rt_unit_tile_spheres_host: bad row set");
+    if (sphere_limit > rtd::kTileSphereMax) sphere_limit = rtd::kTileSphereMax;
+    SceneLayout L;
+    BuildLayout(spheres, n, TreeTopFromEnv(), L);
+    const uint32_t nTop = L.levelCnt[L.nLevels - 1];
+    const uint32_t nFull = (W * rows) >> 6;
+    *n_tiles = (L.nLevels == 1 && !L.gridOn && nTop <= 128u && sphere_limit != 0u) ? nFull : 0u;
+    if (entry_of_sphere) {
+        for (uint32_t k = 0; k < n; ++k) entry_of_sphere[k] = 0xffffffffu;
+        for (uint32_t e = 0; e < (uint32_t)L.orig.size(); ++e)
+            if (L.orig[e] < n) entry_of_sphere[L.orig[e]] = e;
+    }
+    if (*n_tiles == 0u || !lists) return RT_OK;
+    if (cap_tiles < nFull) return Fail(RT_ERR_INVALID_ARG, "rt_unit_tile_spheres_host: capacity too small");
+    const rtd::TileMaskCam c = rtd::tile_mask_cam(camera->origin, camera->x, camera->y, camera->origin_image_plane, camera->aperture, camera->focal_length, W, H);
+    std::vector<int> reached(nTop);
+    for (uint32_t t = 0; t < nFull; ++t) {
+        uint16_t* rec = lists + (size_t)rtd::kTileSphereHalfs * t;
+        for (uint32_t k = 0; k < rtd::kTileSphereHalfs; ++k) rec[k] = 0;
+        bool bad = false;
+        uint32_t cnt = 0;
+        for (uint32_t g = 0; g < nTop; ++g) {
+            const float4 B = L.tree[L.levelOff[L.nLevels - 1] + g];
+            const float b[4] = {B.x, B.y, B.z, B.w};
+            reached[g] = rtd::tile_group_reached(c, rs, t, b);
+            bad = bad || reached[g] < 0;
+            cnt += reached[g] > 0 ? 1u : 0u;
+        }
+        uint32_t nS = 0;
+        const bool masked = rtd::tile_mask_flags(bad, cnt, mask_limit) != 0u;
+        for (uint32_t e = 0; masked && e < 4u * nTop && e < (uint32_t)L.leaf.size() && nS <= sphere_limit; ++e) {
+            const float4 B = L.leaf[e];
+            const float b[4] = {B.x, B.y, B.z, B.w};
+            if (rtd::tile_entry_listed(c, rs, t, reached[e >> 2], L.orig[e], b)) {
+                if (nS < sphere_limit) rec[1u + nS] = (uint16_t)e;
+                ++nS;
+            }
+        }
+        rec[0] = (uint16_t)((masked && nS <= sphere_limit) ? nS : rtd::kTileSphereNone);
+    }
+    return RT_OK;
+}
+
 int rt_unit_tile_cone(const rt_camera* camera, uint32_t W, uint32_t H, uint32_t i0, uint32_t i1, uint32_t j, double out[9]) {
     if (!camera || !out || W == 0 || H == 0) return Fail(RT_ERR_INVALID_ARG, "rt_unit_tile_cone: invalid argument");
     const rtd::TileMaskCam c = rtd::tile_mask_cam(camera->origin, camera->x, camera->y, camera->origin_image_plane, camera->aperture, camera->focal_length, W, H);
diff --git a/cpuraytracer_amd/csrc/rt_kernels.h b/cpuraytracer_amd/csrc/rt_kernels.h
--- a/cpuraytracer_amd/csrc/rt_kernels.h
+++ b/cpuraytracer_amd/csrc/rt_kernels.h
@@ -573,7 +573,12 @@
                             if (tw < (p.npix_local >> 6)) {
                                 const uint32_t tile = (uint32_t)__builtin_amdgcn_readfirstlane((int)(p.tile_order ? p.tile_order[tw] : tw));
                                 const uint32_t flags = (uint32_t)__builtin_amdgcn_readfirstlane((int)p.tile_masks[kTileMaskWords * tile + 4u]);
-                                if (flags & 1u) primTile = tile;
+                                if (flags & 1u) {
+                                    primTile = tile;
+                                    if (p.tile_spheres != nullptr &&
+                                        (uint32_t)__builtin_amdgcn_readfirstlane((int)p.tile_spheres[(size_t)kTileSphereHalfs * tile]) != kTileSphereNone)
+                                        primTile = tile | 0x80000000u;
+                                }
                             }
                         }
                     }
@@ -729,12 +734,17 @@
         const bool live = kStash ? (state == kNeedClosest || state == kNeedShadow) : (state != kIdle);
         if (kMfma) {
             const uint32_t* tileMask = nullptr;
+            if (kPrim && primTile != 0xffffffffu && (primTile & 0x80000000u) != 0u) {
+                if (lane == 0) __hip_atomic_fetch_add(&ldsK->prim_direct, 1u, __ATOMIC_RELAXED, __HIP_MEMORY_SCOPE_WORKGROUP);
+                scan_tile_spheres(scanTab, origTab, p.tile_spheres + (size_t)kTileSphereHalfs * (primTile & 0x7fffffffu), ro, rd, live, tmin, idx, lane);
+            } else {
             if (kPrim && primTile != 0xffffffffu) {
                 tileMask = p.tile_masks + kTileMaskWords * primTile;
                 if (lane == 0) __hip_atomic_fetch_add(&ldsK->prim_masked, 1u, __ATOMIC_RELAXED, __HIP_MEMORY_SCOPE_WORKGROUP);
             }
             scan_list_mfma<kScan == 2, kPrim>(scanTab, leafTab, origTab, mfmaOps, nTiles, nTop, treeTab, p.level_off, p.n_levels, p.bound_norm, p.single_mask, p.n_always, p.tree_box_on ? p.tree_box : nullptr, ro, rd,
                                        live, tmin, idx, waveCand, lane, dbgScan, tileMask);
+            }
         } else if (kScan == 3) {
             const GridParams G{gridCells, p.grid_nu, p.grid_nv, p.grid_ax_u, p.grid_ax_v, p.grid_g0u, p.grid_g0v, p.grid_inv_h, p.grid_rmax_over_h, p.grid_big_norm};
             const GridQuant Q{gridQ, p.grid_q[0], p.grid_q[1], p.grid_q[2], p.grid_q[3], p.grid_q[4], p.grid_q[5], p.grid_q[6], p.grid_q[7]};
@@ -835,7 +845,11 @@
         if (kPrim && p.tile_masks != nullptr) {
             const uint32_t ticket = __hip_atomic_fetch_add(&ldsK->exit_ticket, 1u, __ATOMIC_ACQ_REL, __HIP_MEMORY_SCOPE_WORKGROUP);
             if (ticket == (uint32_t)(kThreads / kWaveSize) - 1u)
-                atomicAdd(&p.counters[3], (unsigned long long)__hip_atomic_load(&ldsK->prim_masked, __ATOMIC_RELAXED, __HIP_MEMORY_SCOPE_WORKGROUP));
+            {
+                const unsigned long long nDirect = __hip_atomic_load(&ldsK->prim_direct, __ATOMIC_RELAXED, __HIP_MEMORY_SCOPE_WORKGROUP);
+                atomicAdd(&p.counters[3], nDirect + (unsigned long long)__hip_atomic_load(&ldsK->prim_masked, __ATOMIC_RELAXED, __HIP_MEMORY_SCOPE_WORKGROUP));
+                atomicAdd(&p.counters[4], nDirect);
+            }
         }
 #ifdef RT_STAMPS
         atomicAdd(&g_dbg[0], cyRefill);
@@ -969,7 +983,8 @@
 }
 
 static_assert(kTileMaskPerRay == 2.0 * (double)kMarginRel, "the masks bound the filter's own per-ray margin");
-__global__ void __launch_bounds__(256) rt_tile_mask_kernel(const TraceParams p, uint32_t nFull, uint32_t limit, uint32_t* __restrict__ words) {
+__global__ void __launch_bounds__(256) rt_tile_mask_kernel(const TraceParams p, uint32_t nFull, uint32_t limit, uint32_t* __restrict__ words,
+                                                           uint32_t sphLimit, uint16_t* __restrict__ lists) {
     const uint32_t tile = blockIdx.x * 4u + (threadIdx.x >> 6), lane = threadIdx.x & 63u;
     if (tile >= nFull) return;
     RT_SITE(T_MASK);
@@ -997,6 +1012,27 @@
         uint4* w = reinterpret_cast<uint4*>(words + (size_t)kTileMaskWords * tile);
         w[0] = make_uint4(wordA(m0), wordA(m1), wordB(m0), wordB(m1));
         w[1] = make_uint4(tile_mask_flags(bad, cnt, limit), cnt, 0u, 0u);
+    }
+    if (lists != nullptr) {
+        RT_SITE(T_SPHERES);
+        uint16_t* rec = lists + (size_t)kTileSphereHalfs * tile;
+        const bool masked = tile_mask_flags(bad, (uint32_t)(__popcll(m0) + __popcll(m1)), limit) != 0u && sphLimit != 0u && sphLimit <= kTileSphereMax;
+        uint32_t nS = 0;
+        for (uint32_t e0 = 0; masked && e0 < 4u * nTop && nS <= sphLimit; e0 += 64u) {
+            const uint32_t e = e0 + lane, g = e >> 2;
+            bool in = false;
+            if (g < nTop && e < p.n_padded) {
+                const int gr = (int)(((g < 64u ? m0 : m1) >> (g & 63u)) & 1ull);
+                const float4 B = p.leaf[e];
+                const float b[4] = {B.x, B.y, B.z, B.w};
+                in = tile_entry_listed(c, p.rs, tile, gr, p.orig[e], b);
+            }
+            const uint64_t m = __ballot(in);
+            const uint32_t at = nS + prefix_count(m);
+            if (in && at < sphLimit) rec[1u + at] = (uint16_t)e;
+            nS += (uint32_t)__popcll(m);
+        }
+        if (lane == 0) rec[0] = (uint16_t)((masked && nS <= sphLimit) ? nS : kTileSphereNone);
     }
 }
 
diff --git a/cpuraytracer_amd/csrc/rt_params.h b/cpuraytracer_amd/csrc/rt_params.h
--- a/cpuraytracer_amd/csrc/rt_params.h
+++ b/cpuraytracer_amd/csrc/rt_params.h
@@ -161,6 +161,7 @@
     uint32_t* shard_heads;
     unsigned long long* counters;
     const uint32_t* tile_masks;
+    const uint16_t* tile_spheres;
 };
 
 struct SceneConsts {
@@ -179,6 +180,7 @@
     uint32_t exit_ticket;
     uint32_t dry_mask;
     uint32_t prim_masked;
+    uint32_t prim_direct;
 };
 constexpr uint32_t kSceneConstBytes = 256;
 constexpr uint32_t kConstBytes = kSceneConstBytes + 8 * 256;
@@ -195,7 +197,7 @@
     k.sg_nx = p.sg_nx; k.sg_ny = p.sg_ny; k.sg_nglobal = p.sg_nglobal; k.sg_enabled = p.sg_enabled;
     k.W = p.W; k.H = p.H; k.s0 = p.s0; k.lens_k0 = p.lens_k0; k.sampler = p.sampler;
     k.jitter_tab = p.jitter_tab; k.lens_tab = p.lens_tab;
-    k.exit_age_max = 0u; k.exit_ticket = 0u; k.dry_mask = 0u; k.prim_masked = 0u;
+    k.exit_age_max = 0u; k.exit_ticket = 0u; k.dry_mask = 0u; k.prim_masked = 0u; k.prim_direct = 0u;
 }
 
 RT_DEV uint32_t rowset_global_row(const rt_rowset& rs, uint32_t lr, FastDiv byBlockRows) {
diff --git a/cpuraytracer_amd/csrc/rt_scan.h b/cpuraytracer_amd/csrc/rt_scan.h
--- a/cpuraytracer_amd/csrc/rt_scan.h
+++ b/cpuraytracer_amd/csrc/rt_scan.h
@@ -344,6 +344,60 @@
     cur &= ~(0x8000000000000000ull >> N);
     gid = hOff + N + (N & 48u);
     return true;
+}
+
+RT_DEV void scan_tile_spheres(const float4* __restrict__ tab, const uint32_t* __restrict__ orig, const uint16_t* __restrict__ rec, V3 o, V3 d, bool live,
+                              float& tmin, int& idx, uint32_t lane) {
+    RT_SITE(S_DIRECT);
+    const float a = dot3(d, d);
+    tmin = __builtin_inff();
+    idx = -1;
+    const uint32_t n = (uint32_t)__builtin_amdgcn_readfirstlane((int)rec[0]);
+    const uint32_t ent = lane < n ? (uint32_t)rec[1u + lane] : 0u;
+    const float4 S = tab[ent];
+    const uint32_t low = (orig[ent] << 16) | ent;
+#if RT_MARKSTEIN && RT_EXACT_MARKSTEIN
+    const bool aOk = (__float_as_uint(a) - 0x36000000u) <= 0x3b800000u;
+    const float ya = recip_rn(a);
+#endif
+    unsigned long long best = ~0ull;
+    for (uint32_t k = 0; k < n; ++k) {
+        RT_SITE(S_DIRECT_STEP);
+        const float sx = __int_as_float(__builtin_amdgcn_readlane(__float_as_int(S.x), (int)k));
+        const float sy = __int_as_float(__builtin_amdgcn_readlane(__float_as_int(S.y), (int)k));
+        const float sz = __int_as_float(__builtin_amdgcn_readlane(__float_as_int(S.z), (int)k));
+        const float sw = __int_as_float(__builtin_amdgcn_readlane(__float_as_int(S.w), (int)k));
+        const float ocx = o.x - sx;
+        const float ocy = o.y - sy;
+        const float ocz = o.z - sz;
+        const float b = (ocx * d.x + ocy * d.y) + ocz * d.z;
+        const float cc = ((ocx * ocx + ocy * ocy) + ocz * ocz) - sw;
+        const float e = b * b - a * cc;
+        if (__ballot(live && root_possible(e, b)) == 0ull) continue;
+        RT_SITE(S_DIRECT_ROOT);
+        const float sq = sqrt_rn(e > 0.f ? e : 1.f);
+        float t;
+#if RT_MARKSTEIN && RT_EXACT_MARKSTEIN
+        const bool ok = aOk && (__builtin_fabsf(b) + sq) < 0x1p100f;
+        if (__builtin_expect(__ballot(!ok) == 0ull, 1)) {
+            t = div_rn(-b - sq, a, ya);
+            if (!(t > 0.001f)) t = div_rn(-b + sq, a, ya);
+        } else
+#endif
+        {
+            RT_SITE(M_ROOT_SLOW);
+            t = (-b - sq) / a;
+            if (!(t > 0.001f)) t = (-b + sq) / a;
+        }
+        const uint32_t lowK = (uint32_t)__builtin_amdgcn_readlane((int)low, (int)k);
+        const unsigned long long key = ((unsigned long long)__float_as_uint(t) << 32) | (unsigned long long)lowK;
+        if (live && e > 0.f && t > 0.001f && t < __builtin_inff() && key < best) best = key;
+    }
+    const uint32_t tb = (uint32_t)(best >> 32);
+    if (tb < 0x7f800000u) {
+        tmin = __uint_as_float(tb);
+        idx = (int)(best & 0xffffull);
+    }
 }
 
 template <bool kTree, bool kPrim = false>
diff --git a/cpuraytracer_amd/csrc/rt_sites.h b/cpuraytracer_amd/csrc/rt_sites.h
--- a/cpuraytracer_amd/csrc/rt_sites.h
+++ b/cpuraytracer_amd/csrc/rt_sites.h
@@ -10,7 +10,7 @@
     X(H_SQ_ROOTS) X(H_SQ_FULL) X(H_SHADE) X(H_INDEXED) X(H_FARHIT) X(S_SCAN) X(S_TILEPAIR) X(S_SINGLE) \
     X(S_SINGLE_PUSH0) X(S_SINGLE_PUSH1) X(S_PASS) X(S_TAKE) X(S_PUSH_WORD) X(S_TAKE_PUSH0) X(S_TAKE_PUSH1) X(S_ASTEP) X(S_ASTEP2) X(S_APUSH) X(S_DRAIN) X(S_BSTEP) X(S_BSTEP2) X(S_BMIN) \
     X(G_SCAN) X(G_DRAIN) X(G_BSTEP) X(G_BMIN) X(G_BIG) X(G_BIGPUSH) X(G_FEED) X(G_FEED_LANE) X(G_ROUND) X(G_STEP) X(G_PUSH) \
-    X(K_GEN_TILE) X(S_MASKED) X(T_MASK)
+    X(K_GEN_TILE) X(S_MASKED) X(T_MASK) X(T_SPHERES) X(S_DIRECT) X(S_DIRECT_STEP) X(S_DIRECT_ROOT)
 enum RtSite : uint32_t {
 #define RT_SITE_ENUM(n) SITE_##n,
     RT_SITE_LIST(RT_SITE_ENUM)
diff --git a/cpuraytracer_amd/csrc/rt_tile_mask.h b/cpuraytracer_amd/csrc/rt_tile_mask.h
--- a/cpuraytracer_amd/csrc/rt_tile_mask.h
+++ b/cpuraytracer_amd/csrc/rt_tile_mask.h
@@ -134,6 +134,16 @@
     return reached;
 }
 
+constexpr uint32_t kTileSphereHalfs = 64;
+constexpr uint32_t kTileSphereMax = kTileSphereHalfs - 1u;
+constexpr uint32_t kTileSphereNone = 0xffffu;
+constexpr uint32_t kTileSphereLimitDefault = 24;
+
+RT_DEV bool tile_entry_listed(const TileMaskCam& c, const rt_rowset& rs, uint32_t tile, int groupReached, uint32_t og, const float lb[4]) {
+    if (groupReached <= 0 || og == 0xffffffffu) return false;
+    return tile_group_reached(c, rs, tile, lb) != 0;
+}
+
 RT_DEV void tile_mask_slot(uint32_t g, uint32_t& word, uint32_t& bit) {
     const uint32_t r = g & 63u, q = r >> 4;
     word = (g >> 6) + 2u * (q & 1u);
diff --git a/include/rt_api.h b/include/rt_api.h
--- a/include/rt_api.h
+++ b/include/rt_api.h
@@ -146,6 +146,9 @@
                        uint32_t cap_spheres, uint32_t* group_of_sphere, uint64_t scans[2]);
 int rt_unit_tile_masks_host(const rt_sphere* spheres, uint32_t n, const rt_camera* camera, uint32_t W, uint32_t H, rt_rowset rs, uint32_t limit,
                             uint32_t cap_tiles, uint32_t* n_tiles, uint32_t* words, uint32_t* group_of_sphere);
+int rt_unit_tile_spheres(rt_ctx* ctx, uint32_t W, uint32_t H, rt_rowset rs, uint32_t cap_tiles, uint32_t* n_tiles, uint16_t* lists, uint64_t scans[3]);
+int rt_unit_tile_spheres_host(const rt_sphere* spheres, uint32_t n, const rt_camera* camera, uint32_t W, uint32_t H, rt_rowset rs, uint32_t mask_limit,
+                              uint32_t sphere_limit, uint32_t cap_tiles, uint32_t* n_tiles, uint16_t* lists, uint32_t* entry_of_sphere);
 int rt_unit_tile_cone(const rt_camera* camera, uint32_t W, uint32_t H, uint32_t i0, uint32_t i1, uint32_t j, double out[9]);
 int rt_unit_tonemap(rt_ctx* ctx, const float* hdr_rgb, uint32_t n, uint32_t n_samples, uint8_t* out_rgb);
 
```

New measurement: 11580 Msamples/s (median of 6 runs). 1.11x the previous value.
